# AndrewRLawrence/dp_gp_lvm

Measured on AMD Instinct MI355X. Metric: ELBO evals/sec (N=2000,D=512,M=128,Q=10), higher is better.
Workload: dtype f32 (psi-statistics: f16 hi/lo-split MFMA operands, fp32 accumulate) + f64 (Cholesky chain)

## Files before the change

dp_gp_lvm_amd/_lib.py:

```python
import ctypes
import os

_HERE = os.path.dirname(os.path.abspath(__file__))
LIB_PATH = os.environ.get('DPGP_LIBRARY') or os.path.join(_HERE, 'csrc', 'libdpgp_hip.so')

FLAG_NOISE, FLAG_JITTER = 1, 2
ALGO = {'auto': 0, 'plain': 1, 'mfma_f32': 2, 'patch_f16': 3}
PREC = {'f32': 0, 'mixed': 1, 'f64': 2, 'mixed_patch': 3, 'mixed_fast': 4}

_vp, _i, _d, _sz = ctypes.c_void_p, ctypes.c_int, ctypes.c_double, ctypes.c_size_t
_ll = ctypes.c_longlong

SIGNATURES = {
    'dpgp_version': (_i, []),
    'dpgp_last_hip_error': (ctypes.c_char_p, []),
    'dpgp_psi1T_y_workspace_bytes': (_sz, [_i, _i, _i]),
    'dpgp_psi2_workspace_bytes': (_sz, [_i, _i, _i, _i, _i]),
    'dpgp_potrf_workspace_bytes': (_sz, [_i, _i, _i]),
    'dpgp_trsm_workspace_bytes': (_sz, [_i, _i, _i, _i]),
    'dpgp_elbo_workspace_bytes': (_sz, [_i, _i, _i, _i, _i]),
    'dpgp_elbo_workspace_layout': (_i, [_i, _i, _i, _i, _i, _vp]),
    'dpgp_elbo_workspace_front_layout': (_i, [_i, _i, _i, _i, _i, _vp]),
    'dpgp_elbo_fhat': (_i, [_i, _i, _i, _i, _vp, _i, _vp, _vp, _vp, _vp, _vp, _vp, _d, _i, _i, _vp, _vp, _vp, _vp, _sz,
                            _vp]),
    'dpgp_elbo_fhat_ex': (_i, [_i, _i, _i, _i, _vp, _i, _vp, _vp, _vp, _vp, _vp, _vp, _d, _i, _i, _vp, _vp, _vp, _vp, _sz,
                               _vp, _vp]),
    'dpgp_elbo_fhat_t_workspace_bytes': (_sz, [_i, _i, _i, _i, _i, _i]),
    'dpgp_elbo_fhat_t': (_i, [_i, _i, _i, _i, _i, _vp, _i, _vp, _vp, _vp, _vp, _vp, _vp, _vp, _vp, _ll, _ll, _d, _i, _vp, _vp,
                              _vp, _vp, _vp, _sz, _vp, _vp, _vp, _vp, _vp, _vp, _vp]),
    'dpgp_elbo_grad_chain': (_i, [_i, _i, _i, _i, _vp, _vp, _d, _i, _vp, _sz, _vp, _vp, _vp, _vp, _vp, _vp]),
    'dpgp_elbo_grad_chain_ex': (_i, [_i, _i, _i, _i, _vp, _vp, _d, _i, _vp, _sz, _i, _vp, _vp, _vp, _vp, _vp, _vp]),
    'dpgp_elbo_grad_psi_workspace_bytes': (_sz, [_i, _i, _i, _i]),
    'dpgp_elbo_grad_psi_workspace_bytes_ex': (_sz, [_i, _i, _i, _i, _i]),
    'dpgp_elbo_fhat_step': (_i, [_i, _i, _i, _i, _vp, _i, _vp, _vp, _vp, _vp, _vp, _vp, _d, _vp, _vp, _vp, _vp, _sz, _vp, _sz, _vp, _vp]),
    'dpgp_elbo_grad_psi_step': (_i, [_i, _i, _i, _i, _vp, _i, _vp, _vp, _vp, _vp, _vp, _vp, _vp, _vp, _i, _vp, _sz, _vp, _sz, _vp, _vp,
                                     _vp, _vp, _vp]),
    'dpgp_elbo_step': (_i, [_i, _i, _i, _i, _vp, _i, _vp, _vp, _vp, _vp, _vp, _vp, _d, _i, _vp, _vp, _vp, _vp, _sz, _vp, _vp, _vp, _vp,
                            _vp, _vp, _sz, _vp, _vp, _vp, _vp, _vp, _vp]),
    'dpgp_elbo_grad_psi': (_i, [_i, _i, _i, _i, _vp, _i, _vp, _vp, _vp, _vp, _vp, _vp, _vp, _vp, _i, _vp, _sz, _vp, _vp, _vp,
                                _vp, _vp]),
    'dpgp_elbo_grad_psi_ex': (_i, [_i, _i, _i, _i, _vp, _i, _vp, _vp, _vp, _vp, _vp, _vp, _vp, _vp, _vp, _i, _vp, _sz, _vp, _vp,
                                   _vp, _vp, _vp]),
    'dpgp_event_create': (_vp, []),
    'dpgp_event_destroy': (None, [_vp]),
    'dpgp_stream_create': (_vp, []),
    'dpgp_stream_destroy': (None, [_vp]),
    'dpgp_event_elapsed_ms': (ctypes.c_float, [_vp, _vp]),
    'dpgp_model_prepare': (_i, [_i, _i, _i, _i, _i, _i, _vp, _vp, _vp, _vp, _vp, _vp, _vp, _vp, _d, _d, _i, _vp, _vp, _vp,
                                _vp, _vp, _vp, _vp]),
    'dpgp_model_prepare_t': (_i, [_i, _i, _i, _i, _i, _i, _vp, _vp, _vp, _vp, _vp, _vp, _vp, _vp, _d, _d, _i, _vp, _vp, _vp,
                                  _vp, _vp]),
    'dpgp_model_scal_count': (_i, [_i]),
    'dpgp_model_backward': (_i, [_i] * 8 + [_vp] * 10 + [_d, _d, _i] + [_vp] * 15 + [_vp]),
    'dpgp_model_backward_t': (_i, [_i] * 8 + [_vp] * 10 + [_d, _d, _i] + [_vp] * 16 + [_vp]),
    'dpgp_model_pack': (_i, [_i, _vp, _vp, _vp, _vp]),
    'dpgp_model_finalize': (_i, [_vp, _vp, _vp, _vp, _vp]),
    'dpgp_elbo_grad_chain_big_workspace_bytes': (_sz, [_i, _i]),
    'dpgp_elbo_grad_chain_big': (_i, [_i, _i, _i, _i, _vp, _vp, _vp, _vp, _d, _i, _vp, _sz, _i, _vp, _sz, _vp, _vp, _vp, _vp, _vp, _vp]),
    'dpgp_trouble_flag': (_i, [_sz, _vp, _i, _vp, _vp, _vp]),
    'dpgp_trtri_lower_batched_f64': (_i, [_i, _i, _vp, _vp, _vp, _sz, _vp]),
    'dpgp_ard_rbf_gram_grad_workspace_bytes': (_sz, [_i, _i]),
    'dpgp_ard_rbf_gram_grad_f64': (_i, [_i, _i, _vp, _vp, _vp, _vp, _i, _vp, _vp, _vp, _vp, _sz, _vp]),
    'dpgp_ard_rbf_gram_grad_batched_workspace_bytes': (_sz, [_i, _i, _i]),
    'dpgp_ard_rbf_gram_grad_batched_f64': (_i, [_i, _i, _i, _vp, _vp, _vp, _vp, _i, _ll, _vp, _vp, _vp, _vp, _sz, _vp]),
    'dpgp_qx_psi_stats_workspace_bytes': (_sz, [_i, _i, _i, _i]),
    'dpgp_qx_psi_stats_batched_f64': (_i, [_i, _i, _i, _i] + [_vp] * 8 + [_vp, _sz, _vp]),
    'dpgp_qx_psi_adjoint_workspace_bytes': (_sz, [_i, _i, _i, _i]),
    'dpgp_qx_psi_adjoint_f64': (_i, [_i, _i, _i, _i] + [_vp] * 10 + [_vp, _sz, _vp]),
    'dpgp_qx_psi_stats_weighted_f64': (_i, [_i, _i, _i, _i] + [_vp] * 9 + [_vp, _sz, _vp]),
    'dpgp_qx_psi_adjoint_weighted_f64': (_i, [_i, _i, _i, _i] + [_vp] * 11 + [_vp, _sz, _vp]),
    'dpgp_qx_psi_param_adjoint_workspace_bytes': (_sz, [_i, _i, _i, _i]),
    'dpgp_qx_psi_param_adjoint_weighted_f64': (_i, [_i, _i, _i, _i] + [_vp] * 12 + [_vp, _sz, _vp]),
    'dpgp_qx_psi_stats_grouped_workspace_bytes': (_sz, [_i] * 5),
    'dpgp_qx_psi_stats_grouped_f64': (_i, [_i] * 5 + [_vp] * 9 + [_vp, _sz, _vp]),
    'dpgp_qx_psi_adjoint_grouped_workspace_bytes': (_sz, [_i] * 5),
    'dpgp_qx_psi_adjoint_grouped_f64': (_i, [_i] * 5 + [_vp] * 11 + [_vp, _sz, _vp]),
    'dpgp_qx_psi_param_adjoint_grouped_workspace_bytes': (_sz, [_i] * 5),
    'dpgp_qx_psi_param_adjoint_grouped_f64': (_i, [_i] * 5 + [_vp] * 12 + [_vp, _sz, _vp]),
    'dpgp_qx_psi_pointwise_workspace_bytes': (_sz, [_i] * 6),
    'dpgp_qx_psi_pointwise_f64': (_i, [_i] * 6 + [_vp] * 10 + [_vp, _sz, _vp]),
    'dpgp_qx_psi_point_moments_workspace_bytes': (_sz, [_i] * 6),
    'dpgp_qx_psi_point_moments_f64': (_i, [_i] * 6 + [_vp] * 12 + [_vp, _sz, _vp]),
    'dpgp_qx_psi_pointwise_adjoint_workspace_bytes': (_sz, [_i] * 6),
    'dpgp_qx_psi_pointwise_adjoint_f64': (_i, [_i] * 6 + [_vp] * 13 + [_vp, _sz, _vp]),
    'dpgp_ard_rbf_point_metric_workspace_bytes': (_sz, [_i] * 4),
    'dpgp_ard_rbf_point_metric_f64': (_i, [_i] * 4 + [_vp] * 6 + [_vp, _sz, _vp]),
    'dpgp_ard_rbf_point_jacobian_workspace_bytes': (_sz, [_i] * 5),
    'dpgp_ard_rbf_point_jacobian_f64': (_i, [_i] * 5 + [_vp] * 6 + [_vp, _sz, _vp]),
    'dpgp_ard_rbf_point_energy_workspace_bytes': (_sz, [_i] * 4),
    'dpgp_ard_rbf_point_energy_f64': (_i, [_i] * 4 + [_vp] * 9 + [_vp, _sz, _vp]),
    'dpgp_ard_rbf_point_christoffel_workspace_bytes': (_sz, [_i] * 4),
    'dpgp_ard_rbf_point_christoffel_f64': (_i, [_i] * 4 + [_vp] * 8 + [_vp, _sz, _vp]),
    'dpgp_geodesic_accel_f64': (_i, [_i] * 3 + [_vp] * 7 + [_vp]),
    'dpgp_ard_rbf_point_christoffel_tangent_workspace_bytes': (_sz, [_i] * 4),
    'dpgp_ard_rbf_point_christoffel_tangent_f64': (_i, [_i] * 4 + [_vp] * 12 + [_vp, _sz, _vp]),
    'dpgp_geodesic_accel_tangent_f64': (_i, [_i] * 3 + [_vp] * 10 + [_vp]),
    'dpgp_ard_rbf_point_transport_workspace_bytes': (_sz, [_i] * 5),
    'dpgp_ard_rbf_point_transport_f64': (_i, [_i] * 5 + [_vp] * 10 + [_vp, _sz, _vp]),
    'dpgp_geodesic_transport_f64': (_i, [_i] * 4 + [_vp] * 9 + [_vp]),
    'dpgp_geodesic_shoot_workspace_bytes': (_sz, [_i, _vp, _vp, _i, _i, _i]),
    'dpgp_geodesic_shoot_f64': (_i, [_i, _vp, _vp, _i, _i, _i] + [_vp] * 10 + [_vp, _sz, _vp]),
    'dpgp_geodesic_shoot_tangent_f64': (_i, [_i, _vp, _vp, _i, _i, _i] + [_vp] * 15 + [_vp, _sz, _vp]),
    'dpgp_ard_rbf_point_cov_workspace_bytes': (_sz, [_i] * 5),
    'dpgp_ard_rbf_point_cov_f64': (_i, [_i] * 5 + [_vp] * 6 + [_vp, _sz, _vp]),
    'dpgp_psi_latent_adjoint_workspace_bytes': (_sz, [_i] * 4),
    'dpgp_psi_latent_adjoint_f64': (_i, [_i] * 4 + [_vp] * 6 + [_i] + [_vp] * 5 + [_vp, _sz, _vp]),
    'dpgp_psi2_weighted_f64': (_i, [_i, _i, _i, _i, _vp, _vp, _vp, _vp, _vp, _vp, _vp, _vp, _sz, _i, _vp]),
    'dpgp_elbo_grad_psi_weighted_f64': (_i, [_i, _i, _i, _i, _vp, _i, _vp, _vp, _vp, _vp, _vp, _vp, _vp, _vp, _vp, _vp, _sz, _vp,
                                             _vp, _vp, _vp, _vp]),
    'dpgp_gemm_strided_f64': (_i, [_i, _i, _i, _i, _d, _vp, _ll, _ll, _ll, _vp, _ll, _ll, _ll, _d, _vp, _ll, _ll, _ll, _vp]),
}
for _t in ('f32', 'f64'):
    SIGNATURES.update({
        'dpgp_ard_rbf_gram_' + _t: (_i, [_i, _i, _i, _i, _vp, _vp, _vp, _vp, _vp, _i, _d, _vp, _vp]),
        'dpgp_ard_rbf_diag_' + _t: (_i, [_i, _i, _vp, _vp, _i, _d, _vp, _vp]),
        'dpgp_psi0_' + _t: (_i, [_i, _i, _vp, _vp, _vp]),
        'dpgp_psi1_' + _t: (_i, [_i, _i, _i, _i, _vp, _vp, _vp, _vp, _vp, _vp, _vp]),
        'dpgp_psi1T_y_' + _t: (_i, [_i, _i, _i, _i, _vp, _vp, _vp, _vp, _vp, _vp, _i, _vp, _vp, _sz, _vp]),
        'dpgp_psi2_' + _t: (_i, [_i, _i, _i, _i, _vp, _vp, _vp, _vp, _vp, _vp, _vp, _sz, _i, _vp]),
        'dpgp_potrf_batched_' + _t: (_i, [_i, _i, _vp, _vp, _vp, _sz, _i, _vp]),
        'dpgp_trsm_batched_' + _t: (_i, [_i, _i, _i, _vp, _vp, _vp, _sz, _i, _vp]),
        'dpgp_kl_qx_' + _t: (_i, [_i, _i, _vp, _vp, _vp, _vp]),
    })



class ExecResources(ctypes.Structure):
    _fields_ = [('ev_psi2_begin', _vp), ('ev_psi2_end', _vp), ('model_scal', _vp), ('model_pack', _vp),
                ('model_out', _vp), ('stream_aux', _vp), ('ev_fork', _vp), ('ev_join', _vp)]


_lib = None


class DpgpLibraryMissing(RuntimeError):
    pass


def lib():
    global _lib
    if _lib is None:
        if not os.path.exists(LIB_PATH):
            raise DpgpLibraryMissing(
                'libdpgp_hip.so is not built: run `make -C %s` (hipcc, gfx950). dp_gp_lvm_amd has no CPU fallback.'
                % os.path.join(_HERE, 'csrc'))
        import torch
        l = ctypes.CDLL(LIB_PATH)
        for name, (res, args) in SIGNATURES.items():
            fn = getattr(l, name)
            fn.restype, fn.argtypes = res, args
        _lib = l
    return _lib


def check(rc, name):
    if rc != 0:
        if rc == -100:
            raise RuntimeError('%s: HIP kernel launch failed: %s' % (name, lib().dpgp_last_hip_error().decode()))
        raise ValueError('%s: bad argument #%d' % (name, -rc))
```

dp_gp_lvm_amd/csrc/elbo.hip:

```cpp
#include "internal.h"
#include "psi2_consts.h"

struct ElboLayout {
    size_t off_yy, off_v, off_p2, off_la, off_ld, off_ik, off_kl, off_pc, off_guard, off_sc, total;
    int ns1, ns2, Mp;
};

static ElboLayout elbo_layout(int D, int N, int M, int Q, int prec) {
    ElboLayout L;
    L.Mp = dpgp_round_up(M, 16);
    L.ns1 = psi1T_y_nsplit(D, N, M);
    L.ns2 = psi2_nsplit(D, N, M);
    const size_t sp = (prec == DPGP_PREC_F64) ? 8 : 4, sl = (prec == DPGP_PREC_F32) ? 4 : 8;
    size_t o = 0;
    L.off_yy = o; o += dpgp_align256(sizeof(double) * DPGP_YY_NCH * D);
    L.off_ld = o; o += dpgp_align256(sizeof(double) * D);
    L.off_ik = o; o += dpgp_align256(sizeof(int) * D);
    L.off_kl = o; o += dpgp_align256(sizeof(double) * DPGP_KL_NBLK + sizeof(int));
    L.off_guard = o; o += dpgp_align256(sizeof(double) * D);
    L.off_pc = o; o += dpgp_align256(psi2_consts_bytes(M, Q));
    L.off_sc = o; o += (prec == DPGP_PREC_F64) ? 0 : psi2_pairs_scale_bytes(D, M);
    L.off_v = o;  o += dpgp_align256(sizeof(double) * (size_t)L.ns1 * D * M);
    L.off_p2 = o; o += dpgp_align256(sp * (size_t)L.ns2 * D * L.Mp * L.Mp);
    L.off_la = o; o += dpgp_align256(sl * (size_t)D * la_chain_ws_elems(M));
    L.total = o;
    return L;
}

extern "C" size_t dpgp_elbo_workspace_bytes(int D, int N, int M, int Q, int prec) {
    if (D <= 0 || N <= 0 || M <= 0 || Q <= 0 || prec < 0 || prec > 2) return 0;
    return elbo_layout(D, N, M, Q, prec).total;
}

extern "C" int dpgp_elbo_workspace_layout(int D, int N, int M, int Q, int prec, size_t *out) {
    if (D <= 0 || N <= 0 || M <= 0 || Q <= 0 || prec < 0 || prec > 2) return -1;
    if (!out) return -6;
    const ElboLayout L = elbo_layout(D, N, M, Q, prec);
    out[0] = L.off_p2; out[1] = (size_t)L.ns2; out[2] = (prec == DPGP_PREC_F64) ? 8 : 4; out[3] = (size_t)L.Mp;
    out[4] = L.off_v;  out[5] = (size_t)L.ns1; out[6] = L.off_yy; out[7] = DPGP_YY_NCH;
    out[8] = L.off_guard; out[9] = (size_t)D;
    return DPGP_OK;
}

extern "C" int dpgp_elbo_workspace_front_layout(int D, int N, int M, int Q, int prec, size_t *out) {
    if (D <= 0 || N <= 0 || M <= 0 || Q <= 0 || prec < 0 || prec > 2) return -1;
    if (!out) return -6;
    const ElboLayout L = elbo_layout(D, N, M, Q, prec);
    const size_t sl = (prec == DPGP_PREC_F32) ? 4 : 8;
    out[0] = L.off_la; out[1] = sl * la_chain_ws_elems(M); out[2] = sl; out[3] = (size_t)L.Mp;
    out[4] = L.off_sc;
    out[5] = (prec != DPGP_PREC_F64 && psi2_pairs_ksteps(Q) <= 8) ? (size_t)psi2_consts_layout(M, Q).Ppad : 0;
    return DPGP_OK;
}

struct AuxJoin {
    hipStream_t st = nullptr, aux = nullptr;
    hipEvent_t ev = nullptr;
    bool armed = false;
    void arm(hipStream_t st_, hipStream_t aux_, hipEvent_t ev_) { st = st_; aux = aux_; ev = ev_; armed = true; }
    int join() {
        armed = false;
        return hipStreamWaitEvent(st, ev, 0) == hipSuccess ? DPGP_OK : DPGP_ERR_LAUNCH;
    }
    ~AuxJoin() {
        if (armed && hipEventRecord(ev, aux) == hipSuccess) (void)hipStreamWaitEvent(st, ev, 0);
    }
};

struct SideLaunch {
    int (*fn)(void *ctx, hipStream_t st);
    void *ctx;
};

template <typename TP, typename TL>
static int elbo_run(int D, int N, int M, int Q, const double *y, int ldy, const double *z, const double *mu,
                    const double *s, const double *gamma, const double *alpha, const double *beta, double jitter,
                    int algo, double *terms, double *sums, int *info, unsigned char *ws, const ElboLayout &L,
                    hipStream_t st, const dpgp_exec_t *ex, TL *lb_out = nullptr, unsigned char *pgws = nullptr,
                    bool psi1_from_pass = false, const SideLaunch *side = nullptr, bool *side_done = nullptr) {
    double *yy = reinterpret_cast<double *>(ws + L.off_yy);
    double *ldk = reinterpret_cast<double *>(ws + L.off_ld);
    int *ik = reinterpret_cast<int *>(ws + L.off_ik);
    double *vpart = reinterpret_cast<double *>(ws + L.off_v);
    TP *p2 = reinterpret_cast<TP *>(ws + L.off_p2);
    TL *la = reinterpret_cast<TL *>(ws + L.off_la);
    double *klp = reinterpret_cast<double *>(ws + L.off_kl);
    unsigned char *pconst = ws + L.off_pc;
    hipEvent_t ev0 = ex ? (hipEvent_t)ex->ev_psi2_begin : nullptr, ev1 = ex ? (hipEvent_t)ex->ev_psi2_end : nullptr;
    int rc;
    const bool pairs_psi2 = (sizeof(TP) == 4 && algo == DPGP_ALGO_AUTO && psi2_pairs_ksteps(Q) <= 8);
    const bool fac_from_gram = pairs_psi2 && pgws == nullptr;
    float *pscale = reinterpret_cast<float *>(ws + L.off_sc);
    if ((rc = launch_elbo_front<TL>(N, Q, mu, s, klp, D, y, ldy, yy, z, M, pconst, gamma, alpha, beta, jitter, la, L.Mp,
                                    la_chain_ws_elems(M), (pairs_psi2 && !fac_from_gram) ? pscale : nullptr,
                                    fac_from_gram ? pscale : nullptr, st)))
        return rc;
    hipStream_t aux = (ex && ex->stream_aux && ex->ev_fork && ex->ev_join) ? (hipStream_t)ex->stream_aux : nullptr;
    if (pgws != nullptr && psi1_from_pass && D > 256) aux = nullptr;
    AuxJoin aj;
    if (aux) {
        if (hipEventRecord((hipEvent_t)ex->ev_fork, st) != hipSuccess || hipStreamWaitEvent(aux, (hipEvent_t)ex->ev_fork, 0) != hipSuccess)
            return DPGP_ERR_LAUNCH;
        aj.arm(st, aux, (hipEvent_t)ex->ev_join);
    }
    const int ns1 = psi1_from_pass ? 1 : L.ns1;
    if (!psi1_from_pass &&
        (rc = launch_psi1T_y_partial<double, TP>(D, N, M, Q, z, mu, s, gamma, alpha, y, ldy, vpart, L.ns1, pconst, 1, aux ? aux : st)))
        return rc;
    const bool k_on_aux = aux && pgws != nullptr && la_chain_k_resident(M, (int)sizeof(TL)) && algo != DPGP_ALGO_PLAIN;
    if (k_on_aux && (rc = launch_chain_k<TL>(D, M, la, ldk, ik, algo, aux))) return rc;
    if (aux && hipEventRecord((hipEvent_t)ex->ev_join, aux) != hipSuccess) return DPGP_ERR_LAUNCH;
    const bool f16_psi2 = (sizeof(TP) == 4 && algo != DPGP_ALGO_MFMA_F32);
    const bool step = pgws != nullptr;
    if (step && !(pairs_psi2 && psi2_pgrad_supported(M, Q))) return -30;
    const bool fused_k = !step && (algo != DPGP_ALGO_PLAIN) && (!f16_psi2 || la_chain_k_resident(M, (int)sizeof(TL))) &&
                         !getenv("DPGP_UNFUSED_K");
    bool big = false;
    if constexpr (sizeof(TL) == 8) {
        big = (algo != DPGP_ALGO_PLAIN) && chain_big_applicable(D, M, 8);
        if (big && (rc = launch_chain_big_k(D, M, reinterpret_cast<double *>(la), ik, st))) return rc;
    }
    if (!big && !fused_k && !k_on_aux && (rc = launch_chain_k<TL>(D, M, la, ldk, ik, algo, st))) return rc;
    if (ev0 && hipEventRecord(ev0, st) != hipSuccess) return DPGP_ERR_LAUNCH;
    if (step) {
        if constexpr (sizeof(TP) == 4) {
            if ((rc = launch_psi2_pgrad(D, N, M, Q, pconst, z, mu, s, gamma, alpha, nullptr, pgws, nullptr, nullptr, nullptr, nullptr,
                                        nullptr, st, 1, reinterpret_cast<float *>(p2), pscale, psi1_from_pass ? y : nullptr, ldy, nullptr, 0,
                                        psi1_from_pass ? vpart : nullptr)))
                return rc;
        }
    } else if ((rc = launch_psi2_partial<double, TP>(D, N, M, Q, z, mu, s, gamma, alpha, p2, L.ns2, algo, st,
                                                     (fused_k && !big) ? (void *)la : nullptr, (int)sizeof(TL), ldk, ik, pconst,
                                                     pairs_psi2 ? 2 : 1, pscale)))
        return rc;
    if (ev1 && hipEventRecord(ev1, st) != hipSuccess) return DPGP_ERR_LAUNCH;
    if (aux && aj.join() != DPGP_OK) return DPGP_ERR_LAUNCH;
    if (big && lb_out) return -30;
    if (side && aux && !big && 2 * D <= 512) {
        if (hipEventRecord((hipEvent_t)ex->ev_fork, st) != hipSuccess || hipStreamWaitEvent(aux, (hipEvent_t)ex->ev_fork, 0) != hipSuccess)
            return DPGP_ERR_LAUNCH;
        aj.arm(st, aux, (hipEvent_t)ex->ev_join);
        if ((rc = side->fn(side->ctx, aux))) return rc;
        if (hipEventRecord((hipEvent_t)ex->ev_join, aux) != hipSuccess) return DPGP_ERR_LAUNCH;
        rc = launch_chain_b<TP, TL>(D, N, M, p2, step ? 1 : L.ns2, vpart, ns1, alpha, beta, yy, ldk, ik, terms, info,
                                    reinterpret_cast<double *>(ws + L.off_guard), la, algo, st, klp, sums,
                                    ex ? (const double *)ex->model_scal : nullptr, ex ? (double *)ex->model_pack : nullptr,
                                    ex ? (double *)ex->model_out : nullptr, lb_out);
        if (rc) return rc;
        if (side_done) *side_done = true;
        return aj.join();
    }
    if constexpr (sizeof(TL) == 8) {
        if (big)
            return launch_chain_big_b<TP>(D, N, M, p2, step ? 1 : L.ns2, vpart, ns1, alpha, beta, yy, ik, terms, info,
                                          reinterpret_cast<double *>(ws + L.off_guard), reinterpret_cast<double *>(la), st, klp,
                                          sums, ex ? (const double *)ex->model_scal : nullptr,
                                          ex ? (double *)ex->model_pack : nullptr, ex ? (double *)ex->model_out : nullptr);
    }
    return launch_chain_b<TP, TL>(D, N, M, p2, step ? 1 : L.ns2, vpart, ns1, alpha, beta, yy, ldk, ik, terms, info,
                                  reinterpret_cast<double *>(ws + L.off_guard), la, algo, st, klp, sums,
                                  ex ? (const double *)ex->model_scal : nullptr, ex ? (double *)ex->model_pack : nullptr,
                                  ex ? (double *)ex->model_out : nullptr, lb_out);
}

extern "C" int dpgp_elbo_grad_chain_ex(int D, int N, int M, int Q, const double *alpha, const double *beta, double jitter,
                                       int prec, void *ws, size_t ws_bytes, int psi2_slabs, double *g_psi2, double *w_kuu, double *g_v,
                                       double *d_alpha_beta, int *info, void *stream) {
    if (D <= 0) return -1;
    if (N <= 0) return -2;
    if (M <= 0) return -3;
    if (Q <= 0 || Q > DPGP_MAX_Q) return -4;
    if (!alpha) return -5;
    if (!beta) return -6;
    if (!(jitter >= 0.0)) return -7;
    if (prec != DPGP_PREC_MIXED && prec != DPGP_PREC_F64) return -8;
    if (!ws) return -9;
    const ElboLayout L = elbo_layout(D, N, M, Q, prec);
    if (ws_bytes < L.total) return -10;
    if (!g_psi2) return -11;
    if (!w_kuu) return -12;
    if (!g_v) return -13;
    if (!d_alpha_beta) return -14;
    if (!info) return -15;
    if (psi2_slabs < 0 || psi2_slabs > L.ns2) return -16;
    unsigned char *w = (unsigned char *)ws;
    const double *yy = reinterpret_cast<const double *>(w + L.off_yy), *vpart = reinterpret_cast<const double *>(w + L.off_v);
    double *la = reinterpret_cast<double *>(w + L.off_la);
    const int ns2 = psi2_slabs ? psi2_slabs : L.ns2;
    if (prec == DPGP_PREC_MIXED)
        return launch_chain_grad<float>(D, N, M, reinterpret_cast<const float *>(w + L.off_p2), ns2, vpart, L.ns1, alpha,
                                        beta, yy, jitter, la, g_psi2, w_kuu, g_v, d_alpha_beta, info, (hipStream_t)stream);
    return launch_chain_grad<double>(D, N, M, reinterpret_cast<const double *>(w + L.off_p2), ns2, vpart, L.ns1, alpha,
                                     beta, yy, jitter, la, g_psi2, w_kuu, g_v, d_alpha_beta, info, (hipStream_t)stream);
}
extern "C" int dpgp_elbo_grad_chain(int D, int N, int M, int Q, const double *alpha, const double *beta, double jitter,
                                    int prec, void *ws, size_t ws_bytes, double *g_psi2, double *w_kuu, double *g_v,
                                    double *d_alpha_beta, int *info, void *stream) {
    return dpgp_elbo_grad_chain_ex(D, N, M, Q, alpha, beta, jitter, prec, ws, ws_bytes, 0, g_psi2, w_kuu, g_v, d_alpha_beta, info, stream);
}

extern "C" size_t dpgp_elbo_grad_chain_big_workspace_bytes(int D, int M) {
    return (D > 0 && M > 0) ? chain_grad_big_ws_bytes(D, M) : 0;
}
extern "C" int dpgp_elbo_grad_chain_big(int D, int N, int M, int Q, const double *z, const double *gamma, const double *alpha,
                                        const double *beta, double jitter, int prec, void *fwd_ws, size_t fwd_ws_bytes, int psi2_slabs,
                                        void *ws, size_t ws_bytes, double *g_psi2, double *w_kuu, double *g_v, double *d_alpha_beta,
                                        int *info, void *stream) {
    if (D <= 0) return -1;
    if (N <= 0) return -2;
    if (M <= 0 || !chain_grad_big_supported(M)) return -3;
    if (Q <= 0 || Q > DPGP_MAX_Q) return -4;
    if (!z) return -5;
    if (!gamma) return -6;
    if (!alpha) return -7;
    if (!beta) return -8;
    if (!(jitter >= 0.0)) return -9;
    if (prec != DPGP_PREC_MIXED && prec != DPGP_PREC_F64) return -10;
    if (!fwd_ws) return -11;
    const ElboLayout L = elbo_layout(D, N, M, Q, prec);
    if (fwd_ws_bytes < L.total) return -12;
    if (psi2_slabs < 0 || psi2_slabs > L.ns2) return -13;
    if (!ws) return -14;
    if (ws_bytes < chain_grad_big_ws_bytes(D, M)) return -15;
    if (!g_psi2) return -16;
    if (!w_kuu) return -17;
    if (!g_v) return -18;
    if (!d_alpha_beta) return -19;
    if (!info) return -20;
    const unsigned char *w = (const unsigned char *)fwd_ws;
    const double *yy = reinterpret_cast<const double *>(w + L.off_yy), *vpart = reinterpret_cast<const double *>(w + L.off_v);
    const int ns2 = psi2_slabs ? psi2_slabs : L.ns2;
    if (prec == DPGP_PREC_MIXED)
        return launch_chain_grad_big<float>(D, N, M, Q, z, gamma, alpha, beta, jitter, reinterpret_cast<const float *>(w + L.off_p2), ns2,
                                            vpart, L.ns1, yy, (unsigned char *)ws, g_psi2, w_kuu, g_v, d_alpha_beta, info, (hipStream_t)stream);
    return launch_chain_grad_big<double>(D, N, M, Q, z, gamma, alpha, beta, jitter, reinterpret_cast<const double *>(w + L.off_p2), ns2,
                                         vpart, L.ns1, yy, (unsigned char *)ws, g_psi2, w_kuu, g_v, d_alpha_beta, info, (hipStream_t)stream);
}

struct GradPsiWs { unsigned char *consts; double *part, *ws1, *stage; unsigned char *pgws; };
static bool grad_psi_needs_patch(int M, int Q, bool patch_form) {
    return patch_form || !psi2_pgrad_supported(M, Q) || getenv("DPGP_GRAD_PATCH");
}
static GradPsiWs grad_psi_ws(int D, int N, int M, int Q, unsigned char *ws, bool patch_form) {
    GradPsiWs W;
    const size_t mx = (size_t)Q * (N > D ? (N > M ? N : M) : (D > M ? D : M));
    W.consts = ws + dpgp_align256(psi_grad_ws_bytes_kuu(D, M, Q));
    W.part = reinterpret_cast<double *>(W.consts + dpgp_align256(psi2_consts_bytes(M, Q)));
    W.ws1 = reinterpret_cast<double *>((unsigned char *)W.part +
                                       (grad_psi_needs_patch(M, Q, patch_form) ? dpgp_align256(sizeof(double) * psi2_grad_part_elems(D, N, M, Q)) : 0));
    W.stage = reinterpret_cast<double *>((unsigned char *)W.ws1 + dpgp_align256(sizeof(double) * psi1_grad_ws_elems(D, N, M, Q)));
    W.pgws = reinterpret_cast<unsigned char *>(W.stage) + dpgp_align256(sizeof(double) * reduce_rows_stage_elems(mx));
    return W;
}
static int grad_psi_mixed(int D, int N, int M, int Q, const double *y, int ldy, const double *z, const double *mu, const double *s,
                          const double *gamma, const double *alpha, const double *g_psi2, const double *w_kuu, const double *g_v,
                          const double *g_psi1, bool patch_form, unsigned char *ws, double *d_mu, double *d_s, double *d_z,
                          double *d_gamma, hipStream_t st, const unsigned char *fwd_consts, const float *fwd_scale,
                          const float *fwd_psi2 = nullptr, int w11 = 0, double *psi1_front_done = nullptr) {
    const bool fast = psi2_grad_supported(M, Q) && !getenv("DPGP_GRAD_PLAIN");
    const bool big = dpgp_round_up(M, 16) > 128;
    if (big && !fast) return -30;
    int rc = DPGP_OK;
    if (!big && !fast) {
        if (g_psi1) return -15;
        return launch_psi_grad<float>(D, N, M, Q, y, ldy, z, mu, s, gamma, alpha, g_psi2, w_kuu, g_v ? g_v : w_kuu, (double *)ws,
                                      d_mu, d_s, d_z, d_gamma, 1, st);
    }
    const GradPsiWs W = grad_psi_ws(D, N, M, Q, ws, patch_form);
    const unsigned char *consts = fwd_consts ? fwd_consts : W.consts;
    if (!fwd_consts && (rc = launch_psi2_consts<double>(z, M, Q, W.consts, st)) != DPGP_OK) return rc;
    rc = launch_kuu_grad(D, M, Q, consts, gamma, w_kuu, (double *)ws, W.stage, d_z, d_gamma, st);
    if (rc != DPGP_OK) return rc;
    const bool pair_form = psi2_pgrad_supported(M, Q) && !patch_form && !getenv("DPGP_GRAD_PATCH");
    const bool psi1_pairs = pair_form && !g_psi1 && y && g_v && !getenv("DPGP_PSI1_PLAIN");
    if (!psi1_pairs) {
        rc = launch_psi1_grad(D, N, M, Q, y, ldy, consts, mu, s, gamma, alpha, g_v, g_psi1, W.ws1, W.stage, d_mu, d_s, d_z, d_gamma, st);
        if (rc != DPGP_OK) return rc;
    }
    if (pair_form)
        return launch_psi2_pgrad(D, N, M, Q, consts, z, mu, s, gamma, alpha, g_psi2, W.pgws, W.stage, d_mu, d_s, d_z, d_gamma, st,
                                 fwd_consts ? 2 : 3, const_cast<float *>(fwd_psi2), fwd_scale, psi1_pairs ? y : nullptr, ldy,
                                 psi1_pairs ? g_v : nullptr, w11, (fwd_consts && psi1_pairs) ? psi1_front_done : nullptr);
    if (fwd_consts) return -30;
    return launch_psi2_grad(D, N, M, Q, consts, mu, s, gamma, alpha, g_psi2, W.part, W.stage, d_mu, d_s, d_z, d_gamma, st);
}

extern "C" size_t dpgp_elbo_grad_psi_workspace_bytes_ex(int D, int N, int M, int Q, int prec) {
    if (D <= 0 || N <= 0 || M <= 0 || Q <= 0) return 0;
    if (prec == DPGP_PREC_F64 || !psi2_grad_supported(M, Q) || getenv("DPGP_GRAD_PLAIN"))
        return dpgp_align256(psi_grad_ws_bytes(D, N, M, Q, nullptr));
    const bool patch = (prec == DPGP_PREC_MIXED_PATCH);
    const size_t mx = (size_t)Q * (N > D ? (N > M ? N : M) : (D > M ? D : M));
    size_t b = dpgp_align256(psi_grad_ws_bytes_kuu(D, M, Q)) + dpgp_align256(psi2_consts_bytes(M, Q)) +
               (grad_psi_needs_patch(M, Q, patch) ? dpgp_align256(sizeof(double) * psi2_grad_part_elems(D, N, M, Q)) : 0) +
               dpgp_align256(sizeof(double) * psi1_grad_ws_elems(D, N, M, Q)) + dpgp_align256(sizeof(double) * reduce_rows_stage_elems(mx));
    if (!patch) b += dpgp_align256(psi2_pgrad_ws_bytes(D, N, M, Q));
    return b;
}
extern "C" size_t dpgp_elbo_grad_psi_workspace_bytes(int D, int N, int M, int Q) {
    return dpgp_elbo_grad_psi_workspace_bytes_ex(D, N, M, Q, DPGP_PREC_MIXED);
}
extern "C" int dpgp_elbo_grad_psi_ex(int D, int N, int M, int Q, const double *y, int ldy, const double *z, const double *mu,
                                     const double *s, const double *gamma, const double *alpha, const double *g_psi2,
                                     const double *w_kuu, const double *g_v, const double *g_psi1, int prec, void *ws,
                                     size_t ws_bytes, double *d_mu, double *d_s, double *d_z, double *d_gamma, void *stream);
extern "C" int dpgp_elbo_grad_psi(int D, int N, int M, int Q, const double *y, int ldy, const double *z, const double *mu,
                                  const double *s, const double *gamma, const double *alpha, const double *g_psi2,
                                  const double *w_kuu, const double *g_v, int prec, void *ws, size_t ws_bytes,
                                  double *d_mu, double *d_s, double *d_z, double *d_gamma, void *stream) {
    return dpgp_elbo_grad_psi_ex(D, N, M, Q, y, ldy, z, mu, s, gamma, alpha, g_psi2, w_kuu, g_v, nullptr, prec, ws, ws_bytes,
                                 d_mu, d_s, d_z, d_gamma, stream);
}
static int elbo_grad_psi_impl(int D, int N, int M, int Q, const double *y, int ldy, const double *z, const double *mu,
                              const double *s, const double *gamma, const double *alpha, const double *g_psi2,
                              const double *w_kuu, const double *g_v, const double *g_psi1, int prec, void *ws,
                              size_t ws_bytes, double *d_mu, double *d_s, double *d_z, double *d_gamma, void *stream,
                              const double *wts) {
    if (D <= 0) return -1;
    if (N <= 0) return -2;
    if (M <= 0) return -3;
    if (Q <= 0 || Q > DPGP_MAX_Q) return -4;
    if (!y && !g_psi1) return -5;
    if (y && ldy < D) return -6;
    if (!z) return -7;
    if (!mu) return -8;
    if (!s) return -9;
    if (!gamma) return -10;
    if (!alpha) return -11;
    if (!g_psi2) return -12;
    if (!w_kuu) return -13;
    if (!g_v && !g_psi1) return -14;
    const bool patch_form = (prec == DPGP_PREC_MIXED_PATCH), fast = (prec == DPGP_PREC_MIXED_FAST);
    if (patch_form || fast) prec = DPGP_PREC_MIXED;
    if (prec != DPGP_PREC_MIXED && prec != DPGP_PREC_F64) return -15;
    if (g_psi1 && (prec != DPGP_PREC_MIXED || !psi2_grad_supported(M, Q))) return -15;
    if (!ws) return -16;
    if (ws_bytes < dpgp_elbo_grad_psi_workspace_bytes_ex(D, N, M, Q, patch_form ? DPGP_PREC_MIXED_PATCH : prec)) return -17;
    if (!d_mu) return -18;
    if (!d_s) return -19;
    if (!d_z) return -20;
    if (!d_gamma) return -21;
    if (prec == DPGP_PREC_MIXED)
        return grad_psi_mixed(D, N, M, Q, y, ldy, z, mu, s, gamma, alpha, g_psi2, w_kuu, g_v, g_psi1, patch_form, (unsigned char *)ws,
                              d_mu, d_s, d_z, d_gamma, (hipStream_t)stream, nullptr, nullptr, nullptr, fast ? 1 : 0);
    if (dpgp_round_up(M, 16) > 128) return -30;
    return launch_psi_grad<double>(D, N, M, Q, y, ldy, z, mu, s, gamma, alpha, g_psi2, w_kuu, g_v, (double *)ws, d_mu, d_s,
                                   d_z, d_gamma, 1, (hipStream_t)stream, wts);
}
extern "C" int dpgp_elbo_grad_psi_ex(int D, int N, int M, int Q, const double *y, int ldy, const double *z, const double *mu,
                                     const double *s, const double *gamma, const double *alpha, const double *g_psi2,
                                     const double *w_kuu, const double *g_v, const double *g_psi1, int prec, void *ws,
                                     size_t ws_bytes, double *d_mu, double *d_s, double *d_z, double *d_gamma, void *stream) {
    return elbo_grad_psi_impl(D, N, M, Q, y, ldy, z, mu, s, gamma, alpha, g_psi2, w_kuu, g_v, g_psi1, prec, ws, ws_bytes, d_mu,
                              d_s, d_z, d_gamma, stream, nullptr);
}
extern "C" int dpgp_elbo_grad_psi_weighted_f64(int D, int N, int M, int Q, const double *y, int ldy, const double *z,
                                               const double *mu, const double *s, const double *gamma, const double *alpha,
                                               const double *w, const double *g_psi2, const double *w_kuu, const double *g_v,
                                               void *ws, size_t ws_bytes, double *d_mu, double *d_s, double *d_z,
                                               double *d_gamma, void *stream) {
    return elbo_grad_psi_impl(D, N, M, Q, y, ldy, z, mu, s, gamma, alpha, g_psi2, w_kuu, g_v, nullptr, DPGP_PREC_F64, ws,
                              ws_bytes, d_mu, d_s, d_z, d_gamma, stream, w);
}

extern "C" int dpgp_elbo_fhat_ex(int D, int N, int M, int Q, const double *y, int ldy, const double *z,
                                 const double *mu, const double *s, const double *gamma, const double *alpha,
                                 const double *beta, double jitter, int prec, int algo, double *terms, double *sums,
                                 int *info, void *ws, size_t ws_bytes, void *stream, const dpgp_exec_t *exec) {
    if (D <= 0) return -1;
    if (N <= 0) return -2;
    if (M <= 0) return -3;
    if (Q <= 0 || Q > DPGP_MAX_Q) return -4;
    if (!y) return -5;
    if (ldy < D) return -6;
    if (!z) return -7;
    if (!mu) return -8;
    if (!s) return -9;
    if (!gamma) return -10;
    if (!alpha) return -11;
    if (!beta) return -12;
    if (!(jitter >= 0.0)) return -13;
    if (prec < 0 || prec > 2) return -14;
    if (algo < 0 || algo > DPGP_ALGO_PATCH_F16) return -15;
    if (!terms) return -16;
    if (!sums) return -17;
    if (!info) return -18;
    if (!ws) return -19;
    const ElboLayout L = elbo_layout(D, N, M, Q, prec);
    if (ws_bytes < L.total) return -20;
    hipStream_t st = (hipStream_t)stream;
    unsigned char *w = (unsigned char *)ws;
    switch (prec) {
    case DPGP_PREC_F32:
        return elbo_run<float, float>(D, N, M, Q, y, ldy, z, mu, s, gamma, alpha, beta, jitter, algo, terms, sums, info,
                                      w, L, st, exec);
    case DPGP_PREC_MIXED:
        return elbo_run<float, double>(D, N, M, Q, y, ldy, z, mu, s, gamma, alpha, beta, jitter, algo, terms, sums,
                                       info, w, L, st, exec);
    default:
        return elbo_run<double, double>(D, N, M, Q, y, ldy, z, mu, s, gamma, alpha, beta, jitter, algo, terms, sums,
                                        info, w, L, st, exec);
    }
}

extern "C" int dpgp_elbo_fhat(int D, int N, int M, int Q, const double *y, int ldy, const double *z, const double *mu,
                              const double *s, const double *gamma, const double *alpha, const double *beta,
                              double jitter, int prec, int algo, double *terms, double *sums, int *info, void *ws,
                              size_t ws_bytes, void *stream) {
    return dpgp_elbo_fhat_ex(D, N, M, Q, y, ldy, z, mu, s, gamma, alpha, beta, jitter, prec, algo, terms, sums, info, ws,
                             ws_bytes, stream, nullptr);
}

extern "C" int dpgp_elbo_step(int D, int N, int M, int Q, const double *y, int ldy, const double *z, const double *mu,
                              const double *s, const double *gamma, const double *alpha, const double *beta, double jitter,
                              int prec, double *terms, double *sums, int *info, void *ws, size_t ws_bytes, double *g_psi2, double *w_kuu,
                              double *g_v, double *d_alpha_beta, int *info_grad, void *gws, size_t gws_bytes, double *d_mu,
                              double *d_s, double *d_z, double *d_gamma, void *stream, const dpgp_exec_t *exec) {
    if (D <= 0) return -1;
    if (N <= 0) return -2;
    if (M <= 0 || dpgp_round_up(M, 16) > 128) return -3;
    if (Q <= 0 || Q > DPGP_MAX_Q || !psi2_pgrad_supported(M, Q)) return -4;
    if (!y) return -5;
    if (ldy < D) return -6;
    if (!z) return -7;
    if (!mu) return -8;
    if (!s) return -9;
    if (!gamma) return -10;
    if (!alpha) return -11;
    if (!beta) return -12;
    if (!(jitter >= 0.0)) return -13;
    if (prec != DPGP_PREC_MIXED && prec != DPGP_PREC_MIXED_FAST) return -14;
    if (!terms) return -15;
    if (!sums) return -16;
    if (!info) return -17;
    if (!ws) return -18;
    const ElboLayout L = elbo_layout(D, N, M, Q, DPGP_PREC_MIXED);
    if (ws_bytes < L.total) return -19;
    if (!g_psi2) return -20;
    if (!w_kuu) return -21;
    if (!g_v) return -22;
    if (!d_alpha_beta) return -23;
    if (!info_grad) return -24;
    if (!gws) return -25;
    if (gws_bytes < dpgp_elbo_grad_psi_workspace_bytes(D, N, M, Q)) return -26;
    if (!d_mu) return -27;
    if (!d_s) return -28;
    if (!d_z) return -29;
    if (!d_gamma) return -30;
    hipStream_t st = (hipStream_t)stream;
    unsigned char *w = (unsigned char *)ws;
    const GradPsiWs W = grad_psi_ws(D, N, M, Q, (unsigned char *)gws, false);
    const bool v_from_pass = !getenv("DPGP_PSI1_PLAIN") && !getenv("DPGP_GRAD_PATCH") && !getenv("DPGP_GRAD_PLAIN");
    struct StageA {
        int D, N, M, ns1;
        const unsigned char *w;
        const ElboLayout *L;
        const double *alpha, *beta;
        double jitter, *g_psi2, *w_kuu, *g_v, *dab;
        int *info;
    } sa = {D, N, M, v_from_pass ? 1 : L.ns1, w, &L, alpha, beta, jitter, g_psi2, w_kuu, g_v, d_alpha_beta, info_grad};
    auto stage_a = [](void *c, hipStream_t s_) -> int {
        const StageA &a = *static_cast<const StageA *>(c);
        return launch_chain_grad<float>(a.D, a.N, a.M, reinterpret_cast<const float *>(a.w + a.L->off_p2), 1,
                                        reinterpret_cast<const double *>(a.w + a.L->off_v), a.ns1, a.alpha, a.beta,
                                        reinterpret_cast<const double *>(a.w + a.L->off_yy), a.jitter,
                                        reinterpret_cast<double *>(const_cast<unsigned char *>(a.w) + a.L->off_la), a.g_psi2, a.w_kuu, a.g_v,
                                        a.dab, a.info, s_);
    };
    const SideLaunch side = {stage_a, &sa};
    bool side_done = false;
    int rc = elbo_run<float, double>(D, N, M, Q, y, ldy, z, mu, s, gamma, alpha, beta, jitter, DPGP_ALGO_AUTO, terms, sums, info, w,
                                     L, st, exec, nullptr, W.pgws, v_from_pass, &side, &side_done);
    if (rc != DPGP_OK) return rc;
    if (!side_done && (rc = stage_a(&sa, st)) != DPGP_OK) return rc;
    return grad_psi_mixed(D, N, M, Q, y, ldy, z, mu, s, gamma, alpha, g_psi2, w_kuu, g_v, nullptr, false, (unsigned char *)gws, d_mu,
                          d_s, d_z, d_gamma, st, w + L.off_pc, reinterpret_cast<const float *>(w + L.off_sc),
                          reinterpret_cast<const float *>(w + L.off_p2), prec == DPGP_PREC_MIXED_FAST ? 1 : 0,
                          v_from_pass ? reinterpret_cast<double *>(w + L.off_v) : nullptr);
}

extern "C" int dpgp_elbo_fhat_step(int D, int N, int M, int Q, const double *y, int ldy, const double *z, const double *mu,
                                   const double *s, const double *gamma, const double *alpha, const double *beta, double jitter,
                                   double *terms, double *sums, int *info, void *ws, size_t ws_bytes, void *gws, size_t gws_bytes,
                                   void *stream, const dpgp_exec_t *exec) {
    if (D <= 0) return -1;
    if (N <= 0) return -2;
    if (M <= 0) return -3;
    if (Q <= 0 || Q > DPGP_MAX_Q || !psi2_pgrad_supported(M, Q)) return -4;
    if (!y) return -5;
    if (ldy < D) return -6;
    if (!z) return -7;
    if (!mu) return -8;
    if (!s) return -9;
    if (!gamma) return -10;
    if (!alpha) return -11;
    if (!beta) return -12;
    if (!(jitter >= 0.0)) return -13;
    if (!terms) return -14;
    if (!sums) return -15;
    if (!info) return -16;
    if (!ws) return -17;
    const ElboLayout L = elbo_layout(D, N, M, Q, DPGP_PREC_MIXED);
    if (ws_bytes < L.total) return -18;
    if (!gws) return -19;
    if (gws_bytes < dpgp_elbo_grad_psi_workspace_bytes(D, N, M, Q)) return -20;
    const GradPsiWs W = grad_psi_ws(D, N, M, Q, (unsigned char *)gws, false);
    return elbo_run<float, double>(D, N, M, Q, y, ldy, z, mu, s, gamma, alpha, beta, jitter, DPGP_ALGO_AUTO, terms, sums, info,
                                   (unsigned char *)ws, L, (hipStream_t)stream, exec, nullptr, W.pgws);
}
extern "C" int dpgp_elbo_grad_psi_step(int D, int N, int M, int Q, const double *y, int ldy, const double *z, const double *mu,
                                       const double *s, const double *gamma, const double *alpha, const double *g_psi2,
                                       const double *w_kuu, const double *g_v, int prec, void *ws, size_t ws_bytes, void *gws,
                                       size_t gws_bytes, double *d_mu, double *d_s, double *d_z, double *d_gamma, void *stream) {
    if (D <= 0) return -1;
    if (N <= 0) return -2;
    if (M <= 0) return -3;
    if (Q <= 0 || Q > DPGP_MAX_Q || !psi2_pgrad_supported(M, Q)) return -4;
    if (!y) return -5;
    if (ldy < D) return -6;
    if (!z) return -7;
    if (!mu) return -8;
    if (!s) return -9;
    if (!gamma) return -10;
    if (!alpha) return -11;
    if (!g_psi2) return -12;
    if (!w_kuu) return -13;
    if (!g_v) return -14;
    if (prec != DPGP_PREC_MIXED && prec != DPGP_PREC_MIXED_FAST) return -15;
    if (!ws) return -16;
    const ElboLayout L = elbo_layout(D, N, M, Q, DPGP_PREC_MIXED);
    if (ws_bytes < L.total) return -17;
    if (!gws) return -18;
    if (gws_bytes < dpgp_elbo_grad_psi_workspace_bytes(D, N, M, Q)) return -19;
    if (!d_mu) return -20;
    if (!d_s) return -21;
    if (!d_z) return -22;
    if (!d_gamma) return -23;
    unsigned char *w = (unsigned char *)ws;
    return grad_psi_mixed(D, N, M, Q, y, ldy, z, mu, s, gamma, alpha, g_psi2, w_kuu, g_v, nullptr, false, (unsigned char *)gws, d_mu,
                          d_s, d_z, d_gamma, (hipStream_t)stream, w + L.off_pc, reinterpret_cast<const float *>(w + L.off_sc),
                          reinterpret_cast<const float *>(w + L.off_p2), prec == DPGP_PREC_MIXED_FAST ? 1 : 0);
}

struct ElboTLayout {
    ElboLayout L;
    size_t off_fused, off_terms, off_sums, off_lb, off_p1, off_vp, total;
    int ksplit, nlow;
};
static ElboTLayout elbo_t_layout(int T, int D, int N, int M, int Q, int prec) {
    ElboTLayout E;
    E.L = elbo_layout(T, N, M, Q, prec);
    const int Mp = E.L.Mp, nb = Mp / 16;
    E.nlow = nb * (nb + 1) / 2;
    const int tiles = dpgp_ceil_div(D, 64) * dpgp_ceil_div(M, 64) * T;
    int ks = 512 / (tiles > 0 ? tiles : 1);
    if (ks > 8) ks = 8;
    if (ks > N / 64) ks = N / 64;
    if (ks < 1) ks = 1;
    E.ksplit = ks;
    size_t o = 0;
    E.off_fused = o; o += dpgp_align256(E.L.total);
    E.off_terms = o; o += dpgp_align256(sizeof(double) * 5 * T);
    E.off_sums = o;  o += 256;
    E.off_lb = o;    o += dpgp_align256(sizeof(double) * (size_t)T * E.nlow * DPGP_LB_TILE_ELEMS);
    E.off_p1 = o;    o += dpgp_align256(sizeof(double) * (size_t)T * N * M);
    E.off_vp = o;    o += dpgp_align256(sizeof(double) * (size_t)ks * T * M * D);
    E.total = o;
    return E;
}
extern "C" size_t dpgp_elbo_fhat_t_workspace_bytes(int T, int D, int N, int M, int Q, int prec) {
    if (T <= 0 || D < T || N <= 0 || M <= 0 || Q <= 0 || prec < 1 || prec > 2) return 0;
    return elbo_t_layout(T, D, N, M, Q, prec).total;
}

__global__ __launch_bounds__(256) void fhat_t_combine_kernel(int T, int D, int N, const double *__restrict__ terms,
                                                             const double *__restrict__ phit, const double *__restrict__ quad,
                                                             const double *__restrict__ yy, const double *__restrict__ beta,
                                                             const double *__restrict__ sums_in, double *__restrict__ per_t,
                                                             double *__restrict__ sums, long long phi_st, long long phi_sd,
                                                             const double *__restrict__ model_scal,
                                                             double *__restrict__ model_pack, double *__restrict__ model_out) {
    __shared__ double scratch[8];
    const int t = threadIdx.x;
    double acc = 0.0;
    for (int e = t; e < T * D; e += 256) {
        const int a = e / D, d = e - a * D;
        const double *o = terms + 5 * a;
        const double pt = o[0] + 0.5 * N * DPGP_LOG_2PI + o[1] + o[2];
        acc += phit[a * phi_st + d * phi_sd] * (pt + 0.5 * quad[e] - 0.5 * beta[a] * yy[d]);
    }
    acc = block_sum(acc, scratch);
    if (t < T) {
        const double *o = terms + 5 * t;
        per_t[t] = o[0] + 0.5 * N * DPGP_LOG_2PI + o[1] + o[2];
    }
    if (t == 0) {
        const double fhat = acc - 0.5 * (double)N * (double)D * DPGP_LOG_2PI, kl = sums_in[1];
        sums[0] = fhat;
        sums[1] = kl;
        if (model_scal) {
            double a = model_scal[0];
            const int nrb = (D + DPGP_PREP_ROWS - 1) / DPGP_PREP_ROWS;
            for (int i = 0; i < nrb; ++i) a += model_scal[2 + i];
            if (model_pack) { model_pack[0] = fhat; model_pack[1] = -a; }
            if (model_out) {
                const double hyper = model_scal[1];
                model_out[0] = -a - (fhat - kl) - hyper;
                model_out[1] = fhat; model_out[2] = kl; model_out[3] = -a; model_out[4] = hyper;
            }
        }
    }
}

extern "C" int dpgp_elbo_fhat_t(int T, int D, int N, int M, int Q, const double *y, int ldy, const double *yy, const double *z,
                                const double *mu, const double *s, const double *gamma, const double *alpha, const double *beta,
                                const double *phit, long long phi_st, long long phi_sd, double jitter, int prec, double *per_t,
                                double *quad, double *sums, int *info, void *ws, size_t ws_bytes, void *stream,
                                const double *model_scal, double *model_pack, double *model_out, void *stream_aux,
                                void *ev_fork, void *ev_join) {
    if (T <= 0) return -1;
    if (D < T) return -2;
    if (N <= 0) return -3;
    if (M <= 0) return -4;
    if (Q <= 0 || Q > DPGP_MAX_Q) return -5;
    if (!y) return -6;
    if (ldy < D) return -7;
    if (!yy) return -8;
    if (!z || !mu || !s) return -9;
    if (!gamma || !alpha || !beta) return -12;
    if (!phit) return -15;
    if (!(jitter >= 0.0)) return -16;
    if (prec != DPGP_PREC_MIXED && prec != DPGP_PREC_F64) return -17;
    if (!per_t || !quad || !sums || !info) return -18;
    if (!ws) return -22;
    if (dpgp_round_up(M, 16) > 128) return -30;
    const ElboTLayout E = elbo_t_layout(T, D, N, M, Q, prec);
    if (ws_bytes < E.total) return -23;
    hipStream_t st = (hipStream_t)stream;
    unsigned char *w = (unsigned char *)ws;
    double *terms = reinterpret_cast<double *>(w + E.off_terms), *sums2 = reinterpret_cast<double *>(w + E.off_sums);
    double *lb = reinterpret_cast<double *>(w + E.off_lb), *p1 = reinterpret_cast<double *>(w + E.off_p1);
    double *vp = reinterpret_cast<double *>(w + E.off_vp);
    int rc;
    hipStream_t aux = (stream_aux && ev_fork && ev_join) ? (hipStream_t)stream_aux : nullptr;
    if (aux) {
        hipStreamCaptureStatus cs = hipStreamCaptureStatusNone;
        if (hipStreamIsCapturing(st, &cs) != hipSuccess || cs != hipStreamCaptureStatusNone) aux = nullptr;
    }
    if (aux && (hipEventRecord((hipEvent_t)ev_fork, st) != hipSuccess || hipStreamWaitEvent(aux, (hipEvent_t)ev_fork, 0) != hipSuccess))
        return DPGP_ERR_LAUNCH;
    AuxJoin aj;
    if (aux) aj.arm(st, aux, (hipEvent_t)ev_join);
    hipStream_t sb = aux ? aux : st;
    if (aux) {
        if ((rc = dpgp_psi1_f64(T, N, M, Q, z, mu, s, gamma, alpha, p1, (void *)sb))) return rc - 100;
        if ((rc = launch_gemm_splitk_f64(T, M, D, N, p1, (long long)N * M, 1, M, y, 0, ldy, 1, vp, (long long)M * D, D, 1, E.ksplit,
                                         (long long)T * M * D, sb)))
            return rc - 200;
        if (hipEventRecord((hipEvent_t)ev_join, aux) != hipSuccess) return DPGP_ERR_LAUNCH;
    }
    if (prec == DPGP_PREC_MIXED)
        rc = elbo_run<float, double>(T, N, M, Q, y, ldy, z, mu, s, gamma, alpha, beta, jitter, DPGP_ALGO_AUTO, terms, sums2, info,
                                     w + E.off_fused, E.L, st, nullptr, lb);
    else
        rc = elbo_run<double, double>(T, N, M, Q, y, ldy, z, mu, s, gamma, alpha, beta, jitter, DPGP_ALGO_AUTO, terms, sums2, info,
                                      w + E.off_fused, E.L, st, nullptr, lb);
    if (rc) return rc;
    if (!aux) {
        if ((rc = dpgp_psi1_f64(T, N, M, Q, z, mu, s, gamma, alpha, p1, stream))) return rc - 100;
        if ((rc = launch_gemm_splitk_f64(T, M, D, N, p1, (long long)N * M, 1, M, y, 0, ldy, 1, vp, (long long)M * D, D, 1, E.ksplit,
                                         (long long)T * M * D, st)))
            return rc - 200;
    } else if (aj.join() != DPGP_OK) {
        return DPGP_ERR_LAUNCH;
    }
    if ((rc = launch_tcols_quad(T, M, D, lb, vp, E.ksplit, (long long)T * M * D, beta, quad, st))) return rc;
    DPGP_PRELAUNCH();
    hipLaunchKernelGGL(fhat_t_combine_kernel, dim3(1), dim3(256), 0, st, T, D, N, terms, phit, quad, yy, beta, sums2, per_t, sums,
                       phi_st, phi_sd, model_scal, model_pack, model_out);
    DPGP_LAUNCH_CHECK();
    return DPGP_OK;
}

extern "C" void *dpgp_event_create(void) {
    hipEvent_t e = nullptr;
    return hipEventCreate(&e) == hipSuccess ? (void *)e : nullptr;
}
extern "C" void dpgp_event_destroy(void *e) {
    if (e) (void)hipEventDestroy((hipEvent_t)e);
}
extern "C" void *dpgp_stream_create(void) {
    hipStream_t s = nullptr;
    return hipStreamCreateWithFlags(&s, hipStreamNonBlocking) == hipSuccess ? (void *)s : nullptr;
}
extern "C" void dpgp_stream_destroy(void *s) {
    if (s) (void)hipStreamDestroy((hipStream_t)s);
}
extern "C" float dpgp_event_elapsed_ms(void *a, void *b) {
    float ms = -1.0f;
    if (hipEventElapsedTime(&ms, (hipEvent_t)a, (hipEvent_t)b) != hipSuccess) return -1.0f;
    return ms;
}

__device__ __forceinline__ double softplus_d(double x) { return fmax(x, 0.0) + log1p(exp(-fabs(x))); }

__device__ double digamma_d(double x) {
    double r = 0.0;
    while (x < 10.0) { r -= 1.0 / x; x += 1.0; }
    const double f = 1.0 / (x * x);
    const double t = f * (-1.0 / 12.0 + f * (1.0 / 120.0 + f * (-1.0 / 252.0 + f * (1.0 / 240.0 + f * (-1.0 / 132.0 +
                     f * (691.0 / 32760.0 + f * (-1.0 / 12.0)))))));
    return r + log(x) - 0.5 / x + t;
}

#define PREP_MAX_T 64
#define PREP_ROWS DPGP_PREP_ROWS

__global__ __launch_bounds__(256) void model_prepare_kernel(
    int D, int T, int Q, int N, int d_offset, int mask_size, int nrb, const double *__restrict__ logits,
    const double *__restrict__ gat_raw, const double *__restrict__ aat_raw, const double *__restrict__ bat_raw,
    const double *__restrict__ s_raw, const double *__restrict__ g1_raw, const double *__restrict__ g2_raw,
    const double *__restrict__ w_raw, double s1, double s2, int add_constants, double *__restrict__ gamma,
    double *__restrict__ alpha, double *__restrict__ beta, double *__restrict__ s_out, double *__restrict__ phi_out,
    double *__restrict__ scal, double *__restrict__ atoms_out) {
    const int t = threadIdx.x;
    __shared__ double scratch[8];
    if ((int)blockIdx.x > nrb) {
        const size_t tot = (size_t)N * Q;
        const int nsb = gridDim.x - 1 - nrb;
        for (size_t i = (size_t)(blockIdx.x - 1 - nrb) * 256 + t; i < tot; i += (size_t)nsb * 256)
            s_out[i] = softplus_d(s_raw[i]);
        return;
    }
    if (blockIdx.x == 0) {
        double hyper = 0.0, consts = 0.0;
        for (int i = t; i < T * Q + 2 * T; i += 256) {
            const double raw = i < T * Q ? gat_raw[i] : (i < T * Q + T ? aat_raw[i - T * Q] : bat_raw[i - T * Q - T]);
            const double sp = softplus_d(raw), lx = log(sp);
            if (atoms_out) atoms_out[i] = sp;
            hyper += -lx - 0.5 * (DPGP_LOG_2PI + lx * lx);
        }
        const double w1 = softplus_d(w_raw[0]), w2 = softplus_d(w_raw[1]);
        __shared__ double sf[6][PREP_MAX_T], sx[3];
        for (int i = t; i < 6 * (T - 1) + 3; i += 256) {
            if (i < 6 * (T - 1)) {
                const int k = i / 6, f = i - 6 * k;
                const double g1 = softplus_d(g1_raw[k]), g2 = softplus_d(g2_raw[k]);
                const double x = (f % 3 == 0) ? g1 : ((f % 3 == 1) ? g2 : g1 + g2);
                sf[f][k] = f < 3 ? lgamma(x) : digamma_d(x);
            } else {
                const int f = i - 6 * (T - 1);
                sx[f] = f == 0 ? digamma_d(w1) : (f == 1 ? lgamma(s1) : lgamma(w1));
            }
        }
        __syncthreads();
        if (t < T - 1) {
            const double g1 = softplus_d(g1_raw[t]), g2 = softplus_d(g2_raw[t]);
            const double p1 = sf[3][t], p2 = sf[4][t], p12 = sf[5][t];
            consts += (w1 / w2 - 1.0) * (p2 - p12) +
                      (sf[0][t] + sf[1][t] - sf[2][t] - (g1 - 1.0) * p1 - (g2 - 1.0) * p2 + (g1 + g2 - 2.0) * p12);
        }
        if (t == 0) {
            const double pw = sx[0], lw2 = log(w2);
            consts += (T - 1.0) * (pw - lw2)
                      + s1 * log(s2) - sx[1] + (s1 - 1.0) * (pw - lw2) - s2 * (w1 / w2)
                      + w1 - lw2 + sx[2] + (1.0 - w1) * pw;
        }
        hyper = block_sum(hyper, scratch);
        consts = block_sum(consts, scratch);
        if (t == 0) {
            scal[0] = add_constants ? consts : 0.0;
            scal[1] = hyper;
        }
        return;
    }
    __shared__ double gat[PREP_MAX_T * DPGP_MAX_Q], aat[PREP_MAX_T], bat[PREP_MAX_T];
    __shared__ double c1[PREP_MAX_T], c2[PREP_MAX_T];
    for (int i = t; i < T * Q; i += 256) gat[i] = softplus_d(gat_raw[i]);
    if (t < T) {
        aat[t] = softplus_d(aat_raw[t]);
        bat[t] = softplus_d(bat_raw[t]);
    }
    __shared__ double dg[3][PREP_MAX_T];
    if (t >= 64 && t - 64 < 3 * (T - 1)) {
        const int k = (t - 64) / 3, f = (t - 64) - 3 * k;
        const double g1 = softplus_d(g1_raw[k]), g2 = softplus_d(g2_raw[k]);
        dg[f][k] = digamma_d(f == 0 ? g1 : (f == 1 ? g2 : g1 + g2));
    }
    __syncthreads();
    if (t < T - 1) {
        c1[t] = dg[0][t] - dg[2][t];
        c2[t] = dg[1][t] - dg[2][t];
    }
    __syncthreads();
    const int rb = blockIdx.x - 1, cols = Q + 1;
    double dsum = 0.0;
    for (int e = t; e < PREP_ROWS * cols; e += 256) {
        const int rr = e / cols, j = e - rr * cols, d = rb * PREP_ROWS + rr;
        if (d >= D) continue;
        const double *lr = logits + (size_t)((d_offset + d) / mask_size) * T;
        double mx = lr[0];
        for (int k = 1; k < T; ++k) mx = fmax(mx, lr[k]);
        double zsum = 0.0;
        for (int k = 0; k < T; ++k) zsum += exp(lr[k] - mx);
        const double lz = log(zsum);
        if (j < Q) {
            double g = 0.0;
            if (!gamma) continue;
            for (int k = 0; k < T; ++k) g += exp(lr[k] - mx - lz) * gat[k * Q + j];
            gamma[(size_t)d * Q + j] = g;
        } else {
            double al = 0.0, be = 0.0, ent = 0.0, ev = 0.0, tail = 0.0;
            for (int k = T - 1; k >= 0; --k) {
                const double lp = lr[k] - mx - lz, p = exp(lp);
                if (phi_out) phi_out[(size_t)d * T + k] = p;
                al += p * aat[k];
                be += p * bat[k];
                ent -= p * lp;
                if (k < T - 1) ev += p * c1[k] + tail * c2[k];
                tail += p;
            }
            if (alpha) alpha[d] = al;
            if (beta) beta[d] = be;
            dsum += ev + ent;
        }
    }
    dsum = block_sum(dsum, scratch);
    if (t == 0) scal[2 + rb] = dsum;
}

__global__ void model_finalize_kernel(const double *__restrict__ fhat, const double *__restrict__ dp,
                                      const double *__restrict__ kl, const double *__restrict__ hyper,
                                      double *__restrict__ out) {
    if (threadIdx.x == 0 && blockIdx.x == 0) {
        out[0] = dp[0] - (fhat[0] - kl[0]) - hyper[0];
        out[1] = fhat[0];
        out[2] = kl[0];
        out[3] = dp[0];
        out[4] = hyper[0];
    }
}

__global__ void model_pack_kernel(const double *__restrict__ fhat, const double *__restrict__ scal, int nrb,
                                  double *__restrict__ pack) {
    if (threadIdx.x == 0 && blockIdx.x == 0) {
        double a = scal[0];
        for (int i = 0; i < nrb; ++i) a += scal[2 + i];
        pack[0] = fhat[0];
        pack[1] = -a;
    }
}

__device__ double trigamma_d(double x) {
    double r = 0.0;
    while (x < 10.0) { r += 1.0 / (x * x); x += 1.0; }
    const double f = 1.0 / (x * x);
    return r + 1.0 / x + 0.5 * f + (1.0 / x) * f * (1.0 / 6.0 - f * (1.0 / 30.0 - f * (1.0 / 42.0 - f * (1.0 / 30.0 - f * (
               5.0 / 66.0 - f * (691.0 / 2730.0 - f * (7.0 / 6.0)))))));
}
__device__ __forceinline__ double sigmoid_d(double x) { return 1.0 / (1.0 + exp(-x)); }

__global__ __launch_bounds__(256) void model_backward_kernel(
    int D, int T, int Q, int N, int M, int d_offset, int mask_size, int nlb, const double *__restrict__ logits,
    const double *__restrict__ gat_raw, const double *__restrict__ aat_raw, const double *__restrict__ bat_raw,
    const double *__restrict__ s_raw, const double *__restrict__ g1_raw, const double *__restrict__ g2_raw,
    const double *__restrict__ w_raw, const double *__restrict__ x_mean, const double *__restrict__ phi, double s1,
    double s2, int add_constants, const double *__restrict__ df_dmu, const double *__restrict__ df_ds,
    const double *__restrict__ df_dz, const double *__restrict__ df_dgamma, const double *__restrict__ df_dab,
    const double *__restrict__ df_dphi, double *__restrict__ d_x_mean, double *__restrict__ d_s_raw, double *__restrict__ d_x_u,
    double *__restrict__ d_logits, double *__restrict__ d_g1_raw, double *__restrict__ d_g2_raw,
    double *__restrict__ d_w_raw, double *__restrict__ d_gat_raw, double *__restrict__ d_aat_raw,
    double *__restrict__ d_bat_raw) {
    const int t = threadIdx.x;
    __shared__ double gat[PREP_MAX_T * DPGP_MAX_Q], aat[PREP_MAX_T], bat[PREP_MAX_T];
    __shared__ double c1[PREP_MAX_T], c2cum[PREP_MAX_T + 1], scratch[8];
    if ((int)blockIdx.x > nlb) {
        const size_t nq = (size_t)N * Q, mq = (size_t)M * Q;
        const int nb = gridDim.x - 1 - nlb;
        for (size_t i = (size_t)(blockIdx.x - 1 - nlb) * 256 + t; i < nq + mq; i += (size_t)nb * 256) {
            if (i < nq) {
                const double sv = softplus_d(s_raw[i]);
                d_x_mean[i] = -df_dmu[i] + (add_constants ? x_mean[i] : 0.0);
                d_s_raw[i] = (-df_ds[i] + (add_constants ? 0.5 * (1.0 - 1.0 / sv) : 0.0)) * sigmoid_d(s_raw[i]);
            } else {
                d_x_u[i - nq] = -df_dz[i - nq];
            }
        }
        return;
    }
    for (int i = t; i < T * Q; i += 256) gat[i] = softplus_d(gat_raw[i]);
    if (t < T) {
        aat[t] = softplus_d(aat_raw[t]);
        bat[t] = softplus_d(bat_raw[t]);
    }
    __shared__ double c2inc[PREP_MAX_T];
    if (t < T) {
        if (t < T - 1) {
            const double g1 = softplus_d(g1_raw[t]), g2 = softplus_d(g2_raw[t]), p12 = digamma_d(g1 + g2);
            c1[t] = digamma_d(g1) - p12;
            c2inc[t] = digamma_d(g2) - p12;
        } else {
            c1[t] = 0.0;
            c2inc[t] = 0.0;
        }
    }
    __shared__ double tg[3][PREP_MAX_T], tg_w;
    if (blockIdx.x == 0) {
        const int u = 255 - t;
        if (u < 3 * (T - 1)) {
            const int k = u / 3, f = u - 3 * k;
            const double g1 = softplus_d(g1_raw[k]), g2 = softplus_d(g2_raw[k]);
            tg[f][k] = trigamma_d(f == 0 ? g1 : (f == 1 ? g2 : g1 + g2));
        } else if (u == 3 * (T - 1) && add_constants) {
            tg_w = trigamma_d(softplus_d(w_raw[0]));
        }
    }
    __syncthreads();
    if (t == 0) {
        double cum = 0.0;
        for (int k = 0; k < T; ++k) {
            c2cum[k] = cum;
            cum += c2inc[k];
        }
        c2cum[T] = cum;
    }
    __syncthreads();
    if (blockIdx.x == 0) {
        const int cols = Q + 3;
        __shared__ double ph_s[2048], x_s[2048], sphi_s[PREP_MAX_T];
        int DC = 2048 / (T > cols ? T : cols);
        DC = DC > 128 ? 128 : DC;
        for (int e0 = 0; e0 < T * cols; e0 += 256) {
            const int e = e0 + t, k = e / cols, j = e - k * cols;
            double acc = 0.0;
            for (int dc = 0; dc < D; dc += DC) {
                __syncthreads();
                for (int i = t; i < DC * T; i += 256) {
                    const int dd = i / T;
                    ph_s[i] = (dc + dd < D) ? phi[(size_t)dc * T + i] : 0.0;
                }
                for (int i = t; i < DC * cols; i += 256) {
                    const int dd = i / cols, jj = i - dd * cols, d = dc + dd;
                    x_s[i] = (d < D) ? (jj > Q + 1 ? 1.0 : (df_dphi ? 0.0 : (jj < Q ? df_dgamma[(size_t)d * Q + jj] : (jj == Q ? df_dab[2 * d] : df_dab[2 * d + 1])))) : 0.0;
                }
                __syncthreads();
                if (e < T * cols)
                    for (int dd = 0; dd < DC; ++dd) acc += ph_s[dd * T + k] * x_s[dd * cols + j];
            }
            if (e < T * cols) {
                if (j <= Q + 1) {
                    if (df_dphi) acc = j < Q ? df_dgamma[(size_t)k * Q + j] : (j == Q ? df_dab[2 * k] : df_dab[2 * k + 1]);
                    const double raw = j < Q ? gat_raw[k * Q + j] : (j == Q ? aat_raw[k] : bat_raw[k]);
                    const double x = softplus_d(raw);
                    const double hyp = add_constants ? (1.0 / x + log(x) / x) : 0.0;
                    const double g = (-acc + hyp) * sigmoid_d(raw);
                    if (j < Q) d_gat_raw[k * Q + j] = g;
                    else if (j == Q) d_aat_raw[k] = g;
                    else d_bat_raw[k] = g;
                } else {
                    sphi_s[k] = acc;
                }
            }
        }
        __syncthreads();
        if (t < T - 1) {
            const int k = t;
            const double sphi = sphi_s[k];
            double stail = 0.0;
            for (int kk = k + 1; kk < T; ++kk) stail += sphi_s[kk];
            const double g1 = softplus_d(g1_raw[k]), g2 = softplus_d(g2_raw[k]);
            const double t1 = tg[0][k], t2 = tg[1][k], t12 = tg[2][k];
            double e1 = sphi * (t1 - t12) - stail * t12, e2 = -sphi * t12 + stail * (t2 - t12);
            if (add_constants) {
                const double w1 = softplus_d(w_raw[0]), w2 = softplus_d(w_raw[1]), r = w1 / w2 - 1.0;
                e1 += -r * t12 - (g1 - 1.0) * t1 + (g1 + g2 - 2.0) * t12;
                e2 += r * (t2 - t12) - (g2 - 1.0) * t2 + (g1 + g2 - 2.0) * t12;
            }
            d_g1_raw[k] = -e1 * sigmoid_d(g1_raw[k]);
            d_g2_raw[k] = -e2 * sigmoid_d(g2_raw[k]);
        }
        if (t == 0) {
            double e1 = 0.0, e2 = 0.0;
            if (add_constants) {
                const double w1 = softplus_d(w_raw[0]), w2 = softplus_d(w_raw[1]), tw = tg_w, sc2 = c2cum[T];
                e1 = (T - 1.0) * tw + sc2 / w2 + (s1 - 1.0) * tw - s2 / w2 + 1.0 + (1.0 - w1) * tw;
                e2 = -(T - 1.0) / w2 - (w1 / (w2 * w2)) * sc2 - (s1 - 1.0) / w2 + s2 * w1 / (w2 * w2) - 1.0 / w2;
            }
            d_w_raw[0] = -e1 * sigmoid_d(w_raw[0]);
            d_w_raw[1] = -e2 * sigmoid_d(w_raw[1]);
        }
        return;
    }
    const int r0 = d_offset / mask_size, r1 = (d_offset + D - 1) / mask_size;
    const int r = r0 + ((int)blockIdx.x - 1) * 256 + t;
    if (r > r1) return;
    const int dlo = max(r * mask_size, d_offset) - d_offset, dhi = min((r + 1) * mask_size, d_offset + D) - d_offset;
    for (int k = 0; k < T; ++k) d_logits[(size_t)r * T + k] = 0.0;
    const double *lr = logits + (size_t)r * T;
    double mx = lr[0];
    for (int k = 1; k < T; ++k) mx = fmax(mx, lr[k]);
    double zsum = 0.0;
    for (int k = 0; k < T; ++k) zsum += exp(lr[k] - mx);
    const double lz = log(zsum);
    for (int d = dlo; d < dhi; ++d) {
        const double *ph = phi + (size_t)d * T;
        const double *dg = df_dgamma + (size_t)(df_dphi ? 0 : d) * Q;
        const double da = df_dphi ? 0.0 : df_dab[2 * d], db = df_dphi ? 0.0 : df_dab[2 * d + 1];
        auto gk = [&](int k) {
            double mix = da * aat[k] + db * bat[k];
            if (df_dphi) mix = df_dphi[(size_t)d * T + k];
            else
                for (int q = 0; q < Q; ++q) mix += dg[q] * gat[k * Q + q];
            return -mix - (c1[k] + c2cum[k] - (lr[k] - mx - lz) - 1.0);
        };
        double sdot = 0.0;
        for (int k = 0; k < T; ++k) sdot += ph[k] * gk(k);
        for (int k = 0; k < T; ++k) d_logits[(size_t)r * T + k] += ph[k] * (gk(k) - sdot);
    }
}

static int model_backward_run(int D, int T, int Q, int N, int M, int d_offset, int mask_size, int logits_rows,
                                   const double *logits, const double *gamma_atoms_raw, const double *alpha_atoms_raw,
                                   const double *beta_atoms_raw, const double *s_raw, const double *g1_raw,
                                   const double *g2_raw, const double *w_raw, const double *x_mean, const double *phi,
                                   double s1, double s2, int add_constants, const double *df_dmu, const double *df_ds,
                                   const double *df_dz, const double *df_dgamma, const double *df_dalpha_beta,
                                   double *d_x_mean, double *d_s_raw, double *d_x_u, double *d_logits, double *d_g1_raw,
                                   double *d_g2_raw, double *d_w_raw, double *d_gamma_atoms_raw,
                                   double *d_alpha_atoms_raw, double *d_beta_atoms_raw, void *stream, const double *df_dphi) {
    if (D <= 0) return -1;
    if (T <= 0 || T > PREP_MAX_T) return -2;
    if (Q <= 0 || Q > DPGP_MAX_Q) return -3;
    if (N <= 0) return -4;
    if (M <= 0) return -5;
    if (d_offset < 0) return -6;
    if (mask_size <= 0) return -7;
    if (logits_rows <= 0 || (d_offset + D - 1) / mask_size >= logits_rows) return -8;
    const void *ins[] = {logits, gamma_atoms_raw, alpha_atoms_raw, beta_atoms_raw, s_raw, g1_raw, g2_raw, w_raw, x_mean, phi};
    for (int i = 0; i < 10; ++i)
        if (!ins[i] && !(T == 1 && (i == 5 || i == 6))) return -(9 + i);
    if (!(s1 > 0.0)) return -19;
    if (!(s2 > 0.0)) return -20;
    const void *gs[] = {df_dmu, df_ds, df_dz, df_dgamma, df_dalpha_beta};
    for (int i = 0; i < 5; ++i)
        if (!gs[i]) return -(22 + i);
    void *outs[] = {d_x_mean, d_s_raw, d_x_u, d_logits, d_g1_raw, d_g2_raw, d_w_raw, d_gamma_atoms_raw, d_alpha_atoms_raw,
                    d_beta_atoms_raw};
    for (int i = 0; i < 10; ++i)
        if (!outs[i] && !(T == 1 && (i == 4 || i == 5))) return -(27 + i);
    hipStream_t st = (hipStream_t)stream;
    if (hipMemsetAsync(d_logits, 0, sizeof(double) * (size_t)logits_rows * T, st) != hipSuccess) return DPGP_ERR_LAUNCH;
    const int rows = (d_offset + D - 1) / mask_size - d_offset / mask_size + 1, nlb = dpgp_ceil_div(rows, 256);
    int neb = dpgp_ceil_div(N * Q + M * Q, 256 * 4);
    if (neb > 1024) neb = 1024;
    DPGP_PRELAUNCH(); hipLaunchKernelGGL(model_backward_kernel, dim3(1 + nlb + neb), dim3(256), 0, st, D, T, Q, N, M, d_offset, mask_size, nlb,
                       logits, gamma_atoms_raw, alpha_atoms_raw, beta_atoms_raw, s_raw, g1_raw, g2_raw, w_raw, x_mean, phi, s1, s2,
                       add_constants, df_dmu, df_ds, df_dz, df_dgamma, df_dalpha_beta, df_dphi, d_x_mean, d_s_raw, d_x_u, d_logits,
                       d_g1_raw, d_g2_raw, d_w_raw, d_gamma_atoms_raw, d_alpha_atoms_raw, d_beta_atoms_raw);
    DPGP_LAUNCH_CHECK();
    return DPGP_OK;
}

__global__ __launch_bounds__(1024) void trouble_flag_kernel(size_t n, const double *__restrict__ flat, int d, const int *__restrict__ info,
                                                            double *__restrict__ out) {
    const int t = threadIdx.x;
    const size_t i0 = (size_t)blockIdx.x * 1024 + t, stride = (size_t)gridDim.x * 1024;
    int bad = 0;
    for (size_t i = i0; i < n; i += stride) {
        const double v = flat[i];
        bad |= !(fabs(v) <= 1.7976931348623157e308);
    }
    for (size_t i = i0; i < (size_t)d; i += stride) bad |= info[i] != 0;
    if (__any(bad) && (t & 63) == 0) out[0] = 1.0;
}
extern "C" int dpgp_trouble_flag(size_t n, const double *flat, int d, const int *info, double *out, void *stream) {
    if (n > 0 && !flat) return -2;
    if (d < 0 || (d > 0 && !info)) return -4;
    if (!out) return -5;
    hipStream_t st = (hipStream_t)stream;
    if (hipMemsetAsync(out, 0, sizeof(double), st) != hipSuccess) return DPGP_ERR_LAUNCH;
    const size_t work = n > (size_t)d ? n : (size_t)d;
    unsigned grid = (unsigned)((work + 8191) / 8192);
    if (grid < 1) grid = 1;
    if (grid > 256) grid = 256;
    DPGP_PRELAUNCH();
    hipLaunchKernelGGL(trouble_flag_kernel, dim3(grid), dim3(1024), 0, st, n, flat, d, info, out);
    DPGP_LAUNCH_CHECK();
    return DPGP_OK;
}

extern "C" int dpgp_model_backward(int D, int T, int Q, int N, int M, int d_offset, int mask_size, int logits_rows,
                                   const double *logits, const double *gamma_atoms_raw, const double *alpha_atoms_raw,
                                   const double *beta_atoms_raw, const double *s_raw, const double *g1_raw,
                                   const double *g2_raw, const double *w_raw, const double *x_mean, const double *phi,
                                   double s1, double s2, int add_constants, const double *df_dmu, const double *df_ds,
                                   const double *df_dz, const double *df_dgamma, const double *df_dalpha_beta,
                                   double *d_x_mean, double *d_s_raw, double *d_x_u, double *d_logits, double *d_g1_raw,
                                   double *d_g2_raw, double *d_w_raw, double *d_gamma_atoms_raw,
                                   double *d_alpha_atoms_raw, double *d_beta_atoms_raw, void *stream) {
    return model_backward_run(D, T, Q, N, M, d_offset, mask_size, logits_rows, logits, gamma_atoms_raw, alpha_atoms_raw, beta_atoms_raw,
                              s_raw, g1_raw, g2_raw, w_raw, x_mean, phi, s1, s2, add_constants, df_dmu, df_ds, df_dz, df_dgamma,
                              df_dalpha_beta, d_x_mean, d_s_raw, d_x_u, d_logits, d_g1_raw, d_g2_raw, d_w_raw, d_gamma_atoms_raw,
                              d_alpha_atoms_raw, d_beta_atoms_raw, stream, nullptr);
}
extern "C" int dpgp_model_backward_t(int D, int T, int Q, int N, int M, int d_offset, int mask_size, int logits_rows,
                                     const double *logits, const double *gamma_atoms_raw, const double *alpha_atoms_raw,
                                     const double *beta_atoms_raw, const double *s_raw, const double *g1_raw, const double *g2_raw,
                                     const double *w_raw, const double *x_mean, const double *phi, double s1, double s2,
                                     int add_constants, const double *df_dmu, const double *df_ds, const double *df_dz,
                                     const double *df_dgamma_atoms, const double *df_dalpha_beta_atoms, const double *df_dphi,
                                     double *d_x_mean, double *d_s_raw, double *d_x_u, double *d_logits, double *d_g1_raw,
                                     double *d_g2_raw, double *d_w_raw, double *d_gamma_atoms_raw, double *d_alpha_atoms_raw,
                                     double *d_beta_atoms_raw, void *stream) {
    if (!df_dphi) return -27;
    const int rc = model_backward_run(D, T, Q, N, M, d_offset, mask_size, logits_rows, logits, gamma_atoms_raw, alpha_atoms_raw,
                                      beta_atoms_raw, s_raw, g1_raw, g2_raw, w_raw, x_mean, phi, s1, s2, add_constants, df_dmu, df_ds,
                                      df_dz, df_dgamma_atoms, df_dalpha_beta_atoms, d_x_mean, d_s_raw, d_x_u, d_logits, d_g1_raw,
                                      d_g2_raw, d_w_raw, d_gamma_atoms_raw, d_alpha_atoms_raw, d_beta_atoms_raw, stream, df_dphi);
    return rc <= -27 ? rc - 1 : rc;
}

extern "C" int dpgp_model_scal_count(int D) { return D > 0 ? 2 + dpgp_ceil_div(D, PREP_ROWS) : 0; }

static int model_prepare_run(int D, int T, int Q, int N, int d_offset, int mask_size, const double *logits,
                             const double *gamma_atoms_raw, const double *alpha_atoms_raw, const double *beta_atoms_raw,
                             const double *s_raw, const double *g1_raw, const double *g2_raw, const double *w_raw, double s1,
                             double s2, int add_constants, double *gamma, double *alpha, double *beta, double *s, double *phi,
                             double *scal, double *atoms, void *stream) {
    if (D <= 0) return -1;
    if (T <= 0 || T > PREP_MAX_T) return -2;
    if (Q <= 0 || Q > DPGP_MAX_Q) return -3;
    if (N <= 0) return -4;
    if (d_offset < 0) return -5;
    if (mask_size <= 0) return -6;
    if (!logits) return -7;
    if (!gamma_atoms_raw) return -8;
    if (!alpha_atoms_raw) return -9;
    if (!beta_atoms_raw) return -10;
    if (!s_raw) return -11;
    if (T > 1 && (!g1_raw || !g2_raw)) return -12;
    if (!w_raw) return -14;
    if (!(s1 > 0.0)) return -15;
    if (!(s2 > 0.0)) return -16;
    if (!s) return -21;
    if (!scal) return -23;
    const int nrb = dpgp_ceil_div(D, PREP_ROWS);
    int sblocks = dpgp_ceil_div(N * Q, 256 * 2);
    if (sblocks > 512) sblocks = 512;
    DPGP_PRELAUNCH(); hipLaunchKernelGGL(model_prepare_kernel, dim3(1 + nrb + sblocks), dim3(256), 0, (hipStream_t)stream, D, T, Q, N,
                       d_offset, mask_size, nrb, logits, gamma_atoms_raw, alpha_atoms_raw, beta_atoms_raw, s_raw, g1_raw,
                       g2_raw, w_raw, s1, s2, add_constants, gamma, alpha, beta, s, phi, scal, atoms);
    DPGP_LAUNCH_CHECK();
    return DPGP_OK;
}
extern "C" int dpgp_model_prepare(int D, int T, int Q, int N, int d_offset, int mask_size, const double *logits,
                                  const double *gamma_atoms_raw, const double *alpha_atoms_raw,
                                  const double *beta_atoms_raw, const double *s_raw, const double *g1_raw,
                                  const double *g2_raw, const double *w_raw, double s1, double s2, int add_constants,
                                  double *gamma, double *alpha, double *beta, double *s, double *phi, double *scal,
                                  void *stream) {
    if (!gamma) return -18;
    if (!alpha) return -19;
    if (!beta) return -20;
    return model_prepare_run(D, T, Q, N, d_offset, mask_size, logits, gamma_atoms_raw, alpha_atoms_raw, beta_atoms_raw, s_raw,
                             g1_raw, g2_raw, w_raw, s1, s2, add_constants, gamma, alpha, beta, s, phi, scal, nullptr, stream);
}
extern "C" int dpgp_model_prepare_t(int D, int T, int Q, int N, int d_offset, int mask_size, const double *logits,
                                    const double *gamma_atoms_raw, const double *alpha_atoms_raw,
                                    const double *beta_atoms_raw, const double *s_raw, const double *g1_raw,
                                    const double *g2_raw, const double *w_raw, double s1, double s2, int add_constants,
                                    double *s, double *phi, double *atoms, double *scal, void *stream) {
    if (!phi) return -22;
    if (!atoms) return -24;
    return model_prepare_run(D, T, Q, N, d_offset, mask_size, logits, gamma_atoms_raw, alpha_atoms_raw, beta_atoms_raw, s_raw,
                             g1_raw, g2_raw, w_raw, s1, s2, add_constants, nullptr, nullptr, nullptr, s, phi, scal, atoms, stream);
}

extern "C" int dpgp_model_pack(int D, const double *fhat, const double *scal, double *pack, void *stream) {
    if (D <= 0) return -1;
    if (!fhat) return -2;
    if (!scal) return -3;
    if (!pack) return -4;
    DPGP_PRELAUNCH(); hipLaunchKernelGGL(model_pack_kernel, dim3(1), dim3(64), 0, (hipStream_t)stream, fhat, scal,
                       dpgp_ceil_div(D, PREP_ROWS), pack);
    DPGP_LAUNCH_CHECK();
    return DPGP_OK;
}

extern "C" int dpgp_model_finalize(const double *pack, const double *kl, const double *hyper, double *out,
                                   void *stream) {
    if (!pack) return -1;
    if (!kl) return -2;
    if (!hyper) return -3;
    if (!out) return -4;
    DPGP_PRELAUNCH(); hipLaunchKernelGGL(model_finalize_kernel, dim3(1), dim3(64), 0, (hipStream_t)stream, pack, pack + 1, kl, hyper, out);
    DPGP_LAUNCH_CHECK();
    return DPGP_OK;
}

extern "C" const char *dpgp_last_hip_error(void) { return hipGetErrorString(dpgp_last_error_slot()); }
```

dp_gp_lvm_amd/csrc/elementwise.hip:

```cpp
#include <cstdlib>
#include "internal.h"
#include "psi2_consts.h"

#define GRAM_T 64
template <typename T> __device__ __forceinline__ float gram_pair_factor(float al2, T acc) {
    if constexpr (sizeof(T) == 8) {
        double x = (-0.25 * DPGP_LOG2E) * acc;
        x = x < -300.0 ? -300.0 : x;
        const double n = rint(x);
        return ldexpf(al2 * __builtin_amdgcn_exp2f((float)(x - n)), (int)n);
    } else {
        return al2 * exp2f((float)(-0.25 * DPGP_LOG2E) * acc);
    }
}
template <typename TIN, typename T, bool FRONT = false>
__device__ __forceinline__ void gram_tile(int b, int i0, int j0, int N0, int N1, int Q, const TIN *__restrict__ x0,
                                          const TIN *__restrict__ x1, const TIN *__restrict__ gamma,
                                          const TIN *__restrict__ alpha, const TIN *__restrict__ beta, int flags, T jitter,
                                          T *__restrict__ out, int ld_out, size_t batch_stride, int symmetric,
                                          unsigned char *smem_raw, float *__restrict__ pair_fac = nullptr, size_t fac_stride = 0) {
    typedef T vec4 __attribute__((ext_vector_type(4)));
    T *xs = reinterpret_cast<T *>(smem_raw);
    T *zs = xs + GRAM_T * Q;
    const double *etab = nullptr;
    if constexpr (sizeof(T) == 8) {
        double *et = reinterpret_cast<double *>(zs + GRAM_T * Q);
        dpgp_exp2_tab_init(et);
        etab = et;
    }
    const int t = threadIdx.x;
    const TIN *g = gamma + (size_t)b * Q;
    {
        const int r = t & 63;
        const bool in0 = i0 + r < N0, in1 = j0 + r < N1;
        for (int q = t >> 6; q < Q; q += 4) {
            const T sg = sqrt((T)g[q]);
            xs[q * GRAM_T + r] = in0 ? sg * (T)x0[(size_t)(i0 + r) * Q + q] : (T)0;
            zs[q * GRAM_T + r] = in1 ? sg * (T)x1[(size_t)(j0 + r) * Q + q] : (T)0;
        }
    }
    __syncthreads();
    const int ty = t >> 4, tx = t & 15;
    T acc[4][4];
#pragma unroll
    for (int r = 0; r < 4; ++r)
#pragma unroll
        for (int c = 0; c < 4; ++c) acc[r][c] = 0;
    for (int q = 0; q < Q; ++q) {
        const vec4 a = *reinterpret_cast<const vec4 *>(xs + q * GRAM_T + ty * 4);
        const vec4 c_ = *reinterpret_cast<const vec4 *>(zs + q * GRAM_T + tx * 4);
#pragma unroll
        for (int r = 0; r < 4; ++r)
#pragma unroll
            for (int c = 0; c < 4; ++c) {
                T d = a[r] - c_[c];
                acc[r][c] = fma(d, d, acc[r][c]);
            }
    }
    const T al = (T)alpha[b];
    const bool add_noise = (symmetric & 1) && (flags & DPGP_FLAG_NOISE), add_jitter = (symmetric & 1) && (flags & DPGP_FLAG_JITTER);
    const T noise = add_noise ? (T)1 / (T)beta[b] : (T)0;
    const T scale = (T)(-0.5 * DPGP_LOG2E);
    T *ob = out + (size_t)b * batch_stride;
    T vt[FRONT ? 4 : 1][4];
#pragma unroll
    for (int r = 0; r < 4; ++r) {
        int i = i0 + ty * 4 + r;
        if (i >= N0) continue;
        T v[4];
#pragma unroll
        for (int c = 0; c < 4; ++c) {
            int j = j0 + tx * 4 + c;
            v[c] = al * dpgp_exp2_hot(scale * acc[r][c], etab);
            if (i == j) {
                if (add_noise) v[c] += noise;
                if (add_jitter) v[c] += jitter;
            }
            if constexpr (FRONT) vt[r][c] = v[c];
        }
        int j = j0 + tx * 4;
        if constexpr (FRONT) {
            if (pair_fac != nullptr && j <= i) {
                const float al2 = (float)(al * al);
                typedef float fvec4u __attribute__((ext_vector_type(4), aligned(4)));
                fvec4u f;
#pragma unroll
                for (int c = 0; c < 4; ++c) f[c] = gram_pair_factor<T>(al2, acc[r][c]);
                float *pf = pair_fac + (size_t)b * fac_stride + (size_t)i * (i + 1) / 2 + j;
                if (j + 3 <= i) {
                    *reinterpret_cast<fvec4u *>(pf) = f;
                } else {
#pragma unroll
                    for (int c = 0; c < 4; ++c)
                        if (j + c <= i) pf[c] = f[c];
                }
            }
        }
        T *p = ob + (size_t)i * ld_out + j;
        if (j + 3 < N1 && ((ld_out & 3) == 0)) {
            vec4 vv = {v[0], v[1], v[2], v[3]};
            if (symmetric & 2) __builtin_nontemporal_store(vv, reinterpret_cast<vec4 *>(p));
            else *reinterpret_cast<vec4 *>(p) = vv;
        } else {
#pragma unroll
            for (int c = 0; c < 4; ++c)
                if (j + c < N1) p[c] = v[c];
        }
    }
    if constexpr (FRONT) {
        if (i0 != j0) {
            const int i = i0 + ty * 4;
#pragma unroll
            for (int c = 0; c < 4; ++c) {
                const int j = j0 + tx * 4 + c;
                if (j >= N1 || i >= N0) continue;
                T *p = ob + (size_t)j * ld_out + i;
                if (i + 3 < N0 && ((ld_out & 3) == 0)) {
                    vec4 vv = {vt[0][c], vt[1][c], vt[2][c], vt[3][c]};
                    *reinterpret_cast<vec4 *>(p) = vv;
                } else {
#pragma unroll
                    for (int r = 0; r < 4; ++r)
                        if (i + r < N0) p[r] = vt[r][c];
                }
            }
        }
    }
}
template <typename TIN, typename T>
__global__ __launch_bounds__(256) void gram_kernel(int N0, int N1, int Q, const TIN *__restrict__ x0,
                                                   const TIN *__restrict__ x1, const TIN *__restrict__ gamma,
                                                   const TIN *__restrict__ alpha, const TIN *__restrict__ beta,
                                                   int flags, T jitter, T *__restrict__ out, int ld_out,
                                                   size_t batch_stride, int symmetric) {
    extern __shared__ __align__(16) unsigned char smem_raw[];
    gram_tile<TIN, T>(blockIdx.z, blockIdx.y * GRAM_T, blockIdx.x * GRAM_T, N0, N1, Q, x0, x1, gamma, alpha, beta, flags, jitter,
                      out, ld_out, batch_stride, symmetric, smem_raw);
}

template <typename TIN, typename T>
int launch_gram(int B, int N0, int N1, int Q, const TIN *x0, const TIN *x1, const TIN *gamma, const TIN *alpha,
                const TIN *beta, int flags, double jitter, T *out, int ld_out, size_t batch_stride, hipStream_t st) {
    int sym = (x1 == nullptr) ? 1 : 0;
    if (sym) { x1 = x0; N1 = N0; }
    const char *nt_ = getenv("DPGP_GRAM_NT");
    if (nt_ ? nt_[0] == '1' : (size_t)B * N0 * N1 * sizeof(T) > ((size_t)256 << 20)) sym |= 2;
    dim3 grid(dpgp_ceil_div(N1, GRAM_T), dpgp_ceil_div(N0, GRAM_T), B);
    size_t lds = sizeof(T) * 2 * GRAM_T * Q + (sizeof(T) == 8 ? sizeof(double) * DPGP_EXP2_TAB_ELEMS : 0);
    DPGP_PRELAUNCH(); hipLaunchKernelGGL((gram_kernel<TIN, T>), grid, dim3(256), lds, st, N0, N1, Q, x0, x1, gamma, alpha, beta, flags,
                       (T)jitter, out, ld_out, batch_stride, sym);
    DPGP_LAUNCH_CHECK();
    return DPGP_OK;
}
template int launch_gram<float, float>(int, int, int, int, const float *, const float *, const float *, const float *,
                                       const float *, int, double, float *, int, size_t, hipStream_t);
template int launch_gram<double, double>(int, int, int, int, const double *, const double *, const double *,
                                         const double *, const double *, int, double, double *, int, size_t,
                                         hipStream_t);
template int launch_gram<double, float>(int, int, int, int, const double *, const double *, const double *,
                                        const double *, const double *, int, double, float *, int, size_t,
                                        hipStream_t);

template <typename T>
__global__ void diag_kernel(int B, int N, const T *alpha, const T *beta, int flags, T jitter, T *out) {
    size_t i = (size_t)blockIdx.x * blockDim.x + threadIdx.x;
    if (i >= (size_t)B * N) return;
    int b = (int)(i / N);
    T v = alpha[b];
    if (flags & DPGP_FLAG_NOISE) v += (T)1 / beta[b];
    if (flags & DPGP_FLAG_JITTER) v += jitter;
    out[i] = v;
}
template <typename T> __global__ void psi0_kernel(int B, int N, const T *alpha, T *out) {
    int b = blockIdx.x * blockDim.x + threadIdx.x;
    if (b < B) out[b] = alpha[b] * (T)N;
}

#define PSI1_NT 32
template <typename T>
__global__ __launch_bounds__(256) void psi1_kernel(int N, int M, int Q, const T *__restrict__ z,
                                                   const T *__restrict__ mu, const T *__restrict__ s,
                                                   const T *__restrict__ gamma, const T *__restrict__ alpha,
                                                   T *__restrict__ out) {
    extern __shared__ __align__(16) unsigned char smem_raw[];
    T *w = reinterpret_cast<T *>(smem_raw);
    T *mus = w + PSI1_NT * Q;
    T *cn = mus + PSI1_NT * Q;
    T *zs = cn + PSI1_NT;
    const int b = blockIdx.y, n0 = blockIdx.x * PSI1_NT, t = threadIdx.x;
    const T *g = gamma + (size_t)b * Q;
    for (int e = t; e < PSI1_NT * Q; e += 256) {
        int r = e / Q, q = e - r * Q, n = n0 + r;
        T sv = n < N ? s[(size_t)n * Q + q] : (T)1, mv = n < N ? mu[(size_t)n * Q + q] : (T)0;
        T den = g[q] * sv + (T)1;
        w[e] = g[q] / den;
        mus[e] = mv;
    }
    if (t < PSI1_NT) {
        int n = n0 + t;
        T a = 0;
        for (int q = 0; q < Q; ++q) a += dpgp_log(g[q] * (n < N ? s[(size_t)n * Q + q] : (T)1) + (T)1);
        cn[t] = (T)(-0.5 * DPGP_LOG2E) * a;
    }
    const T al = alpha[b];
    const int r = t >> 3, c8 = t & 7;
    const int n = n0 + r;
    for (int m0 = 0; m0 < M; m0 += 64) {
        __syncthreads();
        for (int e = t; e < 64 * Q; e += 256) {
            int rr = e / Q, q = e - rr * Q;
            zs[rr * (Q + 1) + q] = (m0 + rr < M) ? z[(size_t)(m0 + rr) * Q + q] : (T)0;
        }
        __syncthreads();
#pragma unroll
        for (int h = 0; h < 2; ++h) {
            int mb = (h * 8 + c8) * 4;
            T acc[4] = {0, 0, 0, 0};
            for (int q = 0; q < Q; ++q) {
                T wq = w[r * Q + q], mq = mus[r * Q + q];
#pragma unroll
                for (int c = 0; c < 4; ++c) {
                    T d = mq - zs[(mb + c) * (Q + 1) + q];
                    acc[c] = fma(wq * d, d, acc[c]);
                }
            }
            if (n < N) {
                T *p = out + ((size_t)b * N + n) * M + m0 + mb;
                T v[4];
#pragma unroll
                for (int c = 0; c < 4; ++c) v[c] = al * dpgp_exp2((T)(-0.5 * DPGP_LOG2E) * acc[c] + cn[r]);
                if (m0 + mb + 3 < M && ((M & 3) == 0)) {
                    typedef T vec4 __attribute__((ext_vector_type(4)));
                    vec4 vv = {v[0], v[1], v[2], v[3]};
                    *reinterpret_cast<vec4 *>(p) = vv;
                } else {
#pragma unroll
                    for (int c = 0; c < 4; ++c)
                        if (m0 + mb + c < M) p[c] = v[c];
                }
            }
        }
    }
}

#define P1Y_NT 32
template <typename TIN, typename T>
__global__ __launch_bounds__(256) void psi1T_y_kernel(int N, int M, int Q, int B, const TIN *__restrict__ z,
                                                      const TIN *__restrict__ mu, const TIN *__restrict__ s,
                                                      const TIN *__restrict__ gamma, const TIN *__restrict__ alpha,
                                                      const TIN *__restrict__ y, int ldy, double *__restrict__ part,
                                                      int n_per_split) {
    __shared__ T w[P1Y_NT][DPGP_MAX_Q + 2];
    __shared__ T mus[P1Y_NT][DPGP_MAX_Q + 2];
    __shared__ T lg[P1Y_NT][DPGP_MAX_Q + 2];
    __shared__ T cn[P1Y_NT], yn[P1Y_NT];
    __shared__ double red[4][128];
    __shared__ double etab[DPGP_EXP2_TAB_ELEMS];
    if (sizeof(T) == 8) dpgp_exp2_tab_init(etab);
    const int b = blockIdx.z, mc = blockIdx.y * 128, sp = blockIdx.x;
    const int t = threadIdx.x, lane = t & 63, wv = t >> 6;
    const TIN *g = gamma + (size_t)b * Q;
    T zr[2][DPGP_MAX_Q];
#pragma unroll
    for (int h = 0; h < 2; ++h) {
        int m = mc + lane + 64 * h;
#pragma unroll
        for (int q = 0; q < DPGP_MAX_Q; ++q) zr[h][q] = (q < Q && m < M) ? (T)z[(size_t)m * Q + q] : (T)0;
    }
    double acc[2] = {0.0, 0.0};
    const int nbeg = sp * n_per_split, nend = min(N, nbeg + n_per_split);
    for (int n0 = nbeg; n0 < nend; n0 += P1Y_NT) {
        __syncthreads();
        for (int e = t; e < P1Y_NT * Q; e += 256) {
            int r = e / Q, q = e - r * Q, n = n0 + r;
            bool ok = n < nend;
            T sv = ok ? (T)s[(size_t)n * Q + q] : (T)1;
            T den = (T)g[q] * sv + (T)1;
            w[r][q] = (T)(-0.5 * DPGP_LOG2E) * (T)g[q] / den;
            mus[r][q] = ok ? (T)mu[(size_t)n * Q + q] : (T)0;
            lg[r][q] = dpgp_log(den);
        }
        __syncthreads();
        if (t < P1Y_NT) {
            int n = n0 + t;
            bool ok = n < nend;
            T a = 0;
            for (int q = 0; q < Q; ++q) a += lg[t][q];
            cn[t] = (T)(-0.5 * DPGP_LOG2E) * a;
            yn[t] = ok ? (T)y[(size_t)n * ldy + b] : (T)0;
        }
        __syncthreads();
        T tacc[2] = {0, 0};
        for (int r = wv; r < P1Y_NT; r += 4) {
            T e0 = cn[r], e1 = cn[r];
#pragma unroll
            for (int q = 0; q < DPGP_MAX_Q; ++q) {
                if (q < Q) {
                    T wq = w[r][q], mq = mus[r][q];
                    T d0 = mq - zr[0][q], d1 = mq - zr[1][q];
                    e0 = fma(wq * d0, d0, e0);
                    e1 = fma(wq * d1, d1, e1);
                }
            }
            tacc[0] = fma(yn[r], dpgp_exp2_hot(e0, etab), tacc[0]);
            tacc[1] = fma(yn[r], dpgp_exp2_hot(e1, etab), tacc[1]);
        }
        acc[0] += (double)tacc[0];
        acc[1] += (double)tacc[1];
    }
    __syncthreads();
    red[wv][lane] = acc[0];
    red[wv][lane + 64] = acc[1];
    __syncthreads();
    if (t < 128 && mc + t < M) {
        double v = red[0][t] + red[1][t] + red[2][t] + red[3][t];
        part[((size_t)sp * B + b) * M + mc + t] = (double)alpha[b] * v;
    }
}

typedef _Float16 p1_h8 __attribute__((ext_vector_type(8)));
typedef _Float16 p1_h2 __attribute__((ext_vector_type(2)));
typedef float p1_f4 __attribute__((ext_vector_type(4)));

template <typename TIN, int KF1, int NJ>
__global__ __launch_bounds__(256) void psi1T_y_f16_kernel(int N, int M, int Q, int B, const TIN *__restrict__ z,
                                                          const unsigned char *__restrict__ consts,
                                                          const TIN *__restrict__ mu, const TIN *__restrict__ s,
                                                          const TIN *__restrict__ gamma,
                                                          const TIN *__restrict__ alpha, const TIN *__restrict__ y,
                                                          int ldy, double *__restrict__ part, int n_per_split) {
    constexpr int SL = 32 * KF1;
    constexpr int QP = 4 * ((32 * KF1 - 2) / 6 / 4 + 1);
    constexpr int QPC = QP < 32 ? QP : 32;
    __shared__ __align__(16) _Float16 bimg[16 * NJ * SL];
    __shared__ __align__(16) _Float16 aimg[4][16 * SL];
    __shared__ float yv[4][16];
    __shared__ float zc[32], gq[32];
    __shared__ __align__(16) float red[16][128];
    const int b = blockIdx.z, mc = blockIdx.y * (16 * NJ), sp = blockIdx.x;
    const int t = threadIdx.x, lane = t & 63, wv = t >> 6, li = lane & 15, kk = lane >> 4;
    const Psi2Consts C = psi2_consts_layout(M, Q);
    const _Float16 *bimg_g = reinterpret_cast<const _Float16 *>(consts + C.off_bimg);
    if (t < 32) {
        gq[t] = (t < Q) ? (float)gamma[(size_t)b * Q + t] : 0.0f;
        zc[t] = reinterpret_cast<const float *>(consts)[t];
    }
    typedef unsigned p1_u4 __attribute__((ext_vector_type(4)));
    for (int e = t; e < 16 * NJ * (SL / 8); e += 256) {
        const int m = e / (SL / 8), k = e - m * (SL / 8);
        p1_u4 v = {0u, 0u, 0u, 0u};
        if (mc + m < C.Mp64) v = reinterpret_cast<const p1_u4 *>(bimg_g + (size_t)(mc + m) * SL)[k];
        reinterpret_cast<p1_u4 *>(bimg)[e] = v;
    }
    for (int e = t; e < 4 * 16 * SL / 2; e += 256) reinterpret_cast<unsigned *>(&aimg[0][0])[e] = 0u;
    __syncthreads();
    p1_h8 bop[NJ][KF1];
#pragma unroll
    for (int J = 0; J < NJ; ++J)
#pragma unroll
        for (int ks = 0; ks < KF1; ++ks)
            bop[J][ks] = *reinterpret_cast<const p1_h8 *>(bimg + (16 * J + li) * SL + 32 * ks + 8 * kk);
    float acc[NJ];
#pragma unroll
    for (int J = 0; J < NJ; ++J) acc[J] = 0.0f;
    _Float16 *am = &aimg[wv][0];
    const int nbeg = sp * n_per_split, nend = min(N, nbeg + n_per_split);
    constexpr int NPF = (16 * QPC + 63) / 64;
    float *cq = &red[wv * 4][0];
    TIN pf_s[NPF], pf_m[NPF], pf_y = (TIN)0;
    auto prefetch = [&](int n0) {
#pragma unroll
        for (int u = 0; u < NPF; ++u) {
            const int e = 64 * u + lane, r = e / QPC, q = e - r * QPC, n = n0 + r;
            const bool ok = (e < 16 * QPC) && (q < Q) && (n < nend);
            pf_s[u] = ok ? s[(size_t)n * Q + q] : (TIN)1;
            pf_m[u] = ok ? mu[(size_t)n * Q + q] : (TIN)0;
        }
        pf_y = (lane < 16 && n0 + lane < nend) ? y[(size_t)(n0 + lane) * ldy + b] : (TIN)0;
    };
    prefetch(nbeg + 16 * wv);
    bool oor = false;
    for (int n0 = nbeg + 16 * wv; n0 < nend; n0 += 64) {
#pragma unroll
        for (int u = 0; u < NPF; ++u) {
            const int e = 64 * u + lane;
            if (e < 16 * QPC) {
                const int r = e / QPC, q = e - r * QPC, n = n0 + r;
                float a = 0.0f, bb = 0.0f, cc = 0.0f;
                if (q < Q) {
                    if (n < nend) {
                        const float g = gq[q], den = g * (float)pf_s[u] + 1.0f;
                        const float w1 = g * __builtin_amdgcn_rcpf(den), mcq = (float)pf_m[u] - zc[q];
                        a = (float)(-0.5 * DPGP_LOG2E) * w1;
                        bb = (float)DPGP_LOG2E * w1 * mcq;
                        cc = w1 * mcq * mcq + 0.6931471805599453f * __builtin_amdgcn_logf(den);
                    }
                    a = dpgp_pin(a);
                    bb = dpgp_pin(bb);
                    const _Float16 ah = (_Float16)a, al = (_Float16)(a - (float)ah);
                    const _Float16 bh = (_Float16)bb, bl = (_Float16)(bb - (float)bh);
                    unsigned *dst = reinterpret_cast<unsigned *>(am + r * SL + 6 * q);
                    const p1_h2 w0 = {ah, ah}, w1_ = {al, bh}, w2 = {bh, bl};
                    dst[0] = __builtin_bit_cast(unsigned, w0);
                    dst[1] = __builtin_bit_cast(unsigned, w1_);
                    dst[2] = __builtin_bit_cast(unsigned, w2);
                }
                cq[e] = cc;
            }
        }
        const float yn = (float)pf_y;
        prefetch(n0 + 64);
        __builtin_amdgcn_fence(__ATOMIC_RELEASE, "wavefront");
        __builtin_amdgcn_s_waitcnt(0xc07f);
        __builtin_amdgcn_fence(__ATOMIC_ACQUIRE, "wavefront");
        if (lane < 16) {
            float c = 0.0f;
#pragma unroll
            for (int q4 = 0; q4 < QPC / 4; ++q4) {
                const p1_f4 v = *reinterpret_cast<const p1_f4 *>(cq + lane * QPC + 4 * q4);
                c += (v[0] + v[1]) + (v[2] + v[3]);
            }
            c = (float)(-0.5 * DPGP_LOG2E) * c;
            oor |= !(c >= -60000.0f);
            c = fmaxf(c, -60000.0f);
            c = dpgp_pin(c);
            const _Float16 ch = (_Float16)c;
            const p1_h2 cw = {ch, (_Float16)(c - (float)ch)};
            *reinterpret_cast<unsigned *>(am + lane * SL + 6 * Q) = __builtin_bit_cast(unsigned, cw);
            yv[wv][lane] = yn;
        }
        __builtin_amdgcn_fence(__ATOMIC_RELEASE, "wavefront");
        __builtin_amdgcn_s_waitcnt(0xc07f);
        __builtin_amdgcn_fence(__ATOMIC_ACQUIRE, "wavefront");
        p1_h8 aop[KF1];
#pragma unroll
        for (int ks = 0; ks < KF1; ++ks) aop[ks] = *reinterpret_cast<const p1_h8 *>(am + li * SL + 32 * ks + 8 * kk);
        float y4[4];
#pragma unroll
        for (int v = 0; v < 4; ++v) y4[v] = yv[wv][4 * kk + v];
        p1_f4 c[NJ];
#pragma unroll
        for (int J = 0; J < NJ; ++J) c[J] = (p1_f4){0, 0, 0, 0};
#pragma unroll
        for (int ks = 0; ks < KF1; ++ks)
#pragma unroll
            for (int J = 0; J < NJ; ++J) c[J] = __builtin_amdgcn_mfma_f32_16x16x32_f16(aop[ks], bop[J][ks], c[J], 0, 0, 0);
#pragma unroll
        for (int J = 0; J < NJ; ++J)
#pragma unroll
            for (int v = 0; v < 4; ++v) acc[J] = fmaf(y4[v], dpgp_exp2(c[J][v]), acc[J]);
        __builtin_amdgcn_fence(__ATOMIC_ACQ_REL, "wavefront");
    }
    const bool any_oor = __syncthreads_or(oor ? 1 : 0) != 0;
#pragma unroll
    for (int J = 0; J < NJ; ++J) red[wv * 4 + kk][16 * J + li] = acc[J];
    __syncthreads();
    if (t < 16 * NJ && mc + t < M) {
        double v = 0.0;
#pragma unroll
        for (int k = 0; k < 16; ++k) v += (double)red[k][t];
        part[((size_t)sp * B + b) * M + mc + t] = any_oor ? (double)__builtin_nanf("") : (double)alpha[b] * v;
    }
}

template <typename TIN, int KF1>
static int launch_psi1T_y_f16_kf(int B, int N, int M, int Q, const TIN *z, const TIN *mu, const TIN *s,
                                 const TIN *gamma, const TIN *alpha, const TIN *y, int ldy, double *part, int ns,
                                 const unsigned char *consts, hipStream_t st) {
    int nper = dpgp_round_up(dpgp_ceil_div(N, ns), 64);
    if (M <= 64) {
        dim3 grid(ns, 1, B);
        DPGP_PRELAUNCH(); hipLaunchKernelGGL((psi1T_y_f16_kernel<TIN, KF1, 4>), grid, dim3(256), 0, st, N, M, Q, B, z, consts, mu, s, gamma,
                           alpha, y, ldy, part, nper);
        DPGP_LAUNCH_CHECK();
        return DPGP_OK;
    }
    dim3 grid(ns, dpgp_ceil_div(M, 128), B);
    DPGP_PRELAUNCH(); hipLaunchKernelGGL((psi1T_y_f16_kernel<TIN, KF1, 8>), grid, dim3(256), 0, st, N, M, Q, B, z, consts, mu, s, gamma, alpha, y,
                       ldy, part, nper);
    DPGP_LAUNCH_CHECK();
    return DPGP_OK;
}

int psi1T_y_nsplit(int B, int N, int M) {
    if (const char *e = getenv("DPGP_PSI1_NS")) {
        const int v = atoi(e);
        if (v >= 1 && v <= 64 && v <= dpgp_ceil_div(N, 4 * P1Y_NT)) return v;
    }
    int wgs = B * dpgp_ceil_div(M, 128);
    int ns = dpgp_ceil_div(512, wgs);
    int max_ns = dpgp_ceil_div(N, 4 * P1Y_NT);
    if (ns > max_ns) ns = max_ns;
    return ns < 1 ? 1 : ns;
}

template <typename TIN, typename T>
int launch_psi1T_y_partial(int B, int N, int M, int Q, const TIN *z, const TIN *mu, const TIN *s, const TIN *gamma,
                           const TIN *alpha, const TIN *y, int ldy, double *part, int ns, unsigned char *consts,
                           int consts_ready, hipStream_t st) {
    if (sizeof(T) == 4) {
        if (!consts) return -18;
        if (!consts_ready) {
            int rc = launch_psi2_consts<TIN>(z, M, Q, consts, st);
            if (rc) return rc;
        }
        switch (dpgp_ceil_div(6 * Q + 2, 32)) {
#define CASE(k) \
    case k: return launch_psi1T_y_f16_kf<TIN, k>(B, N, M, Q, z, mu, s, gamma, alpha, y, ldy, part, ns, consts, st);
            CASE(1) CASE(2) CASE(3) CASE(4) CASE(5) CASE(6)
#undef CASE
        }
        return -4;
    }
    int nper = dpgp_round_up(dpgp_ceil_div(N, ns), P1Y_NT);
    dim3 grid(ns, dpgp_ceil_div(M, 128), B);
    DPGP_PRELAUNCH(); hipLaunchKernelGGL((psi1T_y_kernel<TIN, T>), grid, dim3(256), 0, st, N, M, Q, B, z, mu, s, gamma, alpha, y, ldy,
                       part, nper);
    DPGP_LAUNCH_CHECK();
    return DPGP_OK;
}
template int launch_psi1T_y_partial<float, float>(int, int, int, int, const float *, const float *, const float *,
                                                  const float *, const float *, const float *, int, double *, int,
                                                  unsigned char *, int, hipStream_t);
template int launch_psi1T_y_partial<double, double>(int, int, int, int, const double *, const double *, const double *,
                                                    const double *, const double *, const double *, int, double *, int,
                                                    unsigned char *, int, hipStream_t);
template int launch_psi1T_y_partial<double, float>(int, int, int, int, const double *, const double *, const double *,
                                                   const double *, const double *, const double *, int, double *, int,
                                                   unsigned char *, int, hipStream_t);

template <typename T>
__global__ void sum_slabs_kernel(size_t n, int ns, const double *__restrict__ part, T *__restrict__ out) {
    size_t i = (size_t)blockIdx.x * blockDim.x + threadIdx.x;
    if (i >= n) return;
    double a = 0;
    for (int k = 0; k < ns; ++k) a += part[(size_t)k * n + i];
    out[i] = (T)a;
}

#define YY_NCH DPGP_YY_NCH
template <typename TIN>
__device__ __forceinline__ void kl_yy_block(int blk, int N, int Q, const TIN *__restrict__ mu, const TIN *__restrict__ s,
                                            double *__restrict__ kl_out, int D, const TIN *__restrict__ y, int ldy,
                                            double *__restrict__ yy_out, const TIN *__restrict__ z, int M,
                                            unsigned char *__restrict__ consts, int first_consts_block,
                                            double (*scratch)[64]) {
    const int t = threadIdx.x;
    if (blk >= first_consts_block) {
        const int cb = blk - first_consts_block, nrow = (M + 63) / 64;
        if (cb < nrow) psi2_consts_rows(z, M, Q, consts, cb, &scratch[0][0]);
        else psi2_pair_rows(z, M, Q, consts, cb - nrow, &scratch[0][0]);
        return;
    }
    if (blk < DPGP_KL_NBLK) {
        if (kl_out == nullptr) return;
        double a0 = 0.0;
        const size_t tot = (size_t)N * Q;
        for (size_t i = (size_t)blk * 256 + t; i < tot; i += (size_t)DPGP_KL_NBLK * 256) {
            const double m0 = (double)mu[i], v0 = (double)s[i];
            a0 += m0 * m0 + v0 - log(v0) - 1.0;
        }
        const double a = block_sum(a0, &scratch[0][0]);
        if (t == 0) kl_out[blk] = 0.5 * a;
        if (t == 0 && blk == 0) *reinterpret_cast<int *>(kl_out + DPGP_KL_NBLK) = 0;
        return;
    }
    const int bid = blk - DPGP_KL_NBLK, dblk = bid / YY_NCH, ch = bid - dblk * YY_NCH;
    const int d = dblk * 64 + (t & 63), wv = t >> 6;
    const int nper = (N + YY_NCH - 1) / YY_NCH, n0 = ch * nper, n1 = min(N, n0 + nper);
    double a0 = 0.0, a1 = 0.0;
    if (d < D) {
        int n = n0 + wv;
        for (; n + 4 < n1; n += 8) {
            const double v0 = (double)y[(size_t)n * ldy + d], v1 = (double)y[(size_t)(n + 4) * ldy + d];
            a0 += v0 * v0;
            a1 += v1 * v1;
        }
        for (; n < n1; n += 4) {
            const double v0 = (double)y[(size_t)n * ldy + d];
            a0 += v0 * v0;
        }
    }
    scratch[wv][t & 63] = a0 + a1;
    __syncthreads();
    if (t < 64 && d < D) yy_out[(size_t)ch * D + d] = scratch[0][t] + scratch[1][t] + scratch[2][t] + scratch[3][t];
}
template <typename TIN>
__global__ __launch_bounds__(256) void kl_yy_kernel(int N, int Q, const TIN *__restrict__ mu,
                                                    const TIN *__restrict__ s, double *__restrict__ kl_out, int D,
                                                    const TIN *__restrict__ y, int ldy, double *__restrict__ yy_out,
                                                    const TIN *__restrict__ z, int M, unsigned char *__restrict__ consts,
                                                    int first_consts_block) {
    __shared__ double scratch[5][64];
    kl_yy_block<TIN>((int)blockIdx.x, N, Q, mu, s, kl_out, D, y, ldy, yy_out, z, M, consts, first_consts_block, scratch);
}
template <typename TL>
__global__ __launch_bounds__(256) void elbo_front_kernel(int N, int Q, const double *__restrict__ mu,
                                                         const double *__restrict__ s, double *__restrict__ kl_out, int D,
                                                         const double *__restrict__ y, int ldy, double *__restrict__ yy_out,
                                                         const double *__restrict__ z, int M, unsigned char *__restrict__ consts,
                                                         int first_consts_block, int first_gram_block,
                                                         const double *__restrict__ gamma, const double *__restrict__ alpha,
                                                         const double *__restrict__ beta, TL jitter, TL *__restrict__ kuu,
                                                         int ld_kuu, size_t kuu_stride, int first_scale_block,
                                                         float *__restrict__ pair_scale, float *__restrict__ pair_fac) {
    __shared__ double scratch[5][64];
    extern __shared__ __align__(16) unsigned char smem_raw[];
    const int blk = (int)blockIdx.x;
#ifdef FRONT_DIAG_SKIP
    if ((FRONT_DIAG_SKIP & 1) && blk < first_gram_block) return;
#endif
    if (blk < first_gram_block) {
        kl_yy_block<double>(blk, N, Q, mu, s, kl_out, D, y, ldy, yy_out, z, M, consts, first_consts_block, scratch);
        return;
    }
    const int ng = first_scale_block - first_gram_block, nsb = (int)gridDim.x - first_scale_block;
    int g = blk - first_gram_block;
    if (nsb > 0) {
        const long long T = (long long)ng + nsb;
        const int c0 = (int)((long long)g * nsb / T), c1 = (int)((long long)(g + 1) * nsb / T);
        if (c1 > c0) {
#ifdef FRONT_DIAG_SKIP
            if (FRONT_DIAG_SKIP & 4) return;
#endif
            const int nb = (psi2_consts_layout(M, Q).Ppad + 255) / 256, sb = c0;
            const int dch = psi2_scale_dchunk(D), b0 = (sb / nb) * dch;
            psi2_pair_scale_chunk<double, double>(b0, min(dch, D - b0), sb % nb, M, Q, z, gamma, alpha, pair_scale,
                                                  reinterpret_cast<float *>(smem_raw));
            return;
        }
        g -= c0;
    }
#ifdef FRONT_DIAG_SKIP
    if (FRONT_DIAG_SKIP & 2) return;
#endif
    const int tm = (M + GRAM_T - 1) / GRAM_T, tl = tm * (tm + 1) / 2, b = g / tl, r = g - b * tl;
    int ti = 0;
    while ((ti + 1) * (ti + 2) / 2 <= r) ++ti;
    const int tj = r - ti * (ti + 1) / 2;
    gram_tile<double, TL, true>(b, ti * GRAM_T, tj * GRAM_T, M, M, Q, z, z, gamma, alpha, beta, DPGP_FLAG_JITTER, jitter, kuu,
                                ld_kuu, kuu_stride, 1, smem_raw, pair_fac, (size_t)psi2_consts_layout(M, Q).Ppad);
}
template <typename TL>
int launch_elbo_front(int N, int Q, const double *mu, const double *s, double *kl_out, int D, const double *y, int ldy,
                      double *yy_out, const double *z, int M, unsigned char *psi2_consts, const double *gamma,
                      const double *alpha, const double *beta, double jitter, TL *kuu, int ld_kuu, size_t kuu_stride,
                      float *pair_scale, float *pair_fac, hipStream_t st) {
    int blocks = DPGP_KL_NBLK + dpgp_ceil_div(D, 64) * YY_NCH;
    const int first_consts = blocks;
    blocks += dpgp_ceil_div(M, 64) + dpgp_ceil_div(psi2_consts_layout(M, Q).Ppad, PSI2_PAIR_ROWS_PER_BLOCK);
    const int first_gram = blocks, tm = dpgp_ceil_div(M, GRAM_T);
    blocks += D * (tm * (tm + 1) / 2);
    const int first_scale = blocks;
    if (pair_scale) blocks += dpgp_ceil_div(D, psi2_scale_dchunk(D)) * dpgp_ceil_div(psi2_consts_layout(M, Q).Ppad, 256);
    const size_t lds = sizeof(TL) * 2 * GRAM_T * (Q + 1);
    DPGP_PRELAUNCH(); hipLaunchKernelGGL((elbo_front_kernel<TL>), dim3(blocks), dim3(256), lds, st, N, Q, mu, s, kl_out, D, y, ldy, yy_out,
                       z, M, psi2_consts, first_consts, first_gram, gamma, alpha, beta, (TL)jitter, kuu, ld_kuu, kuu_stride,
                       first_scale, pair_scale, pair_fac);
    DPGP_LAUNCH_CHECK();
    return DPGP_OK;
}
template int launch_elbo_front<float>(int, int, const double *, const double *, double *, int, const double *, int, double *,
                                      const double *, int, unsigned char *, const double *, const double *, const double *,
                                      double, float *, int, size_t, float *, float *, hipStream_t);
template int launch_elbo_front<double>(int, int, const double *, const double *, double *, int, const double *, int, double *,
                                       const double *, int, unsigned char *, const double *, const double *, const double *,
                                       double, double *, int, size_t, float *, float *, hipStream_t);

template <typename TIN>
int launch_kl_yy(int N, int Q, const TIN *mu, const TIN *s, double *kl_out, int D, const TIN *y, int ldy,
                 double *yy_out, const TIN *z, int M, unsigned char *psi2_consts, hipStream_t st) {
    int blocks = DPGP_KL_NBLK;
    if (yy_out) {
        blocks += dpgp_ceil_div(D, 64) * YY_NCH;
    }
    const int first_consts = blocks;
    if (psi2_consts) blocks += dpgp_ceil_div(M, 64) + dpgp_ceil_div(psi2_consts_layout(M, Q).Ppad, PSI2_PAIR_ROWS_PER_BLOCK);
    DPGP_PRELAUNCH(); hipLaunchKernelGGL((kl_yy_kernel<TIN>), dim3(blocks), dim3(256), 0, st, N, Q, mu, s, kl_out, D, y, ldy, yy_out, z, M,
                       psi2_consts, first_consts);
    DPGP_LAUNCH_CHECK();
    return DPGP_OK;
}
template int launch_kl_yy<float>(int, int, const float *, const float *, double *, int, const float *, int, double *,
                                 const float *, int, unsigned char *, hipStream_t);
template int launch_kl_yy<double>(int, int, const double *, const double *, double *, int, const double *, int,
                                  double *, const double *, int, unsigned char *, hipStream_t);

#define CHECK_ARG(cond, idx) \
    do {                     \
        if (!(cond)) return -(idx); \
    } while (0)

template <typename T>
static int gram_api(int B, int N0, int N1, int Q, const T *x0, const T *x1, const T *gamma, const T *alpha,
                    const T *beta, int flags, double jitter, T *out, void *stream) {
    CHECK_ARG(B > 0, 1); CHECK_ARG(N0 > 0, 2); CHECK_ARG(x1 == nullptr || N1 > 0, 3);
    CHECK_ARG(Q > 0 && Q <= DPGP_MAX_Q, 4); CHECK_ARG(x0, 5); CHECK_ARG(gamma, 7); CHECK_ARG(alpha, 8);
    CHECK_ARG(beta || !(flags & DPGP_FLAG_NOISE), 9); CHECK_ARG(out, 12);
    int n1 = x1 ? N1 : N0;
    return launch_gram<T, T>(B, N0, n1, Q, x0, x1, gamma, alpha, beta, flags, jitter, out, n1, (size_t)N0 * n1,
                             (hipStream_t)stream);
}
extern "C" int dpgp_ard_rbf_gram_f32(int B, int N0, int N1, int Q, const float *x0, const float *x1, const float *gamma,
                                     const float *alpha, const float *beta, int flags, double jitter, float *out,
                                     void *stream) {
    return gram_api<float>(B, N0, N1, Q, x0, x1, gamma, alpha, beta, flags, jitter, out, stream);
}
extern "C" int dpgp_ard_rbf_gram_f64(int B, int N0, int N1, int Q, const double *x0, const double *x1,
                                     const double *gamma, const double *alpha, const double *beta, int flags,
                                     double jitter, double *out, void *stream) {
    return gram_api<double>(B, N0, N1, Q, x0, x1, gamma, alpha, beta, flags, jitter, out, stream);
}

template <typename T>
static int diag_api(int B, int N, const T *alpha, const T *beta, int flags, double jitter, T *out, void *stream) {
    CHECK_ARG(B > 0, 1); CHECK_ARG(N > 0, 2); CHECK_ARG(alpha, 3); CHECK_ARG(beta || !(flags & DPGP_FLAG_NOISE), 4);
    CHECK_ARG(out, 7);
    size_t tot = (size_t)B * N;
    DPGP_PRELAUNCH(); hipLaunchKernelGGL((diag_kernel<T>), dim3((unsigned)((tot + 255) / 256)), dim3(256), 0, (hipStream_t)stream, B, N,
                       alpha, beta, flags, (T)jitter, out);
    DPGP_LAUNCH_CHECK();
    return DPGP_OK;
}
extern "C" int dpgp_ard_rbf_diag_f32(int B, int N, const float *alpha, const float *beta, int flags, double jitter,
                                     float *out, void *stream) {
    return diag_api<float>(B, N, alpha, beta, flags, jitter, out, stream);
}
extern "C" int dpgp_ard_rbf_diag_f64(int B, int N, const double *alpha, const double *beta, int flags, double jitter,
                                     double *out, void *stream) {
    return diag_api<double>(B, N, alpha, beta, flags, jitter, out, stream);
}

template <typename T> static int psi0_api(int B, int N, const T *alpha, T *out, void *stream) {
    CHECK_ARG(B > 0, 1); CHECK_ARG(N > 0, 2); CHECK_ARG(alpha, 3); CHECK_ARG(out, 4);
    DPGP_PRELAUNCH(); hipLaunchKernelGGL((psi0_kernel<T>), dim3((B + 255) / 256), dim3(256), 0, (hipStream_t)stream, B, N, alpha, out);
    DPGP_LAUNCH_CHECK();
    return DPGP_OK;
}
extern "C" int dpgp_psi0_f32(int B, int N, const float *alpha, float *out, void *stream) {
    return psi0_api<float>(B, N, alpha, out, stream);
}
extern "C" int dpgp_psi0_f64(int B, int N, const double *alpha, double *out, void *stream) {
    return psi0_api<double>(B, N, alpha, out, stream);
}

template <typename T>
static int psi1_api(int B, int N, int M, int Q, const T *z, const T *mu, const T *s, const T *gamma, const T *alpha,
                    T *out, void *stream) {
    CHECK_ARG(B > 0, 1); CHECK_ARG(N > 0, 2); CHECK_ARG(M > 0, 3); CHECK_ARG(Q > 0 && Q <= DPGP_MAX_Q, 4);
    CHECK_ARG(z, 5); CHECK_ARG(mu, 6); CHECK_ARG(s, 7); CHECK_ARG(gamma, 8); CHECK_ARG(alpha, 9); CHECK_ARG(out, 10);
    size_t lds = sizeof(T) * (2 * PSI1_NT * Q + PSI1_NT + 64 * (Q + 1));
    DPGP_PRELAUNCH(); hipLaunchKernelGGL((psi1_kernel<T>), dim3(dpgp_ceil_div(N, PSI1_NT), B), dim3(256), lds, (hipStream_t)stream, N, M,
                       Q, z, mu, s, gamma, alpha, out);
    DPGP_LAUNCH_CHECK();
    return DPGP_OK;
}
extern "C" int dpgp_psi1_f32(int B, int N, int M, int Q, const float *z, const float *mu, const float *s,
                             const float *gamma, const float *alpha, float *out, void *stream) {
    return psi1_api<float>(B, N, M, Q, z, mu, s, gamma, alpha, out, stream);
}
extern "C" int dpgp_psi1_f64(int B, int N, int M, int Q, const double *z, const double *mu, const double *s,
                             const double *gamma, const double *alpha, double *out, void *stream) {
    return psi1_api<double>(B, N, M, Q, z, mu, s, gamma, alpha, out, stream);
}

extern "C" size_t dpgp_psi1T_y_workspace_bytes(int B, int N, int M) {
    if (B <= 0 || N <= 0 || M <= 0) return 0;
    return dpgp_align256(sizeof(double) * (size_t)psi1T_y_nsplit(B, N, M) * B * M) + psi2_consts_bytes(M, DPGP_MAX_Q);
}
template <typename T>
static int psi1T_y_api(int B, int N, int M, int Q, const T *z, const T *mu, const T *s, const T *gamma, const T *alpha,
                       const T *y, int ldy, T *out, void *ws, size_t ws_bytes, void *stream) {
    CHECK_ARG(B > 0, 1); CHECK_ARG(N > 0, 2); CHECK_ARG(M > 0, 3); CHECK_ARG(Q > 0 && Q <= DPGP_MAX_Q, 4);
    CHECK_ARG(z, 5); CHECK_ARG(mu, 6); CHECK_ARG(s, 7); CHECK_ARG(gamma, 8); CHECK_ARG(alpha, 9); CHECK_ARG(y, 10);
    CHECK_ARG(ldy >= B, 11); CHECK_ARG(out, 12); CHECK_ARG(ws, 13);
    CHECK_ARG(ws_bytes >= dpgp_psi1T_y_workspace_bytes(B, N, M), 14);
    int ns = psi1T_y_nsplit(B, N, M);
    unsigned char *consts = (unsigned char *)ws + dpgp_align256(sizeof(double) * (size_t)ns * B * M);
    int rc = launch_psi1T_y_partial<T, T>(B, N, M, Q, z, mu, s, gamma, alpha, y, ldy, (double *)ws, ns, consts, 0,
                                          (hipStream_t)stream);
    if (rc) return rc;
    size_t tot = (size_t)B * M;
    DPGP_PRELAUNCH(); hipLaunchKernelGGL((sum_slabs_kernel<T>), dim3((unsigned)((tot + 255) / 256)), dim3(256), 0, (hipStream_t)stream,
                       tot, ns, (const double *)ws, out);
    DPGP_LAUNCH_CHECK();
    return DPGP_OK;
}
extern "C" int dpgp_psi1T_y_f32(int B, int N, int M, int Q, const float *z, const float *mu, const float *s,
                                const float *gamma, const float *alpha, const float *y, int ldy, float *out, void *ws,
                                size_t ws_bytes, void *stream) {
    return psi1T_y_api<float>(B, N, M, Q, z, mu, s, gamma, alpha, y, ldy, out, ws, ws_bytes, stream);
}
extern "C" int dpgp_psi1T_y_f64(int B, int N, int M, int Q, const double *z, const double *mu, const double *s,
                                const double *gamma, const double *alpha, const double *y, int ldy, double *out,
                                void *ws, size_t ws_bytes, void *stream) {
    return psi1T_y_api<double>(B, N, M, Q, z, mu, s, gamma, alpha, y, ldy, out, ws, ws_bytes, stream);
}

__global__ void kl_single_block_kernel(int N, int Q, const float *muf, const float *sf, const double *mud,
                                       const double *sd, double *out) {
    __shared__ double scratch[8];
    double a = 0.0;
    const size_t tot = (size_t)N * Q;
    for (size_t i = threadIdx.x; i < tot; i += 256) {
        const double m0 = muf ? (double)muf[i] : mud[i], v0 = sf ? (double)sf[i] : sd[i];
        a += m0 * m0 + v0 - log(v0) - 1.0;
    }
    a = block_sum(a, scratch);
    if (threadIdx.x == 0) out[0] = 0.5 * a;
}
static int kl_api_launch(int N, int Q, const float *muf, const float *sf, const double *mud, const double *sd,
                         double *out, void *stream) {
    CHECK_ARG(N > 0, 1); CHECK_ARG(Q > 0, 2); CHECK_ARG(muf || mud, 3); CHECK_ARG(sf || sd, 4); CHECK_ARG(out, 5);
    DPGP_PRELAUNCH(); hipLaunchKernelGGL(kl_single_block_kernel, dim3(1), dim3(256), 0, (hipStream_t)stream, N, Q, muf, sf, mud, sd, out);
    DPGP_LAUNCH_CHECK();
    return DPGP_OK;
}
extern "C" int dpgp_kl_qx_f32(int N, int Q, const float *mu, const float *s, double *out, void *stream) {
    return kl_api_launch(N, Q, mu, s, nullptr, nullptr, out, stream);
}
extern "C" int dpgp_kl_qx_f64(int N, int Q, const double *mu, const double *s, double *out, void *stream) {
    return kl_api_launch(N, Q, nullptr, nullptr, mu, s, out, stream);
}
extern "C" int dpgp_version(void) { return 200; }
```

dp_gp_lvm_amd/csrc/internal.h:

```cpp
#pragma once
#include "common.h"

static inline int dpgp_env_plan(const char *name, int lo, int hi) {
    const char *e = getenv(name);
    if (!e) return 0;
    const int v = atoi(e);
    return v < lo ? 0 : (v > hi ? hi : v);
}

static inline int dpgp_set_dyn_lds(const void *fn, size_t lds) {
    if (lds > 48 * 1024 && hipFuncSetAttribute(fn, hipFuncAttributeMaxDynamicSharedMemorySize, (int)lds) != hipSuccess)
        return DPGP_ERR_LAUNCH;
    return DPGP_OK;
}

struct DpgpSlabSplit { int outer_slabs, outer_per_slab, pair_slabs, tiles_per_slab; };
static inline DpgpSlabSplit dpgp_slab_split(long base, int target, int n_outer, int tiles, const char *env_outer,
                                            const char *env_pair) {
    DpgpSlabSplit p;
    long os = (target + base - 1) / base;
    if (const int v = dpgp_env_plan(env_outer, 1, n_outer)) os = v;
    os = os < 1 ? 1 : (os > n_outer ? n_outer : os);
    p.outer_per_slab = (n_outer + (int)os - 1) / (int)os;
    p.outer_slabs = (n_outer + p.outer_per_slab - 1) / p.outer_per_slab;
    long ps = (target + base * p.outer_slabs - 1) / (base * p.outer_slabs);
    if (const int v = dpgp_env_plan(env_pair, 1, tiles)) ps = v;
    ps = ps < 1 ? 1 : (ps > tiles ? tiles : ps);
    p.tiles_per_slab = (tiles + (int)ps - 1) / (int)ps;
    p.pair_slabs = (tiles + p.tiles_per_slab - 1) / p.tiles_per_slab;
    return p;
}

int launch_point_adjoint_slab_sum(size_t nq, int slabs, const double *part, double *d_mu, double *d_s, hipStream_t st);

template <typename TIN, typename T>
int launch_gram(int B, int N0, int N1, int Q, const TIN *x0, const TIN *x1, const TIN *gamma, const TIN *alpha,
                const TIN *beta, int flags, double jitter, T *out, int ld_out, size_t batch_stride, hipStream_t st);

int psi1T_y_nsplit(int B, int N, int M);
template <typename TIN, typename T>
int launch_psi1T_y_partial(int B, int N, int M, int Q, const TIN *z, const TIN *mu, const TIN *s, const TIN *gamma,
                           const TIN *alpha, const TIN *y, int ldy, double *part, int ns, unsigned char *psi2_consts,
                           int consts_ready, hipStream_t st);

#define DPGP_YY_NCH 16
#define DPGP_KL_NBLK 16
template <typename TIN>
int launch_kl_yy(int N, int Q, const TIN *mu, const TIN *s, double *kl_out, int D, const TIN *y, int ldy,
                 double *yy_out, const TIN *z, int M, unsigned char *psi2_consts, hipStream_t st);
template <typename TL>
int launch_elbo_front(int N, int Q, const double *mu, const double *s, double *kl_out, int D, const double *y, int ldy,
                      double *yy_out, const double *z, int M, unsigned char *psi2_consts, const double *gamma,
                      const double *alpha, const double *beta, double jitter, TL *kuu, int ld_kuu, size_t kuu_stride,
                      float *pair_scale, float *pair_fac, hipStream_t st);

int psi2_nsplit(int B, int N, int M);
size_t psi2_consts_bytes(int M, int Q);
template <typename TIN> int launch_psi2_consts(const TIN *z, int M, int Q, unsigned char *consts, hipStream_t st);
template <typename TIN, typename T>
int launch_psi2_partial(int B, int N, int M, int Q, const TIN *z, const TIN *mu, const TIN *s, const TIN *gamma,
                        const TIN *alpha, T *part, int ns, int algo, hipStream_t st, void *chain_ws, int chain_elem,
                        double *logdet_k, int *info_k, unsigned char *consts, int consts_ready, float *pair_scale);
size_t psi2_pairs_scale_bytes(int B, int M);

size_t la_chain_ws_elems(int M);
bool la_chain_k_resident(int M, int elem);
template <typename TL>
int launch_chain_k(int D, int M, TL *ws, double *logdet_k, int *info_k, int algo, hipStream_t st);
template <typename TP, typename TL>
int launch_chain_b(int D, int N, int M, const TP *psi2_part, int ns2, const double *v_part, int ns1,
                   const double *alpha, const double *beta, const double *yy_part, const double *logdet_k,
                   const int *info_k, double *terms, int *info, double *guard, TL *ws, int algo, hipStream_t st,
                   const double *kl_part = nullptr, double *sums = nullptr, const double *model_scal = nullptr,
                   double *model_pack = nullptr, double *model_out = nullptr, TL *lb_out = nullptr);
int launch_sum_terms(int D, const double *terms, const double *kl_part, double *sums, const double *model_scal,
                     double *model_pack, double *model_out, hipStream_t st);
size_t potrf_big_ws_elems(int B, int M);
template <typename T> int launch_potrf_big(int B, int M, T *a, int *info, T *ws, hipStream_t st);
bool potrf_persist_applicable(int B, int M, int elem_size);
int launch_potrf_persist(int B, int Mw, double *w, int *info, hipStream_t st, size_t wstride = 0);
int launch_ptrsm_persist(int B, int Mw, const double *l, size_t lstride, double *x, size_t xstride, double *nrm2,
                         size_t nstride, hipStream_t st, int identity = 0);
int launch_tcols_quad(int T, int M, int D, const double *lb, const double *vp, int nsl, long long v_ss, const double *scale,
                      double *quad, hipStream_t st);
int launch_gemm_splitk_f64(int batch, int m, int n, int k, const double *a, long long a_sb, long long a_si, long long a_sk,
                           const double *b, long long b_sb, long long b_sk, long long b_sj, double *c, long long c_sb,
                           long long c_si, long long c_sj, int ksplit, long long c_ss, hipStream_t st);
bool chain_big_applicable(int D, int M, int elem);
size_t chain_big_ws_elems(int M);
int launch_chain_big_k(int D, int M, double *ws, int *info_k, hipStream_t st);
template <typename TP>
int launch_chain_big_b(int D, int N, int M, const TP *psi2_part, int ns2, const double *v_part, int ns1, const double *alpha,
                       const double *beta, const double *yy_part, const int *info_k, double *terms, int *info, double *guard,
                       double *ws, hipStream_t st, const double *kl_part, double *sums, const double *model_scal,
                       double *model_pack, double *model_out);
template <typename TP>
int launch_chain_grad(int D, int N, int M, const TP *psi2_part, int ns2, const double *v_part, int ns1, const double *alpha,
                      const double *beta, const double *yy_part, double jitter, double *ws, double *GP, double *WK,
                      double *Gv, double *dab, int *info, hipStream_t st);
size_t psi_grad_ws_bytes(int D, int N, int M, int Q, int *nsplit_out);
size_t psi_grad_ws_bytes_kuu(int D, int M, int Q);
template <typename TC>
int launch_psi_grad(int D, int N, int M, int Q, const double *y, int ldy, const double *z, const double *mu, const double *s,
                    const double *gamma, const double *alpha, const double *GP, const double *WK, const double *Gv,
                    double *ws, double *dmu, double *ds, double *dz, double *dgamma, int do_psi2, hipStream_t st,
                    const double *wts = nullptr);
size_t psi1_grad_ws_elems(int D, int N, int M, int Q);
int launch_psi1_grad(int D, int N, int M, int Q, const double *y, int ldy, const unsigned char *consts, const double *mu,
                     const double *s, const double *gamma, const double *alpha, const double *Gv, const double *G1,
                     double *ws, double *stage, double *dmu, double *ds, double *dz, double *dgamma, hipStream_t st);
int launch_kuu_grad(int D, int M, int Q, const unsigned char *consts, const double *gamma, const double *WK, double *ws,
                    double *stage, double *dz, double *dgamma, hipStream_t st);
size_t reduce_rows_stage_elems(size_t n);
template <typename TP>
int launch_reduce_rows(size_t n, size_t pitch, int nk, const TP *part, double *out, int accumulate, double *stage, hipStream_t st);
bool psi2_grad_supported(int M, int Q);
size_t psi2_grad_part_elems(int B, int N, int M, int Q);
int launch_psi2_grad(int B, int N, int M, int Q, const unsigned char *consts, const double *mu, const double *s,
                     const double *gamma, const double *alpha, const double *GP, double *part, double *stage, double *dmu,
                     double *ds, double *dz, double *dgamma, hipStream_t st);
#define DPGP_LB_TILE_ELEMS (16 * 17)
#define DPGP_PREP_ROWS 16

bool psi2_pgrad_supported(int M, int Q);
size_t psi2_pgrad_ws_bytes(int D, int N, int M, int Q);
bool chain_grad_big_supported(int M);
size_t chain_grad_big_ws_bytes(int D, int M);
template <typename TP>
int launch_chain_grad_big(int D, int N, int M, int Q, const double *z, const double *gamma, const double *alpha, const double *beta,
                          double jitter, const TP *psi2_part, int ns2, const double *v_part, int ns1, const double *yy_part,
                          unsigned char *ws, double *GP, double *WK, double *Gv, double *dab, int *info, hipStream_t st);
int launch_psi2_pgrad(int D, int N, int M, int Q, const unsigned char *consts, const double *z, const double *mu,
                      const double *s, const double *gamma, const double *alpha, const double *GP, unsigned char *ws,
                      double *stage, double *dmu, double *ds, double *dz, double *dgamma, hipStream_t st, int which = 3,
                      float *psi2_part = nullptr, const float *scale = nullptr, const double *y = nullptr, int ldy = 0,
                      const double *Gv = nullptr, int fast = 0, double *psi1v = nullptr);
```

dp_gp_lvm_amd/csrc/psi2_consts.h:

```cpp
#pragma once
#include "common.h"

struct Psi2Consts {
    int ZLD, SL, Mp64;
    size_t off_zs, off_bimg, bytes;
    int KS, SLP, P, Ppad;
    size_t off_pairs;
    size_t off_pmap;
};
__host__ __device__ inline int psi2_pairs_ksteps(int Q) {
    const int ks = (6 * Q + 2 + 15) / 16;
    return ks <= 2 ? 2 : (ks <= 4 ? 4 : (ks <= 6 ? 6 : (ks <= 8 ? 8 : 12)));
}
__host__ __device__ inline Psi2Consts psi2_consts_layout(int M, int Q) {
    Psi2Consts c;
    const int KQ = 4 * ((Q + 3) / 4);
    c.ZLD = ((KQ / 4) & 1) ? KQ : KQ + 4;
    c.SL = 32 * ((6 * Q + 2 + 31) / 32);
    c.Mp64 = (M + 63) & ~63;
    c.off_zs = 128;
    c.off_bimg = c.off_zs + sizeof(float) * (size_t)c.Mp64 * c.ZLD;
    c.off_pairs = (c.off_bimg + sizeof(_Float16) * (size_t)c.Mp64 * c.SL + 255) & ~(size_t)255;
    c.KS = psi2_pairs_ksteps(Q);
    c.SLP = 16 * c.KS;
    c.P = (int)((long long)M * (M + 1) / 2);
    c.Ppad = (c.P + 31) & ~31;
    c.off_pmap = (c.off_pairs + sizeof(_Float16) * (size_t)c.Ppad * c.SLP + 255) & ~(size_t)255;
    c.bytes = (c.off_pmap + sizeof(unsigned) * (size_t)c.Ppad + 255) & ~(size_t)255;
    return c;
}

template <typename TIN>
__device__ __forceinline__ void psi2_consts_rows(const TIN *__restrict__ z, int M, int Q, unsigned char *__restrict__ dst,
                                                 int blk, double *scratch) {
    const Psi2Consts c = psi2_consts_layout(M, Q);
    float *zc = reinterpret_cast<float *>(scratch + 8 * 32);
    block_column_means(z, M, Q, zc, scratch);
    const int t = threadIdx.x;
    if (blk == 0 && t < 32) reinterpret_cast<float *>(dst)[t] = (t < Q) ? zc[t] : 0.0f;
    float *zs = reinterpret_cast<float *>(dst + c.off_zs);
    _Float16 *bimg = reinterpret_cast<_Float16 *>(dst + c.off_bimg);
    const int m0 = 64 * blk;
    for (int e = t; e < 64 * c.ZLD; e += 256) {
        const int r = e / c.ZLD, k = e - r * c.ZLD, m = m0 + r;
        zs[(size_t)m * c.ZLD + k] = (k < Q && m < M) ? (float)z[(size_t)m * Q + k] - zc[k] : 0.0f;
    }
    for (int e = t; e < 64 * c.SL / 2; e += 256) {
        const int r = e / (c.SL / 2), w = e - r * (c.SL / 2), m = m0 + r;
        _Float16 h2[2];
#pragma unroll
        for (int i = 0; i < 2; ++i) {
            const int slot = 2 * w + i;
            float val = 0.0f;
            if (slot < 6 * Q) {
                const int tt = slot / 3, part = slot - 3 * tt, q = tt >> 1;
                const float zz = (m < M) ? (float)z[(size_t)m * Q + q] - zc[q] : 0.0f;
                const float v = dpgp_pin((tt & 1) ? zz : zz * zz);
                const _Float16 h = (_Float16)v;
                val = (part == 1) ? (float)(_Float16)(v - (float)h) : (float)h;
            } else if (slot < 6 * Q + 2) {
                val = 1.0f;
            }
            h2[i] = (_Float16)val;
        }
        typedef _Float16 h2v __attribute__((ext_vector_type(2)));
        const h2v hv = {h2[0], h2[1]};
        reinterpret_cast<unsigned *>(bimg)[(size_t)m * (c.SL / 2) + w] = __builtin_bit_cast(unsigned, hv);
    }
}

__host__ __device__ inline void psi2_pair_of(int p, int &m, int &mp) {
    int i = (int)((sqrtf(8.0f * (float)p + 1.0f) - 1.0f) * 0.5f);
    while ((long long)(i + 1) * (i + 2) / 2 <= p) ++i;
    while ((long long)i * (i + 1) / 2 > p) --i;
    m = i;
    mp = p - (int)((long long)i * (i + 1) / 2);
}
#define PSI2_PAIR_ROWS_PER_BLOCK 256
#define PSI2_PAIR_S2_SCALE 0.015625f
template <typename TIN>
__device__ __forceinline__ void psi2_pair_rows(const TIN *__restrict__ z, int M, int Q, unsigned char *__restrict__ dst,
                                               int blk, double *scratch) {
    const Psi2Consts c = psi2_consts_layout(M, Q);
    float *zc = reinterpret_cast<float *>(scratch + 8 * 32);
    block_column_means(z, M, Q, zc, scratch);
    const int t = threadIdx.x, wpr = c.SLP / 2;
    unsigned *img = reinterpret_cast<unsigned *>(dst + c.off_pairs);
    const int p0 = PSI2_PAIR_ROWS_PER_BLOCK * blk;
    if (p0 + t < c.Ppad) {
        const int p = p0 + t;
        int m = 0, mp = 0;
        if (p < c.P) psi2_pair_of(p, m, mp);
        reinterpret_cast<unsigned *>(dst + c.off_pmap)[p] = (p < c.P) ? ((unsigned)m << 16 | (unsigned)mp) : 0xffffffffu;
    }
    auto put = [&](int p, int w, unsigned word) {
        const int ks = w >> 3, hf = (w >> 2) & 1, wi = w & 3, lane = 32 * hf + (p & 31);
        img[(((size_t)(p >> 5) * c.KS + ks) * 64 + lane) * 4 + wi] = word;
    };
    typedef _Float16 h2v __attribute__((ext_vector_type(2)));
    for (int e = t; e < PSI2_PAIR_ROWS_PER_BLOCK * (Q + 1); e += 256) {
        const int r = e % PSI2_PAIR_ROWS_PER_BLOCK, q = e / PSI2_PAIR_ROWS_PER_BLOCK, p = p0 + r;
        if (p >= c.Ppad) continue;
        const bool real = p < c.P;
        if (q == Q) {
            const h2v one2 = {(_Float16)1.0f, (_Float16)1.0f}, one1 = {(_Float16)1.0f, (_Float16)0.0f};
            for (int w = 3 * Q; w < wpr; ++w) {
                unsigned word = 0u;
                if (real && w == 3 * Q) word = __builtin_bit_cast(unsigned, one2);
                if (real && w == 3 * Q + 1 && 6 * Q + 2 < c.SLP) word = __builtin_bit_cast(unsigned, one1);
                put(p, w, word);
            }
            continue;
        }
        unsigned w0 = 0u, w1 = 0u, w2 = 0u;
        if (real) {
            int m, mp;
            psi2_pair_of(p, m, mp);
            const float sq = ((float)z[(size_t)m * Q + q] - zc[q]) + ((float)z[(size_t)mp * Q + q] - zc[q]);
            const float f1 = dpgp_pin(sq * sq * PSI2_PAIR_S2_SCALE), f2 = dpgp_pin(sq);
            const _Float16 f1h = (_Float16)f1, f1l = (_Float16)(f1 - (float)f1h);
            const _Float16 f2h = (_Float16)f2, f2l = (_Float16)(f2 - (float)f2h);
            const h2v a = {f1h, f1l}, b = {f1h, f2h}, d = {f2l, f2h};
            w0 = __builtin_bit_cast(unsigned, a); w1 = __builtin_bit_cast(unsigned, b); w2 = __builtin_bit_cast(unsigned, d);
        }
        put(p, 3 * q, w0); put(p, 3 * q + 1, w1); put(p, 3 * q + 2, w2);
    }
}

__host__ __device__ inline int psi2_scale_dchunk(int D) {
    const int c = D / 32;
    return c < 1 ? 1 : (c > 16 ? 16 : c);
}
template <typename TIN, typename TG>
__device__ __forceinline__ void psi2_pair_scale_chunk(int b0, int nb, int pblk, int M, int Q, const TIN *__restrict__ z,
                                                      const TG *__restrict__ gamma, const TG *__restrict__ alpha,
                                                      float *__restrict__ scale, float *__restrict__ lds = nullptr) {
    const int P = (int)((long long)M * (M + 1) / 2), Ppad = (P + 31) & ~31;
    const int p = pblk * 256 + (int)threadIdx.x;
    if (lds) {
        for (int e = (int)threadIdx.x; e < nb * (Q + 1); e += 256) {
            const int bb = e / (Q + 1), q = e - bb * (Q + 1);
            const float al = (float)alpha[b0 + bb];
            lds[e] = q < Q ? (float)gamma[(size_t)(b0 + bb) * Q + q] : al * al;
        }
        __syncthreads();
    }
    if (p >= Ppad) return;
    float d2[DPGP_MAX_Q];
#pragma unroll
    for (int q = 0; q < DPGP_MAX_Q; ++q) d2[q] = 0.0f;
    if (p < P) {
        int m, mp;
        psi2_pair_of(p, m, mp);
#pragma unroll
        for (int q = 0; q < DPGP_MAX_Q; ++q)
            if (q < Q) {
                const float d = (float)((double)z[(size_t)m * Q + q] - (double)z[(size_t)mp * Q + q]);
                d2[q] = d * d;
            }
    }
    for (int b = b0; b < b0 + nb; ++b) {
        float bsum = 0.0f, al2;
        if (lds) {
            const float *gl = lds + (b - b0) * (Q + 1);
#pragma unroll
            for (int q = 0; q < DPGP_MAX_Q; ++q)
                if (q < Q) bsum += gl[q] * d2[q];
            al2 = gl[Q];
        } else {
#pragma unroll
            for (int q = 0; q < DPGP_MAX_Q; ++q)
                if (q < Q) bsum += (float)gamma[(size_t)b * Q + q] * d2[q];
            const float al = (float)alpha[b];
            al2 = al * al;
        }
        scale[(size_t)b * Ppad + p] = al2 * __builtin_amdgcn_exp2f((float)(-0.25 * DPGP_LOG2E) * bsum);
    }
}
template <typename TIN, typename TG>
__device__ __forceinline__ void psi2_pair_scale_block(int b, int pblk, int M, int Q, const TIN *__restrict__ z,
                                                      const TG *__restrict__ gamma, const TG *__restrict__ alpha,
                                                      float *__restrict__ scale) {
    psi2_pair_scale_chunk<TIN, TG>(b, 1, pblk, M, Q, z, gamma, alpha, scale);
}
```

include/dpgp.h:

```cpp
#ifndef DPGP_H
#define DPGP_H
#include <stddef.h>
#ifdef __cplusplus
extern "C" {
#endif

#define DPGP_OK 0
#define DPGP_ERR_LAUNCH (-100)
#define DPGP_FLAG_NOISE 1
#define DPGP_FLAG_JITTER 2
#define DPGP_MAX_Q 30

#define DPGP_ALGO_AUTO 0
#define DPGP_ALGO_PLAIN 1
#define DPGP_ALGO_MFMA_F32 2
#define DPGP_ALGO_PATCH_F16 3

#define DPGP_PREC_F32 0
#define DPGP_PREC_MIXED 1
#define DPGP_PREC_F64 2
#define DPGP_PREC_MIXED_FAST 4
#define DPGP_PREC_MIXED_PATCH 3

#define DPGP_INFO_ILL_CONDITIONED (-2)
#define DPGP_GUARD_REL 2.0e-3

int dpgp_version(void);
const char *dpgp_last_hip_error(void);

int dpgp_ard_rbf_gram_f32(int B, int N0, int N1, int Q, const float *x0, const float *x1, const float *gamma,
                          const float *alpha, const float *beta, int flags, double jitter, float *out, void *stream);
int dpgp_ard_rbf_gram_f64(int B, int N0, int N1, int Q, const double *x0, const double *x1, const double *gamma,
                          const double *alpha, const double *beta, int flags, double jitter, double *out, void *stream);

#define DPGP_GRAM_GRAD_MAX_Q 64
size_t dpgp_ard_rbf_gram_grad_workspace_bytes(int N, int Q);
int dpgp_ard_rbf_gram_grad_f64(int N, int Q, const double *x, const double *gamma, const double *alpha, const double *w, int ldw,
                               double *r, double *sx, double *sq, void *ws, size_t ws_bytes, void *stream);
size_t dpgp_ard_rbf_gram_grad_batched_workspace_bytes(int B, int N, int Q);
int dpgp_ard_rbf_gram_grad_batched_f64(int B, int N, int Q, const double *x, const double *gamma, const double *alpha,
                                       const double *w, int ldw, long long w_stride, double *r, double *sx, double *sq, void *ws,
                                       size_t ws_bytes, void *stream);

#define DPGP_QX_PSI_MAX_Q 64
size_t dpgp_qx_psi_stats_workspace_bytes(int B, int N, int M, int Q);
int dpgp_qx_psi_stats_batched_f64(int B, int N, int M, int Q, const double *z, const double *mu, const double *s,
                                  const double *gamma, const double *alpha, const double *zfac, double *psi1, double *psi2,
                                  void *ws, size_t ws_bytes, void *stream);
size_t dpgp_qx_psi_adjoint_workspace_bytes(int B, int N, int M, int Q);
int dpgp_qx_psi_adjoint_f64(int B, int N, int M, int Q, const double *z, const double *mu, const double *s, const double *gamma,
                            const double *alpha, const double *zfac, const double *g1, const double *g2, double *d_mu, double *d_s,
                            void *ws, size_t ws_bytes, void *stream);
int dpgp_qx_psi_stats_weighted_f64(int B, int N, int M, int Q, const double *z, const double *mu, const double *s,
                                   const double *gamma, const double *alpha, const double *zfac, const double *w, double *psi1,
                                   double *psi2, void *ws, size_t ws_bytes, void *stream);
int dpgp_qx_psi_adjoint_weighted_f64(int B, int N, int M, int Q, const double *z, const double *mu, const double *s,
                                     const double *gamma, const double *alpha, const double *zfac, const double *w,
                                     const double *g1, const double *g2, double *d_mu, double *d_s, void *ws, size_t ws_bytes,
                                     void *stream);
size_t dpgp_qx_psi_param_adjoint_workspace_bytes(int B, int N, int M, int Q);
int dpgp_qx_psi_param_adjoint_weighted_f64(int B, int N, int M, int Q, const double *z, const double *mu, const double *s,
                                           const double *gamma, const double *alpha, const double *zfac, const double *w,
                                           const double *g1, const double *g2, double *d_z, double *d_gamma, double *d_alpha,
                                           void *ws, size_t ws_bytes, void *stream);

size_t dpgp_qx_psi_stats_grouped_workspace_bytes(int K, int P, int N, int M, int Q);
int dpgp_qx_psi_stats_grouped_f64(int K, int P, int N, int M, int Q, const double *z, const double *mu, const double *s,
                                  const double *gamma, const double *alpha, const double *zfac, const double *w, double *psi1,
                                  double *psi2, void *ws, size_t ws_bytes, void *stream);
size_t dpgp_qx_psi_adjoint_grouped_workspace_bytes(int K, int P, int N, int M, int Q);
int dpgp_qx_psi_adjoint_grouped_f64(int K, int P, int N, int M, int Q, const double *z, const double *mu, const double *s,
                                    const double *gamma, const double *alpha, const double *zfac, const double *w,
                                    const double *g1, const double *g2, double *d_mu, double *d_s, void *ws, size_t ws_bytes,
                                    void *stream);
size_t dpgp_qx_psi_param_adjoint_grouped_workspace_bytes(int K, int P, int N, int M, int Q);
int dpgp_qx_psi_param_adjoint_grouped_f64(int K, int P, int N, int M, int Q, const double *z, const double *mu, const double *s,
                                          const double *gamma, const double *alpha, const double *zfac, const double *w,
                                          const double *g1, const double *g2, double *d_z, double *d_gamma, double *d_alpha,
                                          void *ws, size_t ws_bytes, void *stream);

size_t dpgp_qx_psi_pointwise_workspace_bytes(int K, int G, int J, int N, int M, int Q);
int dpgp_qx_psi_pointwise_f64(int K, int G, int J, int N, int M, int Q, const double *z, const double *mu, const double *s,
                              const double *gamma, const double *alpha, const double *zfac, const double *c, const double *r,
                              double *tr, double *quad, void *ws, size_t ws_bytes, void *stream);

size_t dpgp_qx_psi_point_moments_workspace_bytes(int K, int G, int J, int N, int M, int Q);
int dpgp_qx_psi_point_moments_f64(int K, int G, int J, int N, int M, int Q, const double *z, const double *mu, const double *s,
                                  const double *gamma, const double *alpha, const double *zfac, const double *c, const double *r,
                                  const int *gidx, const double *beta, double *mean, double *var, void *ws, size_t ws_bytes,
                                  void *stream);

size_t dpgp_qx_psi_pointwise_adjoint_workspace_bytes(int K, int G, int J, int N, int M, int Q);
int dpgp_qx_psi_pointwise_adjoint_f64(int K, int G, int J, int N, int M, int Q, const double *z, const double *mu, const double *s,
                                      const double *gamma, const double *alpha, const double *zfac, const double *c,
                                      const double *r, const double *h, const double *gq, const double *gt, double *d_mu,
                                      double *d_s, void *ws, size_t ws_bytes, void *stream);

size_t dpgp_ard_rbf_point_metric_workspace_bytes(int K, int N, int M, int Q);
int dpgp_ard_rbf_point_metric_f64(int K, int N, int M, int Q, const double *z, const double *x, const double *gamma,
                                  const double *alpha, const double *p, double *g, void *ws, size_t ws_bytes, void *stream);
size_t dpgp_ard_rbf_point_jacobian_workspace_bytes(int K, int J, int N, int M, int Q);
int dpgp_ard_rbf_point_jacobian_f64(int K, int J, int N, int M, int Q, const double *z, const double *x, const double *gamma,
                                    const double *alpha, const double *r, double *jac, void *ws, size_t ws_bytes, void *stream);

size_t dpgp_ard_rbf_point_energy_workspace_bytes(int K, int N, int M, int Q);
int dpgp_ard_rbf_point_energy_f64(int K, int N, int M, int Q, const double *z, const double *x, const double *v,
                                  const double *gamma, const double *alpha, const double *p, double *e, double *dx, double *dv,
                                  void *ws, size_t ws_bytes, void *stream);

size_t dpgp_ard_rbf_point_christoffel_workspace_bytes(int K, int N, int M, int Q);
int dpgp_ard_rbf_point_christoffel_f64(int K, int N, int M, int Q, const double *z, const double *x, const double *v,
                                       const double *gamma, const double *alpha, const double *p, double *g, double *gam,
                                       void *ws, size_t ws_bytes, void *stream);
int dpgp_geodesic_accel_f64(int K, int N, int Q, const double *g, const double *gam, const double *prior, const double *v,
                            double *a, double *speed, int *info, void *stream);

size_t dpgp_ard_rbf_point_christoffel_tangent_workspace_bytes(int K, int N, int M, int Q);
int dpgp_ard_rbf_point_christoffel_tangent_f64(int K, int N, int M, int Q, const double *z, const double *x, const double *v,
                                               const double *dx, const double *dv, const double *gamma, const double *alpha,
                                               const double *p, double *g, double *gam, double *dg, double *dgam, void *ws,
                                               size_t ws_bytes, void *stream);
int dpgp_geodesic_accel_tangent_f64(int K, int N, int Q, const double *g, const double *gam, const double *dg,
                                    const double *dgam, const double *prior, const double *v, double *a, double *da,
                                    double *speed, int *info, void *stream);

size_t dpgp_ard_rbf_point_transport_workspace_bytes(int K, int N, int M, int Q, int F);
int dpgp_ard_rbf_point_transport_f64(int K, int N, int M, int Q, int F, const double *z, const double *x, const double *v,
                                     const double *w, const double *gamma, const double *alpha, const double *p, double *g,
                                     double *gam, double *tgam, void *ws, size_t ws_bytes, void *stream);
int dpgp_geodesic_transport_f64(int K, int N, int Q, int F, const double *g, const double *gam, const double *tgam,
                                const double *prior, const double *v, double *a, double *dw, double *speed, int *info,
                                void *stream);

size_t dpgp_geodesic_shoot_workspace_bytes(int parts, const int *K, const int *M, int Q, int C, int tangent);
int dpgp_geodesic_shoot_f64(int parts, const int *K, const int *M, int Q, int C, int S, const double *const *z,
                            const double *const *gamma, const double *const *alpha, const double *const *p, const double *prior,
                            const double *x, const double *v, double *curve, double *vel, int *bad, void *ws, size_t ws_bytes,
                            void *stream);
int dpgp_geodesic_shoot_tangent_f64(int parts, const int *K, const int *M, int Q, int C, int S, const double *const *z,
                                    const double *const *gamma, const double *const *alpha, const double *const *p,
                                    const double *prior, const double *x, const double *v, const double *dx, const double *dv,
                                    double *curve, double *vel, double *dcurve, double *dvel, int *bad, double *speed0, void *ws,
                                    size_t ws_bytes, void *stream);

size_t dpgp_ard_rbf_point_cov_workspace_bytes(int K, int G, int N, int M, int Q);
int dpgp_ard_rbf_point_cov_f64(int K, int G, int N, int M, int Q, const double *z, const double *x, const double *gamma,
                               const double *alpha, const double *c, double *out, void *ws, size_t ws_bytes, void *stream);

size_t dpgp_psi_latent_adjoint_workspace_bytes(int B, int N, int M, int Q);
int dpgp_psi_latent_adjoint_f64(int B, int N, int M, int Q, const double *z, const double *mu, const double *s,
                                const double *gamma, const double *alpha, const double *y, int ldy, const double *w,
                                const double *g_v, const double *g_psi2, double *d_mu, double *d_s, void *ws, size_t ws_bytes,
                                void *stream);

int dpgp_ard_rbf_diag_f32(int B, int N, const float *alpha, const float *beta, int flags, double jitter, float *out,
                          void *stream);
int dpgp_ard_rbf_diag_f64(int B, int N, const double *alpha, const double *beta, int flags, double jitter, double *out,
                          void *stream);

int dpgp_psi0_f32(int B, int N, const float *alpha, float *out, void *stream);
int dpgp_psi0_f64(int B, int N, const double *alpha, double *out, void *stream);

int dpgp_psi1_f32(int B, int N, int M, int Q, const float *z, const float *mu, const float *s, const float *gamma,
                  const float *alpha, float *out, void *stream);
int dpgp_psi1_f64(int B, int N, int M, int Q, const double *z, const double *mu, const double *s, const double *gamma,
                  const double *alpha, double *out, void *stream);

size_t dpgp_psi1T_y_workspace_bytes(int B, int N, int M);
int dpgp_psi1T_y_f32(int B, int N, int M, int Q, const float *z, const float *mu, const float *s, const float *gamma,
                     const float *alpha, const float *y, int ldy, float *out, void *ws, size_t ws_bytes, void *stream);
int dpgp_psi1T_y_f64(int B, int N, int M, int Q, const double *z, const double *mu, const double *s,
                     const double *gamma, const double *alpha, const double *y, int ldy, double *out, void *ws,
                     size_t ws_bytes, void *stream);

size_t dpgp_psi2_workspace_bytes(int B, int N, int M, int Q, int elem_size);
int dpgp_psi2_f32(int B, int N, int M, int Q, const float *z, const float *mu, const float *s, const float *gamma,
                  const float *alpha, float *out, void *ws, size_t ws_bytes, int algo, void *stream);
int dpgp_psi2_f64(int B, int N, int M, int Q, const double *z, const double *mu, const double *s, const double *gamma,
                  const double *alpha, double *out, void *ws, size_t ws_bytes, int algo, void *stream);
int dpgp_psi2_weighted_f64(int B, int N, int M, int Q, const double *z, const double *mu, const double *s,
                           const double *gamma, const double *alpha, const double *w , double *out,
                           void *ws, size_t ws_bytes, int algo, void *stream);

size_t dpgp_potrf_workspace_bytes(int B, int M, int elem_size);
int dpgp_potrf_batched_f32(int B, int M, float *a, int *info, void *ws, size_t ws_bytes, int algo, void *stream);
int dpgp_potrf_batched_f64(int B, int M, double *a, int *info, void *ws, size_t ws_bytes, int algo, void *stream);

size_t dpgp_trsm_workspace_bytes(int B, int M, int K, int elem_size);
int dpgp_trsm_batched_f32(int B, int M, int K, const float *l, float *rhs, void *ws, size_t ws_bytes, int algo,
                          void *stream);
int dpgp_trsm_batched_f64(int B, int M, int K, const double *l, double *rhs, void *ws, size_t ws_bytes, int algo,
                          void *stream);
int dpgp_trtri_lower_batched_f64(int B, int M, const double *l, double *out, void *ws, size_t ws_bytes, void *stream);

int dpgp_gemm_strided_f64(int batch, int m, int n, int k, double alpha, const double *a, long long a_sb, long long a_si,
                          long long a_sk, const double *b, long long b_sb, long long b_sk, long long b_sj, double beta,
                          double *c, long long c_sb, long long c_si, long long c_sj, void *stream);

int dpgp_kl_qx_f32(int N, int Q, const float *mu, const float *s, double *out, void *stream);
int dpgp_kl_qx_f64(int N, int Q, const double *mu, const double *s, double *out, void *stream);

size_t dpgp_elbo_workspace_bytes(int D, int N, int M, int Q, int prec);
int dpgp_elbo_workspace_layout(int D, int N, int M, int Q, int prec, size_t *out);
int dpgp_elbo_workspace_front_layout(int D, int N, int M, int Q, int prec, size_t *out);
int dpgp_elbo_fhat(int D, int N, int M, int Q, const double *y, int ldy, const double *z, const double *mu,
                   const double *s, const double *gamma, const double *alpha, const double *beta, double jitter,
                   int prec, int algo, double *terms, double *sums, int *info, void *ws, size_t ws_bytes,
                   void *stream);
typedef struct dpgp_exec {
    void *ev_psi2_begin;
    void *ev_psi2_end;
    const double *model_scal;
    double *model_pack;
    double *model_out;
    void *stream_aux;
    void *ev_fork;
    void *ev_join;
} dpgp_exec_t;
int dpgp_elbo_fhat_ex(int D, int N, int M, int Q, const double *y, int ldy, const double *z, const double *mu,
                      const double *s, const double *gamma, const double *alpha, const double *beta, double jitter,
                      int prec, int algo, double *terms, double *sums, int *info, void *ws, size_t ws_bytes,
                      void *stream, const dpgp_exec_t *exec);
int dpgp_elbo_grad_chain(int D, int N, int M, int Q, const double *alpha, const double *beta, double jitter, int prec,
                         void *ws, size_t ws_bytes, double *g_psi2, double *w_kuu, double *g_v, double *d_alpha_beta,
                         int *info, void *stream);
int dpgp_elbo_grad_chain_ex(int D, int N, int M, int Q, const double *alpha, const double *beta, double jitter, int prec,
                            void *ws, size_t ws_bytes, int psi2_slabs, double *g_psi2, double *w_kuu, double *g_v,
                            double *d_alpha_beta, int *info, void *stream);
size_t dpgp_elbo_grad_chain_big_workspace_bytes(int D, int M);
int dpgp_elbo_grad_chain_big(int D, int N, int M, int Q, const double *z, const double *gamma, const double *alpha,
                             const double *beta, double jitter, int prec, void *fwd_ws, size_t fwd_ws_bytes, int psi2_slabs, void *ws,
                             size_t ws_bytes, double *g_psi2, double *w_kuu, double *g_v, double *d_alpha_beta, int *info,
                             void *stream);

size_t dpgp_elbo_grad_psi_workspace_bytes(int D, int N, int M, int Q);
size_t dpgp_elbo_grad_psi_workspace_bytes_ex(int D, int N, int M, int Q, int prec);
int dpgp_elbo_grad_psi(int D, int N, int M, int Q, const double *y, int ldy, const double *z, const double *mu,
                       const double *s, const double *gamma, const double *alpha, const double *g_psi2,
                       const double *w_kuu, const double *g_v, int prec, void *ws, size_t ws_bytes, double *d_mu,
                       double *d_s, double *d_z, double *d_gamma, void *stream);
int dpgp_elbo_grad_psi_weighted_f64(int D, int N, int M, int Q, const double *y, int ldy, const double *z, const double *mu,
                                    const double *s, const double *gamma, const double *alpha,
                                    const double *w , const double *g_psi2, const double *w_kuu,
                                    const double *g_v, void *ws, size_t ws_bytes, double *d_mu, double *d_s, double *d_z,
                                    double *d_gamma, void *stream);
int dpgp_elbo_grad_psi_ex(int D, int N, int M, int Q, const double *y, int ldy, const double *z, const double *mu,
                          const double *s, const double *gamma, const double *alpha, const double *g_psi2,
                          const double *w_kuu, const double *g_v, const double *g_psi1, int prec, void *ws,
                          size_t ws_bytes, double *d_mu, double *d_s, double *d_z, double *d_gamma, void *stream);

int dpgp_elbo_step(int D, int N, int M, int Q, const double *y, int ldy, const double *z, const double *mu, const double *s,
                   const double *gamma, const double *alpha, const double *beta, double jitter, int prec, double *terms, double *sums,
                   int *info, void *ws, size_t ws_bytes, double *g_psi2, double *w_kuu, double *g_v, double *d_alpha_beta,
                   int *info_grad, void *gws, size_t gws_bytes, double *d_mu, double *d_s, double *d_z, double *d_gamma,
                   void *stream, const dpgp_exec_t *exec);

int dpgp_elbo_fhat_step(int D, int N, int M, int Q, const double *y, int ldy, const double *z, const double *mu, const double *s,
                        const double *gamma, const double *alpha, const double *beta, double jitter, double *terms, double *sums,
                        int *info, void *ws, size_t ws_bytes, void *gws, size_t gws_bytes, void *stream, const dpgp_exec_t *exec);
int dpgp_elbo_grad_psi_step(int D, int N, int M, int Q, const double *y, int ldy, const double *z, const double *mu, const double *s,
                            const double *gamma, const double *alpha, const double *g_psi2, const double *w_kuu, const double *g_v,
                            int prec, void *ws, size_t ws_bytes, void *gws, size_t gws_bytes, double *d_mu, double *d_s, double *d_z,
                            double *d_gamma, void *stream);

size_t dpgp_elbo_fhat_t_workspace_bytes(int T, int D, int N, int M, int Q, int prec);
int dpgp_elbo_fhat_t(int T, int D, int N, int M, int Q, const double *y, int ldy, const double *yy, const double *z,
                     const double *mu, const double *s, const double *gamma, const double *alpha, const double *beta,
                     const double *phit, long long phi_st, long long phi_sd, double jitter, int prec, double *per_t,
                     double *quad, double *sums, int *info, void *ws, size_t ws_bytes, void *stream,
                     const double *model_scal, double *model_pack, double *model_out, void *stream_aux, void *ev_fork,
                     void *ev_join);

void *dpgp_event_create(void);
void dpgp_event_destroy(void *event);
void *dpgp_stream_create(void);
void dpgp_stream_destroy(void *stream);
float dpgp_event_elapsed_ms(void *begin, void *end);

int dpgp_model_scal_count(int D);
int dpgp_model_prepare(int D, int T, int Q, int N, int d_offset, int mask_size, const double *logits,
                       const double *gamma_atoms_raw, const double *alpha_atoms_raw, const double *beta_atoms_raw,
                       const double *s_raw, const double *g1_raw, const double *g2_raw, const double *w_raw, double s1,
                       double s2, int add_constants, double *gamma, double *alpha, double *beta, double *s, double *phi,
                       double *scal, void *stream);
int dpgp_model_prepare_t(int D, int T, int Q, int N, int d_offset, int mask_size, const double *logits,
                         const double *gamma_atoms_raw, const double *alpha_atoms_raw, const double *beta_atoms_raw,
                         const double *s_raw, const double *g1_raw, const double *g2_raw, const double *w_raw, double s1,
                         double s2, int add_constants, double *s, double *phi, double *atoms, double *scal, void *stream);
int dpgp_trouble_flag(size_t n, const double *flat, int d, const int *info, double *out, void *stream);
int dpgp_model_backward(int D, int T, int Q, int N, int M, int d_offset, int mask_size, int logits_rows,
                        const double *logits, const double *gamma_atoms_raw, const double *alpha_atoms_raw,
                        const double *beta_atoms_raw, const double *s_raw, const double *g1_raw, const double *g2_raw,
                        const double *w_raw, const double *x_mean, const double *phi, double s1, double s2,
                        int add_constants, const double *df_dmu, const double *df_ds, const double *df_dz,
                        const double *df_dgamma, const double *df_dalpha_beta, double *d_x_mean, double *d_s_raw,
                        double *d_x_u, double *d_logits, double *d_g1_raw, double *d_g2_raw, double *d_w_raw,
                        double *d_gamma_atoms_raw, double *d_alpha_atoms_raw, double *d_beta_atoms_raw, void *stream);
int dpgp_model_backward_t(int D, int T, int Q, int N, int M, int d_offset, int mask_size, int logits_rows, const double *logits,
                          const double *gamma_atoms_raw, const double *alpha_atoms_raw, const double *beta_atoms_raw,
                          const double *s_raw, const double *g1_raw, const double *g2_raw, const double *w_raw,
                          const double *x_mean, const double *phi, double s1, double s2, int add_constants, const double *df_dmu,
                          const double *df_ds, const double *df_dz, const double *df_dgamma_atoms,
                          const double *df_dalpha_beta_atoms, const double *df_dphi, double *d_x_mean, double *d_s_raw,
                          double *d_x_u, double *d_logits, double *d_g1_raw, double *d_g2_raw, double *d_w_raw,
                          double *d_gamma_atoms_raw, double *d_alpha_atoms_raw, double *d_beta_atoms_raw, void *stream);
int dpgp_model_pack(int D, const double *fhat, const double *scal, double *pack, void *stream);
int dpgp_model_finalize(const double *pack, const double *kl, const double *hyper, double *out, void *stream);

#ifdef __cplusplus
}
#endif
#endif
```

Baseline: 816.5.

## Fold Psi1^T y partial into the ELBO front kernel as an extra role

The Psi1^T·y partial-sum computation now runs as extra workgroups inside the fused ELBO front launch in the forward f16 path, and the aux-stream fork is disabled there. The kernel body is restructured to stage row chunks of A operands cooperatively in LDS, build the B image on the fly from z, and software-pipeline MFMA chains against exp/FMA work. This removes a separate launch, the precomputed constants dependency and stream fork/join overhead. In exchange the front kernel gets heavier and loses overlap with the aux stream.

```diff
diff --git a/dp_gp_lvm_amd/_lib.py b/dp_gp_lvm_amd/_lib.py
--- a/dp_gp_lvm_amd/_lib.py
+++ b/dp_gp_lvm_amd/_lib.py
@@ -15,6 +15,7 @@
     'dpgp_version': (_i, []),
     'dpgp_last_hip_error': (ctypes.c_char_p, []),
     'dpgp_psi1T_y_workspace_bytes': (_sz, [_i, _i, _i]),
+    'dpgp_psi1T_y_chunk_rows': (_i, [_i]),
     'dpgp_psi2_workspace_bytes': (_sz, [_i, _i, _i, _i, _i]),
     'dpgp_potrf_workspace_bytes': (_sz, [_i, _i, _i]),
     'dpgp_trsm_workspace_bytes': (_sz, [_i, _i, _i, _i]),
diff --git a/dp_gp_lvm_amd/csrc/elbo.hip b/dp_gp_lvm_amd/csrc/elbo.hip
--- a/dp_gp_lvm_amd/csrc/elbo.hip
+++ b/dp_gp_lvm_amd/csrc/elbo.hip
@@ -91,12 +91,18 @@
     const bool pairs_psi2 = (sizeof(TP) == 4 && algo == DPGP_ALGO_AUTO && psi2_pairs_ksteps(Q) <= 8);
     const bool fac_from_gram = pairs_psi2 && pgws == nullptr;
     float *pscale = reinterpret_cast<float *>(ws + L.off_sc);
+    const bool forward_f16 = pgws == nullptr && !psi1_from_pass && lb_out == nullptr && sizeof(TP) == 4;
+    bool p1_role = forward_f16 && psi1T_y_role_supported(Q);
+    if (p1_role)
+        if (const char *e = getenv("DPGP_PSI1_ROLE")) p1_role = atoi(e) != 0;
+    const Psi1TyRole role = {p1_role ? vpart : nullptr, L.ns1};
     if ((rc = launch_elbo_front<TL>(N, Q, mu, s, klp, D, y, ldy, yy, z, M, pconst, gamma, alpha, beta, jitter, la, L.Mp,
                                     la_chain_ws_elems(M), (pairs_psi2 && !fac_from_gram) ? pscale : nullptr,
-                                    fac_from_gram ? pscale : nullptr, st)))
+                                    fac_from_gram ? pscale : nullptr, &role, st)))
         return rc;
     hipStream_t aux = (ex && ex->stream_aux && ex->ev_fork && ex->ev_join) ? (hipStream_t)ex->stream_aux : nullptr;
     if (pgws != nullptr && psi1_from_pass && D > 256) aux = nullptr;
+    if (forward_f16) aux = nullptr;
     AuxJoin aj;
     if (aux) {
         if (hipEventRecord((hipEvent_t)ex->ev_fork, st) != hipSuccess || hipStreamWaitEvent(aux, (hipEvent_t)ex->ev_fork, 0) != hipSuccess)
@@ -104,8 +110,8 @@
         aj.arm(st, aux, (hipEvent_t)ex->ev_join);
     }
     const int ns1 = psi1_from_pass ? 1 : L.ns1;
-    if (!psi1_from_pass &&
-        (rc = launch_psi1T_y_partial<double, TP>(D, N, M, Q, z, mu, s, gamma, alpha, y, ldy, vpart, L.ns1, pconst, 1, aux ? aux : st)))
+    if (!psi1_from_pass && !p1_role &&
+        (rc = launch_psi1T_y_partial<double, TP>(D, N, M, Q, z, mu, s, gamma, alpha, y, ldy, vpart, L.ns1, aux ? aux : st)))
         return rc;
     const bool k_on_aux = aux && pgws != nullptr && la_chain_k_resident(M, (int)sizeof(TL)) && algo != DPGP_ALGO_PLAIN;
     if (k_on_aux && (rc = launch_chain_k<TL>(D, M, la, ldk, ik, algo, aux))) return rc;
diff --git a/dp_gp_lvm_amd/csrc/elementwise.hip b/dp_gp_lvm_amd/csrc/elementwise.hip
--- a/dp_gp_lvm_amd/csrc/elementwise.hip
+++ b/dp_gp_lvm_amd/csrc/elementwise.hip
@@ -321,104 +321,106 @@
 typedef _Float16 p1_h8 __attribute__((ext_vector_type(8)));
 typedef _Float16 p1_h2 __attribute__((ext_vector_type(2)));
 typedef float p1_f4 __attribute__((ext_vector_type(4)));
+typedef unsigned p1_u4 __attribute__((ext_vector_type(4)));
+
+__host__ __device__ constexpr int psi1T_y_chunk_rows_kf(int kf1) { return kf1 == 1 ? 256 : (kf1 == 2 ? 192 : (kf1 == 3 ? 128 : 64)); }
+template <int KF1> struct P1YChunk {
+    static constexpr int SL = 32 * KF1;
+    static constexpr int LD = SL + 8;
+    static constexpr int R = psi1T_y_chunk_rows_kf(KF1);
+    static constexpr int QP = 4 * ((SL - 2) / 6 / 4 + 1);
+    static constexpr int QPC = QP < 32 ? QP : 32;
+    static constexpr int off_y = R * LD * 2;
+    static constexpr int off_zc = off_y + R * 4, off_gq = off_zc + 128, bytes = off_gq + 128;
+    static constexpr int CLD = 40;
+    static_assert(bytes <= 32768, "LDS of a Psi1^T y workgroup");
+    static_assert(off_y >= 128 * CLD * 2 && off_y >= 8 * 32 * 8 && off_y >= 16 * 128 * 4, "staging areas inside the image region");
+};
+extern "C" int dpgp_psi1T_y_chunk_rows(int Q) {
+    return (Q > 0 && Q <= DPGP_MAX_Q) ? psi1T_y_chunk_rows_kf(dpgp_ceil_div(6 * Q + 2, 32)) : 0;
+}
 
 template <typename TIN, int KF1, int NJ>
-__global__ __launch_bounds__(256) void psi1T_y_f16_kernel(int N, int M, int Q, int B, const TIN *__restrict__ z,
-                                                          const unsigned char *__restrict__ consts,
-                                                          const TIN *__restrict__ mu, const TIN *__restrict__ s,
-                                                          const TIN *__restrict__ gamma,
-                                                          const TIN *__restrict__ alpha, const TIN *__restrict__ y,
-                                                          int ldy, double *__restrict__ part, int n_per_split) {
-    constexpr int SL = 32 * KF1;
-    constexpr int QP = 4 * ((32 * KF1 - 2) / 6 / 4 + 1);
-    constexpr int QPC = QP < 32 ? QP : 32;
-    __shared__ __align__(16) _Float16 bimg[16 * NJ * SL];
-    __shared__ __align__(16) _Float16 aimg[4][16 * SL];
-    __shared__ float yv[4][16];
-    __shared__ float zc[32], gq[32];
-    __shared__ __align__(16) float red[16][128];
-    const int b = blockIdx.z, mc = blockIdx.y * (16 * NJ), sp = blockIdx.x;
-    const int t = threadIdx.x, lane = t & 63, wv = t >> 6, li = lane & 15, kk = lane >> 4;
-    const Psi2Consts C = psi2_consts_layout(M, Q);
-    const _Float16 *bimg_g = reinterpret_cast<const _Float16 *>(consts + C.off_bimg);
-    if (t < 32) {
-        gq[t] = (t < Q) ? (float)gamma[(size_t)b * Q + t] : 0.0f;
-        zc[t] = reinterpret_cast<const float *>(consts)[t];
-    }
-    typedef unsigned p1_u4 __attribute__((ext_vector_type(4)));
-    for (int e = t; e < 16 * NJ * (SL / 8); e += 256) {
-        const int m = e / (SL / 8), k = e - m * (SL / 8);
-        p1_u4 v = {0u, 0u, 0u, 0u};
-        if (mc + m < C.Mp64) v = reinterpret_cast<const p1_u4 *>(bimg_g + (size_t)(mc + m) * SL)[k];
-        reinterpret_cast<p1_u4 *>(bimg)[e] = v;
-    }
-    for (int e = t; e < 4 * 16 * SL / 2; e += 256) reinterpret_cast<unsigned *>(&aimg[0][0])[e] = 0u;
-    __syncthreads();
+__device__ __forceinline__ void psi1T_y_chunk_body(int sp, int mc, int b, int N, int M, int Q, int B, const TIN *__restrict__ z,
+                                                   const TIN *__restrict__ mu, const TIN *__restrict__ s,
+                                                   const TIN *__restrict__ gamma, const TIN *__restrict__ alpha,
+                                                   const TIN *__restrict__ y, int ldy, double *__restrict__ part, int n_per_split,
+                                                   unsigned char *smem) {
+    typedef P1YChunk<KF1> L;
+    constexpr int NC = 2, NP = NJ / NC;
+    _Float16 *img = reinterpret_cast<_Float16 *>(smem);
+    float *yl = reinterpret_cast<float *>(smem + L::off_y);
+    float *zc = reinterpret_cast<float *>(smem + L::off_zc), *gq = reinterpret_cast<float *>(smem + L::off_gq);
+    const int t = threadIdx.x, lane = t & 63, wv = __builtin_amdgcn_readfirstlane(t >> 6), li = lane & 15, kk = lane >> 4;
+    block_column_means(z, M, Q, zc, reinterpret_cast<double *>(smem));
+    if (t < 32) gq[t] = (t < Q) ? (float)gamma[(size_t)b * Q + t] : 0.0f;
     p1_h8 bop[NJ][KF1];
 #pragma unroll
-    for (int J = 0; J < NJ; ++J)
-#pragma unroll
-        for (int ks = 0; ks < KF1; ++ks)
-            bop[J][ks] = *reinterpret_cast<const p1_h8 *>(bimg + (16 * J + li) * SL + 32 * ks + 8 * kk);
+    for (int ks = 0; ks < KF1; ++ks) {
+        if (ks) __syncthreads();
+        for (int e = t; e < 16 * NJ * 16; e += 256) {
+            const int r = e >> 4, w = e & 15;
+            reinterpret_cast<unsigned *>(img)[r * (L::CLD / 2) + w] = psi2_bimg_word(z, M, Q, zc, mc + r, 16 * ks + w);
+        }
+        __syncthreads();
+#pragma unroll
+        for (int J = 0; J < NJ; ++J) bop[J][ks] = *reinterpret_cast<const p1_h8 *>(img + (16 * J + li) * L::CLD + 8 * kk);
+    }
     float acc[NJ];
 #pragma unroll
     for (int J = 0; J < NJ; ++J) acc[J] = 0.0f;
-    _Float16 *am = &aimg[wv][0];
     const int nbeg = sp * n_per_split, nend = min(N, nbeg + n_per_split);
-    constexpr int NPF = (16 * QPC + 63) / 64;
-    float *cq = &red[wv * 4][0];
-    TIN pf_s[NPF], pf_m[NPF], pf_y = (TIN)0;
-    auto prefetch = [&](int n0) {
-#pragma unroll
-        for (int u = 0; u < NPF; ++u) {
-            const int e = 64 * u + lane, r = e / QPC, q = e - r * QPC, n = n0 + r;
-            const bool ok = (e < 16 * QPC) && (q < Q) && (n < nend);
-            pf_s[u] = ok ? s[(size_t)n * Q + q] : (TIN)1;
-            pf_m[u] = ok ? mu[(size_t)n * Q + q] : (TIN)0;
-        }
-        pf_y = (lane < 16 && n0 + lane < nend) ? y[(size_t)(n0 + lane) * ldy + b] : (TIN)0;
-    };
-    prefetch(nbeg + 16 * wv);
     bool oor = false;
-    for (int n0 = nbeg + 16 * wv; n0 < nend; n0 += 64) {
-#pragma unroll
-        for (int u = 0; u < NPF; ++u) {
-            const int e = 64 * u + lane;
-            if (e < 16 * QPC) {
-                const int r = e / QPC, q = e - r * QPC, n = n0 + r;
-                float a = 0.0f, bb = 0.0f, cc = 0.0f;
-                if (q < Q) {
-                    if (n < nend) {
-                        const float g = gq[q], den = g * (float)pf_s[u] + 1.0f;
-                        const float w1 = g * __builtin_amdgcn_rcpf(den), mcq = (float)pf_m[u] - zc[q];
-                        a = (float)(-0.5 * DPGP_LOG2E) * w1;
-                        bb = (float)DPGP_LOG2E * w1 * mcq;
-                        cc = w1 * mcq * mcq + 0.6931471805599453f * __builtin_amdgcn_logf(den);
+    for (int nb = nbeg; nb < nend; nb += L::R) {
+        __syncthreads();
+        const int ntile = min(L::R / 16, (nend - nb + 15) >> 4);
+        if (t < 16 * ntile) {
+            const int n = nb + t;
+            const bool ok = n < nend;
+            const size_t nc = (size_t)(ok ? n : nend - 1);
+            const TIN yn = y[nc * ldy + b];
+            p1_u4 *row = reinterpret_cast<p1_u4 *>(img + t * L::LD);
+            float c = 0.0f;
+#pragma unroll
+            for (int q4 = 0; q4 < L::QPC / 4; ++q4) {
+                unsigned w[12];
+                float v[4];
+#pragma unroll
+                for (int i = 0; i < 12; ++i) w[i] = 0u;
+#pragma unroll
+                for (int i = 0; i < 4; ++i) v[i] = 0.0f;
+                if (4 * q4 < Q) {
+                    float sv[4], mv[4];
+#pragma unroll
+                    for (int i = 0; i < 4; ++i) {
+                        const int qc = min(4 * q4 + i, Q - 1);
+                        sv[i] = (float)s[nc * Q + qc];
+                        mv[i] = (float)mu[nc * Q + qc];
                     }
-                    a = dpgp_pin(a);
-                    bb = dpgp_pin(bb);
-                    const _Float16 ah = (_Float16)a, al = (_Float16)(a - (float)ah);
-                    const _Float16 bh = (_Float16)bb, bl = (_Float16)(bb - (float)bh);
-                    unsigned *dst = reinterpret_cast<unsigned *>(am + r * SL + 6 * q);
-                    const p1_h2 w0 = {ah, ah}, w1_ = {al, bh}, w2 = {bh, bl};
-                    dst[0] = __builtin_bit_cast(unsigned, w0);
-                    dst[1] = __builtin_bit_cast(unsigned, w1_);
-                    dst[2] = __builtin_bit_cast(unsigned, w2);
+#pragma unroll
+                    for (int i = 0; i < 4; ++i) {
+                        const int q = 4 * q4 + i;
+                        const bool valid = ok && q < Q;
+                        const float g = gq[q], den = g * sv[i] + 1.0f;
+                        const float w1 = g * __builtin_amdgcn_rcpf(den), mcq = mv[i] - zc[q];
+                        float a = (float)(-0.5 * DPGP_LOG2E) * w1;
+                        float bb = (float)DPGP_LOG2E * w1 * mcq;
+                        const float cc = w1 * mcq * mcq + 0.6931471805599453f * __builtin_amdgcn_logf(den);
+                        a = dpgp_pin(valid ? a : 0.0f);
+                        bb = dpgp_pin(valid ? bb : 0.0f);
+                        const _Float16 ah = (_Float16)a, al = (_Float16)(a - (float)ah);
+                        const _Float16 bh = (_Float16)bb, bl = (_Float16)(bb - (float)bh);
+                        const p1_h2 w0 = {ah, ah}, w1_ = {al, bh}, w2 = {bh, bl};
+                        w[3 * i] = __builtin_bit_cast(unsigned, w0);
+                        w[3 * i + 1] = __builtin_bit_cast(unsigned, w1_);
+                        w[3 * i + 2] = __builtin_bit_cast(unsigned, w2);
+                        v[i] = valid ? cc : 0.0f;
+                    }
                 }
-                cq[e] = cc;
-            }
-        }
-        const float yn = (float)pf_y;
-        prefetch(n0 + 64);
-        __builtin_amdgcn_fence(__ATOMIC_RELEASE, "wavefront");
-        __builtin_amdgcn_s_waitcnt(0xc07f);
-        __builtin_amdgcn_fence(__ATOMIC_ACQUIRE, "wavefront");
-        if (lane < 16) {
-            float c = 0.0f;
-#pragma unroll
-            for (int q4 = 0; q4 < QPC / 4; ++q4) {
-                const p1_f4 v = *reinterpret_cast<const p1_f4 *>(cq + lane * QPC + 4 * q4);
                 c += (v[0] + v[1]) + (v[2] + v[3]);
+#pragma unroll
+                for (int u = 0; u < 3; ++u)
+                    if (3 * q4 + u < L::SL / 8) row[3 * q4 + u] = (p1_u4){w[4 * u], w[4 * u + 1], w[4 * u + 2], w[4 * u + 3]};
             }
             c = (float)(-0.5 * DPGP_LOG2E) * c;
             oor |= !(c >= -60000.0f);
@@ -426,60 +428,103 @@
             c = dpgp_pin(c);
             const _Float16 ch = (_Float16)c;
             const p1_h2 cw = {ch, (_Float16)(c - (float)ch)};
-            *reinterpret_cast<unsigned *>(am + lane * SL + 6 * Q) = __builtin_bit_cast(unsigned, cw);
-            yv[wv][lane] = yn;
-        }
-        __builtin_amdgcn_fence(__ATOMIC_RELEASE, "wavefront");
-        __builtin_amdgcn_s_waitcnt(0xc07f);
-        __builtin_amdgcn_fence(__ATOMIC_ACQUIRE, "wavefront");
-        p1_h8 aop[KF1];
-#pragma unroll
-        for (int ks = 0; ks < KF1; ++ks) aop[ks] = *reinterpret_cast<const p1_h8 *>(am + li * SL + 32 * ks + 8 * kk);
-        float y4[4];
-#pragma unroll
-        for (int v = 0; v < 4; ++v) y4[v] = yv[wv][4 * kk + v];
-        p1_f4 c[NJ];
-#pragma unroll
-        for (int J = 0; J < NJ; ++J) c[J] = (p1_f4){0, 0, 0, 0};
-#pragma unroll
-        for (int ks = 0; ks < KF1; ++ks)
-#pragma unroll
-            for (int J = 0; J < NJ; ++J) c[J] = __builtin_amdgcn_mfma_f32_16x16x32_f16(aop[ks], bop[J][ks], c[J], 0, 0, 0);
-#pragma unroll
-        for (int J = 0; J < NJ; ++J)
-#pragma unroll
-            for (int v = 0; v < 4; ++v) acc[J] = fmaf(y4[v], dpgp_exp2(c[J][v]), acc[J]);
-        __builtin_amdgcn_fence(__ATOMIC_ACQ_REL, "wavefront");
+            reinterpret_cast<unsigned *>(row)[3 * Q] = __builtin_bit_cast(unsigned, cw);
+            yl[t] = ok ? (float)yn : 0.0f;
+        }
+        __syncthreads();
+        int j = wv;
+        if (j < ntile) {
+            auto load_a = [&](int jj, p1_h8 *aop, p1_f4 &y4) {
+#pragma unroll
+                for (int ks = 0; ks < KF1; ++ks)
+                    aop[ks] = *reinterpret_cast<const p1_h8 *>(img + (16 * jj + li) * L::LD + 32 * ks + 8 * kk);
+                y4 = *reinterpret_cast<const p1_f4 *>(yl + 16 * jj + 4 * kk);
+            };
+            auto chains = [&](const p1_h8 *aop, int h, p1_f4 *c) {
+#pragma unroll
+                for (int J = 0; J < NC; ++J) c[J] = (p1_f4){0, 0, 0, 0};
+#pragma unroll
+                for (int ks = 0; ks < KF1; ++ks)
+#pragma unroll
+                    for (int J = 0; J < NC; ++J)
+                        c[J] = __builtin_amdgcn_mfma_f32_16x16x32_f16(aop[ks], bop[h * NC + J][ks], c[J], 0, 0, 0);
+            };
+            auto expfma = [&](const p1_f4 *c, int h, const p1_f4 &y4) {
+#pragma unroll
+                for (int J = 0; J < NC; ++J)
+#pragma unroll
+                    for (int v = 0; v < 4; ++v) acc[h * NC + J] = fmaf(y4[v], dpgp_exp2(c[J][v]), acc[h * NC + J]);
+            };
+            p1_h8 aop[KF1];
+            p1_f4 y4, y4n, cc[2][NC];
+            load_a(j, aop, y4);
+            chains(aop, 0, cc[0]);
+            while (j + 4 < ntile) {
+#pragma unroll
+                for (int p = 0; p < NP; ++p) {
+                    chains(aop, (p + 1) % NP, cc[(p + 1) & 1]);
+                    __builtin_amdgcn_sched_barrier(0);
+                    if (p == NP - 2) load_a(j + 4, aop, y4n);
+                    expfma(cc[p & 1], p, y4);
+                    __builtin_amdgcn_sched_barrier(0);
+                }
+                y4 = y4n;
+                j += 4;
+            }
+#pragma unroll
+            for (int p = 0; p < NP; ++p) {
+                if (p + 1 < NP) chains(aop, p + 1, cc[(p + 1) & 1]);
+                __builtin_amdgcn_sched_barrier(0);
+                expfma(cc[p & 1], p, y4);
+                __builtin_amdgcn_sched_barrier(0);
+            }
+        }
     }
     const bool any_oor = __syncthreads_or(oor ? 1 : 0) != 0;
-#pragma unroll
-    for (int J = 0; J < NJ; ++J) red[wv * 4 + kk][16 * J + li] = acc[J];
+    float *red = reinterpret_cast<float *>(smem);
+#pragma unroll
+    for (int J = 0; J < NJ; ++J) red[(wv * 4 + kk) * (16 * NJ) + 16 * J + li] = acc[J];
     __syncthreads();
     if (t < 16 * NJ && mc + t < M) {
         double v = 0.0;
 #pragma unroll
-        for (int k = 0; k < 16; ++k) v += (double)red[k][t];
+        for (int k = 0; k < 16; ++k) v += (double)red[k * (16 * NJ) + t];
         part[((size_t)sp * B + b) * M + mc + t] = any_oor ? (double)__builtin_nanf("") : (double)alpha[b] * v;
     }
 }
 
+template <typename TIN, int KF1, int NJ>
+__global__ __launch_bounds__(256, (KF1 <= 2 ? 4 : 1)) void psi1T_y_chunk_kernel(int N, int M, int Q, int B, const TIN *__restrict__ z,
+                                                            const TIN *__restrict__ mu, const TIN *__restrict__ s,
+                                                            const TIN *__restrict__ gamma, const TIN *__restrict__ alpha,
+                                                            const TIN *__restrict__ y, int ldy, double *__restrict__ part,
+                                                            int n_per_split) {
+    extern __shared__ __align__(16) unsigned char p1y_smem[];
+    psi1T_y_chunk_body<TIN, KF1, NJ>((int)blockIdx.x, (int)blockIdx.y * (16 * NJ), (int)blockIdx.z, N, M, Q, B, z, mu, s, gamma, alpha,
+                                     y, ldy, part, n_per_split, p1y_smem);
+}
+
 template <typename TIN, int KF1>
-static int launch_psi1T_y_f16_kf(int B, int N, int M, int Q, const TIN *z, const TIN *mu, const TIN *s,
-                                 const TIN *gamma, const TIN *alpha, const TIN *y, int ldy, double *part, int ns,
-                                 const unsigned char *consts, hipStream_t st) {
+static int launch_psi1T_y_chunk_kf(int B, int N, int M, int Q, const TIN *z, const TIN *mu, const TIN *s,
+                                   const TIN *gamma, const TIN *alpha, const TIN *y, int ldy, double *part, int ns,
+                                   hipStream_t st) {
     int nper = dpgp_round_up(dpgp_ceil_div(N, ns), 64);
-    if (M <= 64) {
-        dim3 grid(ns, 1, B);
-        DPGP_PRELAUNCH(); hipLaunchKernelGGL((psi1T_y_f16_kernel<TIN, KF1, 4>), grid, dim3(256), 0, st, N, M, Q, B, z, consts, mu, s, gamma,
-                           alpha, y, ldy, part, nper);
+    if constexpr (KF1 < 5) {
+        if (M > 64) {
+            dim3 grid(ns, dpgp_ceil_div(M, 128), B);
+            DPGP_PRELAUNCH(); hipLaunchKernelGGL((psi1T_y_chunk_kernel<TIN, KF1, 8>), grid, dim3(256), P1YChunk<KF1>::bytes, st, N, M, Q, B, z, mu,
+                               s, gamma, alpha, y, ldy, part, nper);
+            DPGP_LAUNCH_CHECK();
+            return DPGP_OK;
+        }
+    }
+    {
+        dim3 grid(ns, dpgp_ceil_div(M, 64), B);
+        DPGP_PRELAUNCH(); hipLaunchKernelGGL((psi1T_y_chunk_kernel<TIN, KF1, 4>), grid, dim3(256), P1YChunk<KF1>::bytes, st, N, M, Q, B, z,
+                           mu, s, gamma, alpha, y, ldy, part, nper);
         DPGP_LAUNCH_CHECK();
         return DPGP_OK;
     }
-    dim3 grid(ns, dpgp_ceil_div(M, 128), B);
-    DPGP_PRELAUNCH(); hipLaunchKernelGGL((psi1T_y_f16_kernel<TIN, KF1, 8>), grid, dim3(256), 0, st, N, M, Q, B, z, consts, mu, s, gamma, alpha, y,
-                       ldy, part, nper);
-    DPGP_LAUNCH_CHECK();
-    return DPGP_OK;
 }
 
 int psi1T_y_nsplit(int B, int N, int M) {
@@ -496,17 +541,11 @@
 
 template <typename TIN, typename T>
 int launch_psi1T_y_partial(int B, int N, int M, int Q, const TIN *z, const TIN *mu, const TIN *s, const TIN *gamma,
-                           const TIN *alpha, const TIN *y, int ldy, double *part, int ns, unsigned char *consts,
-                           int consts_ready, hipStream_t st) {
+                           const TIN *alpha, const TIN *y, int ldy, double *part, int ns, hipStream_t st) {
     if (sizeof(T) == 4) {
-        if (!consts) return -18;
-        if (!consts_ready) {
-            int rc = launch_psi2_consts<TIN>(z, M, Q, consts, st);
-            if (rc) return rc;
-        }
         switch (dpgp_ceil_div(6 * Q + 2, 32)) {
 #define CASE(k) \
-    case k: return launch_psi1T_y_f16_kf<TIN, k>(B, N, M, Q, z, mu, s, gamma, alpha, y, ldy, part, ns, consts, st);
+    case k: return launch_psi1T_y_chunk_kf<TIN, k>(B, N, M, Q, z, mu, s, gamma, alpha, y, ldy, part, ns, st);
             CASE(1) CASE(2) CASE(3) CASE(4) CASE(5) CASE(6)
 #undef CASE
         }
@@ -521,13 +560,13 @@
 }
 template int launch_psi1T_y_partial<float, float>(int, int, int, int, const float *, const float *, const float *,
                                                   const float *, const float *, const float *, int, double *, int,
-                                                  unsigned char *, int, hipStream_t);
+                                                  hipStream_t);
 template int launch_psi1T_y_partial<double, double>(int, int, int, int, const double *, const double *, const double *,
                                                     const double *, const double *, const double *, int, double *, int,
-                                                    unsigned char *, int, hipStream_t);
+                                                    hipStream_t);
 template int launch_psi1T_y_partial<double, float>(int, int, int, int, const double *, const double *, const double *,
                                                    const double *, const double *, const double *, int, double *, int,
-                                                   unsigned char *, int, hipStream_t);
+                                                   hipStream_t);
 
 template <typename T>
 __global__ void sum_slabs_kernel(size_t n, int ns, const double *__restrict__ part, T *__restrict__ out) {
@@ -594,8 +633,8 @@
     __shared__ double scratch[5][64];
     kl_yy_block<TIN>((int)blockIdx.x, N, Q, mu, s, kl_out, D, y, ldy, yy_out, z, M, consts, first_consts_block, scratch);
 }
-template <typename TL>
-__global__ __launch_bounds__(256) void elbo_front_kernel(int N, int Q, const double *__restrict__ mu,
+template <typename TL, int P1KF, int P1NJ>
+__global__ __launch_bounds__(256, (P1KF > 0 ? 4 : 1)) void elbo_front_kernel(int N, int Q, const double *__restrict__ mu,
                                                          const double *__restrict__ s, double *__restrict__ kl_out, int D,
                                                          const double *__restrict__ y, int ldy, double *__restrict__ yy_out,
                                                          const double *__restrict__ z, int M, unsigned char *__restrict__ consts,
@@ -603,10 +642,20 @@
                                                          const double *__restrict__ gamma, const double *__restrict__ alpha,
                                                          const double *__restrict__ beta, TL jitter, TL *__restrict__ kuu,
                                                          int ld_kuu, size_t kuu_stride, int first_scale_block,
-                                                         float *__restrict__ pair_scale, float *__restrict__ pair_fac) {
+                                                         float *__restrict__ pair_scale, float *__restrict__ pair_fac,
+                                                         int p1_blocks, int p1_ns, int p1_nper, double *__restrict__ p1_part) {
     __shared__ double scratch[5][64];
     extern __shared__ __align__(16) unsigned char smem_raw[];
-    const int blk = (int)blockIdx.x;
+    int blk = (int)blockIdx.x;
+    if constexpr (P1KF > 0) {
+        if (blk < p1_blocks) {
+            const int nch = (M + 16 * P1NJ - 1) / (16 * P1NJ), sp = blk % p1_ns, r = blk / p1_ns, ch = r % nch, b = r / nch;
+            psi1T_y_chunk_body<double, P1KF, P1NJ>(sp, ch * (16 * P1NJ), b, N, M, Q, D, z, mu, s, gamma, alpha, y, ldy, p1_part, p1_nper,
+                                                   smem_raw);
+            return;
+        }
+        blk -= p1_blocks;
+    }
 #ifdef FRONT_DIAG_SKIP
     if ((FRONT_DIAG_SKIP & 1) && blk < first_gram_block) return;
 #endif
@@ -614,7 +663,7 @@
         kl_yy_block<double>(blk, N, Q, mu, s, kl_out, D, y, ldy, yy_out, z, M, consts, first_consts_block, scratch);
         return;
     }
-    const int ng = first_scale_block - first_gram_block, nsb = (int)gridDim.x - first_scale_block;
+    const int ng = first_scale_block - first_gram_block, nsb = (int)gridDim.x - p1_blocks - first_scale_block;
     int g = blk - first_gram_block;
     if (nsb > 0) {
         const long long T = (long long)ng + nsb;
@@ -641,11 +690,12 @@
     gram_tile<double, TL, true>(b, ti * GRAM_T, tj * GRAM_T, M, M, Q, z, z, gamma, alpha, beta, DPGP_FLAG_JITTER, jitter, kuu,
                                 ld_kuu, kuu_stride, 1, smem_raw, pair_fac, (size_t)psi2_consts_layout(M, Q).Ppad);
 }
-template <typename TL>
-int launch_elbo_front(int N, int Q, const double *mu, const double *s, double *kl_out, int D, const double *y, int ldy,
-                      double *yy_out, const double *z, int M, unsigned char *psi2_consts, const double *gamma,
-                      const double *alpha, const double *beta, double jitter, TL *kuu, int ld_kuu, size_t kuu_stride,
-                      float *pair_scale, float *pair_fac, hipStream_t st) {
+bool psi1T_y_role_supported(int Q) { return dpgp_ceil_div(6 * Q + 2, 32) <= 2; }
+template <typename TL, int P1KF, int P1NJ>
+static int launch_elbo_front_p1(int N, int Q, const double *mu, const double *s, double *kl_out, int D, const double *y, int ldy,
+                                double *yy_out, const double *z, int M, unsigned char *psi2_consts, const double *gamma,
+                                const double *alpha, const double *beta, double jitter, TL *kuu, int ld_kuu, size_t kuu_stride,
+                                float *pair_scale, float *pair_fac, const Psi1TyRole *p1y, hipStream_t st) {
     int blocks = DPGP_KL_NBLK + dpgp_ceil_div(D, 64) * YY_NCH;
     const int first_consts = blocks;
     blocks += dpgp_ceil_div(M, 64) + dpgp_ceil_div(psi2_consts_layout(M, Q).Ppad, PSI2_PAIR_ROWS_PER_BLOCK);
@@ -653,19 +703,49 @@
     blocks += D * (tm * (tm + 1) / 2);
     const int first_scale = blocks;
     if (pair_scale) blocks += dpgp_ceil_div(D, psi2_scale_dchunk(D)) * dpgp_ceil_div(psi2_consts_layout(M, Q).Ppad, 256);
-    const size_t lds = sizeof(TL) * 2 * GRAM_T * (Q + 1);
-    DPGP_PRELAUNCH(); hipLaunchKernelGGL((elbo_front_kernel<TL>), dim3(blocks), dim3(256), lds, st, N, Q, mu, s, kl_out, D, y, ldy, yy_out,
-                       z, M, psi2_consts, first_consts, first_gram, gamma, alpha, beta, (TL)jitter, kuu, ld_kuu, kuu_stride,
-                       first_scale, pair_scale, pair_fac);
+    size_t lds = sizeof(TL) * 2 * GRAM_T * (Q + 1);
+    int p1_blocks = 0, p1_ns = 1, p1_nper = 0;
+    double *p1_part = nullptr;
+    if constexpr (P1KF > 0) {
+        p1_ns = p1y->ns;
+        p1_part = p1y->part;
+        p1_nper = dpgp_round_up(dpgp_ceil_div(N, p1_ns), 64);
+        p1_blocks = p1_ns * dpgp_ceil_div(M, 16 * P1NJ) * D;
+        if (lds < (size_t)P1YChunk<(P1KF > 0 ? P1KF : 1)>::bytes) lds = (size_t)P1YChunk<(P1KF > 0 ? P1KF : 1)>::bytes;
+    }
+    DPGP_PRELAUNCH(); hipLaunchKernelGGL((elbo_front_kernel<TL, P1KF, P1NJ>), dim3(blocks + p1_blocks), dim3(256), lds, st, N, Q, mu, s,
+                       kl_out, D, y, ldy, yy_out, z, M, psi2_consts, first_consts, first_gram, gamma, alpha, beta, (TL)jitter, kuu, ld_kuu,
+                       kuu_stride, first_scale, pair_scale, pair_fac, p1_blocks, p1_ns, p1_nper, p1_part);
     DPGP_LAUNCH_CHECK();
     return DPGP_OK;
 }
+template <typename TL>
+int launch_elbo_front(int N, int Q, const double *mu, const double *s, double *kl_out, int D, const double *y, int ldy,
+                      double *yy_out, const double *z, int M, unsigned char *psi2_consts, const double *gamma,
+                      const double *alpha, const double *beta, double jitter, TL *kuu, int ld_kuu, size_t kuu_stride,
+                      float *pair_scale, float *pair_fac, const Psi1TyRole *p1y, hipStream_t st) {
+#define FRONT(kf, nj)                                                                                                               \
+    return launch_elbo_front_p1<TL, kf, nj>(N, Q, mu, s, kl_out, D, y, ldy, yy_out, z, M, psi2_consts, gamma, alpha, beta, jitter, kuu, \
+                                            ld_kuu, kuu_stride, pair_scale, pair_fac, p1y, st)
+    if (p1y && p1y->part) {
+        if (!psi1T_y_role_supported(Q) || p1y->ns < 1) return -4;
+        const int kf1 = dpgp_ceil_div(6 * Q + 2, 32);
+        if (M <= 64) {
+            if (kf1 == 1) FRONT(1, 4);
+            FRONT(2, 4);
+        }
+        if (kf1 == 1) FRONT(1, 8);
+        FRONT(2, 8);
+    }
+    FRONT(0, 0);
+#undef FRONT
+}
 template int launch_elbo_front<float>(int, int, const double *, const double *, double *, int, const double *, int, double *,
                                       const double *, int, unsigned char *, const double *, const double *, const double *,
-                                      double, float *, int, size_t, float *, float *, hipStream_t);
+                                      double, float *, int, size_t, float *, float *, const Psi1TyRole *, hipStream_t);
 template int launch_elbo_front<double>(int, int, const double *, const double *, double *, int, const double *, int, double *,
                                        const double *, int, unsigned char *, const double *, const double *, const double *,
-                                       double, double *, int, size_t, float *, float *, hipStream_t);
+                                       double, double *, int, size_t, float *, float *, const Psi1TyRole *, hipStream_t);
 
 template <typename TIN>
 int launch_kl_yy(int N, int Q, const TIN *mu, const TIN *s, double *kl_out, int D, const TIN *y, int ldy,
@@ -766,7 +846,7 @@
 
 extern "C" size_t dpgp_psi1T_y_workspace_bytes(int B, int N, int M) {
     if (B <= 0 || N <= 0 || M <= 0) return 0;
-    return dpgp_align256(sizeof(double) * (size_t)psi1T_y_nsplit(B, N, M) * B * M) + psi2_consts_bytes(M, DPGP_MAX_Q);
+    return dpgp_align256(sizeof(double) * (size_t)psi1T_y_nsplit(B, N, M) * B * M);
 }
 template <typename T>
 static int psi1T_y_api(int B, int N, int M, int Q, const T *z, const T *mu, const T *s, const T *gamma, const T *alpha,
@@ -776,9 +856,7 @@
     CHECK_ARG(ldy >= B, 11); CHECK_ARG(out, 12); CHECK_ARG(ws, 13);
     CHECK_ARG(ws_bytes >= dpgp_psi1T_y_workspace_bytes(B, N, M), 14);
     int ns = psi1T_y_nsplit(B, N, M);
-    unsigned char *consts = (unsigned char *)ws + dpgp_align256(sizeof(double) * (size_t)ns * B * M);
-    int rc = launch_psi1T_y_partial<T, T>(B, N, M, Q, z, mu, s, gamma, alpha, y, ldy, (double *)ws, ns, consts, 0,
-                                          (hipStream_t)stream);
+    int rc = launch_psi1T_y_partial<T, T>(B, N, M, Q, z, mu, s, gamma, alpha, y, ldy, (double *)ws, ns, (hipStream_t)stream);
     if (rc) return rc;
     size_t tot = (size_t)B * M;
     DPGP_PRELAUNCH(); hipLaunchKernelGGL((sum_slabs_kernel<T>), dim3((unsigned)((tot + 255) / 256)), dim3(256), 0, (hipStream_t)stream,
diff --git a/dp_gp_lvm_amd/csrc/internal.h b/dp_gp_lvm_amd/csrc/internal.h
--- a/dp_gp_lvm_amd/csrc/internal.h
+++ b/dp_gp_lvm_amd/csrc/internal.h
@@ -40,19 +40,23 @@
 int psi1T_y_nsplit(int B, int N, int M);
 template <typename TIN, typename T>
 int launch_psi1T_y_partial(int B, int N, int M, int Q, const TIN *z, const TIN *mu, const TIN *s, const TIN *gamma,
-                           const TIN *alpha, const TIN *y, int ldy, double *part, int ns, unsigned char *psi2_consts,
-                           int consts_ready, hipStream_t st);
+                           const TIN *alpha, const TIN *y, int ldy, double *part, int ns, hipStream_t st);
 
 #define DPGP_YY_NCH 16
 #define DPGP_KL_NBLK 16
 template <typename TIN>
 int launch_kl_yy(int N, int Q, const TIN *mu, const TIN *s, double *kl_out, int D, const TIN *y, int ldy,
                  double *yy_out, const TIN *z, int M, unsigned char *psi2_consts, hipStream_t st);
+struct Psi1TyRole {
+    double *part;
+    int ns;
+};
+bool psi1T_y_role_supported(int Q);
 template <typename TL>
 int launch_elbo_front(int N, int Q, const double *mu, const double *s, double *kl_out, int D, const double *y, int ldy,
                       double *yy_out, const double *z, int M, unsigned char *psi2_consts, const double *gamma,
                       const double *alpha, const double *beta, double jitter, TL *kuu, int ld_kuu, size_t kuu_stride,
-                      float *pair_scale, float *pair_fac, hipStream_t st);
+                      float *pair_scale, float *pair_fac, const Psi1TyRole *p1y, hipStream_t st);
 
 int psi2_nsplit(int B, int N, int M);
 size_t psi2_consts_bytes(int M, int Q);
diff --git a/dp_gp_lvm_amd/csrc/psi2_consts.h b/dp_gp_lvm_amd/csrc/psi2_consts.h
--- a/dp_gp_lvm_amd/csrc/psi2_consts.h
+++ b/dp_gp_lvm_amd/csrc/psi2_consts.h
@@ -31,6 +31,29 @@
 }
 
 template <typename TIN>
+__device__ __forceinline__ unsigned psi2_bimg_word(const TIN *__restrict__ z, int M, int Q, const float *zc, int m, int w) {
+    _Float16 h2[2];
+#pragma unroll
+    for (int i = 0; i < 2; ++i) {
+        const int slot = 2 * w + i;
+        float val = 0.0f;
+        if (slot < 6 * Q) {
+            const int tt = slot / 3, part = slot - 3 * tt, q = tt >> 1;
+            const float zz = (m < M) ? (float)z[(size_t)m * Q + q] - zc[q] : 0.0f;
+            const float v = dpgp_pin((tt & 1) ? zz : zz * zz);
+            const _Float16 h = (_Float16)v;
+            val = (part == 1) ? (float)(_Float16)(v - (float)h) : (float)h;
+        } else if (slot < 6 * Q + 2) {
+            val = 1.0f;
+        }
+        h2[i] = (_Float16)val;
+    }
+    typedef _Float16 h2v __attribute__((ext_vector_type(2)));
+    const h2v hv = {h2[0], h2[1]};
+    return __builtin_bit_cast(unsigned, hv);
+}
+
+template <typename TIN>
 __device__ __forceinline__ void psi2_consts_rows(const TIN *__restrict__ z, int M, int Q, unsigned char *__restrict__ dst,
                                                  int blk, double *scratch) {
     const Psi2Consts c = psi2_consts_layout(M, Q);
@@ -47,25 +70,7 @@
     }
     for (int e = t; e < 64 * c.SL / 2; e += 256) {
         const int r = e / (c.SL / 2), w = e - r * (c.SL / 2), m = m0 + r;
-        _Float16 h2[2];
-#pragma unroll
-        for (int i = 0; i < 2; ++i) {
-            const int slot = 2 * w + i;
-            float val = 0.0f;
-            if (slot < 6 * Q) {
-                const int tt = slot / 3, part = slot - 3 * tt, q = tt >> 1;
-                const float zz = (m < M) ? (float)z[(size_t)m * Q + q] - zc[q] : 0.0f;
-                const float v = dpgp_pin((tt & 1) ? zz : zz * zz);
-                const _Float16 h = (_Float16)v;
-                val = (part == 1) ? (float)(_Float16)(v - (float)h) : (float)h;
-            } else if (slot < 6 * Q + 2) {
-                val = 1.0f;
-            }
-            h2[i] = (_Float16)val;
-        }
-        typedef _Float16 h2v __attribute__((ext_vector_type(2)));
-        const h2v hv = {h2[0], h2[1]};
-        reinterpret_cast<unsigned *>(bimg)[(size_t)m * (c.SL / 2) + w] = __builtin_bit_cast(unsigned, hv);
+        reinterpret_cast<unsigned *>(bimg)[(size_t)m * (c.SL / 2) + w] = psi2_bimg_word(z, M, Q, zc, m, w);
     }
 }
 
diff --git a/include/dpgp.h b/include/dpgp.h
--- a/include/dpgp.h
+++ b/include/dpgp.h
@@ -167,6 +167,7 @@
                   const double *alpha, double *out, void *stream);
 
 size_t dpgp_psi1T_y_workspace_bytes(int B, int N, int M);
+int dpgp_psi1T_y_chunk_rows(int Q);
 int dpgp_psi1T_y_f32(int B, int N, int M, int Q, const float *z, const float *mu, const float *s, const float *gamma,
                      const float *alpha, const float *y, int ldy, float *out, void *ws, size_t ws_bytes, void *stream);
 int dpgp_psi1T_y_f64(int B, int N, int M, int Q, const double *z, const double *mu, const double *s,
```

New measurement: 820.4 (median of 6 runs). Within noise of the previous version (+0.5%).
